# bronemos/view-fusion

Measured on AMD Instinct MI355X. Metric: denoise_steps_per_sec, higher is better.
Workload: dtype f32; 1 GPU; small UNet 64x64 (33.9M params), B=16/GPU N=6 (S=96 views/GPU), training iteration fwd+bwd+Adam, linear T=2000 schedule; global_batch=16, views=6, parallelism=dp1, launch=HIP-graph replay of the whole iteration

## Files before the change

### include/vf_hip.h

```cpp
#ifndef VF_HIP_H
#define VF_HIP_H
#ifdef __cplusplus
extern "C" {
#endif

int vf_gn_fwd(const float* x, const float* gamma, const float* beta, float* y, float* mean ,
              float* rstd , int S, int C, int HW, int groups, float eps, int silu, void* stream);
int vf_gn_bwd_emits_rowsum(int C, int HW, int groups);
int vf_gn_bwd(const float* x, const float* gamma, const float* beta, const float* mean, const float* rstd,
              const float* dy, const float* addend, float* dx, float* dgamma_part, float* dbeta_part,
              float* dx_rowsum, int S, int C, int HW, int groups, int silu, void* stream);
int vf_gn_cat_fwd(const float* x, const float* x2, int C1, const float* gamma, const float* beta, float* y, float* mean,
                  float* rstd, int S, int C, int HW, int groups, float eps, int silu, void* stream);
int vf_gn_cat_bwd(const float* x, const float* x2, int C1, const float* gamma, const float* beta, const float* mean,
                  const float* rstd, const float* dy, const float* addend, const float* addend2, float* dx, float* dx2,
                  float* dgamma_part, float* dbeta_part, float* dx_rowsum, int S, int C, int HW, int groups, int silu,
                  void* stream);
int vf_rowsum(const float* x, float* out , int rows, int len, void* stream);
int vf_bias_grad(const float* dy, float* db, float* dvb, int S, int C, int HW, void* stream);
int vf_colsum(const float* part , float* out , int batch, int S, int C,
              void* stream);
int vf_colsum_multi(const void* desc, int n, long total_blocks, void* stream);

int vf_conv_pack_sizes(int Cout, int Cin, int KS, long* fwd_floats, long* bwd_floats);
int vf_conv_pack_weights(const float* w_oihw, float* w_fwd, float* w_bwd , int Cout, int Cin, int KS,
                         void* stream);
int vf_conv_pack_weights_multi(const void* desc, int nlayers, long total_blocks, void* stream);
int vf_conv_fwd(const float* x, const float* w_packed, const float* bias ,
                const float* view_bias , const float* residual , float* y,
                float* ws , long ws_floats, int S, int Cin, int Cout, int H, int W, int KS, int mode,
                void* stream);
int vf_conv_fwd_gn(const float* x, const float* w_packed, const float* bias, const float* view_bias, const float* residual,
                   float* y, int store_y, const float* gn_gamma, const float* gn_beta, float* a_out, float* gn_stats,
                   int groups, float eps, int silu, float* ws, long ws_floats, int S, int Cin, int Cout, int H, int W,
                   int KS, int mode, void* stream);
int vf_conv_small_supported(int Cin, int Cout, int H, int W, int KS, int mode);
int vf_conv_small(const float* x, const float* x2 , int C1, const float* w_oihw, const float* bias ,
                  const float* view_bias , const float* residual , float* y, int S, int Cin, int Cout,
                  int H, int W, int KS, int mode, void* stream);
int vf_conv_small_res(const float* x, const float* w_oihw, const float* bias , const float* view_bias ,
                      float* y, int S, int Cin, int Cout, int H, int W, const float* rx, const float* rx2 ,
                      int rC1, int rC, const float* rw_oihw, const float* rbias , void* stream);
int vf_conv_small_gn(const float* x, const float* x2 , int C1, const float* w_oihw, const float* bias ,
                     const float* view_bias , const float* residual , float* y, int S, int Cin,
                     int Cout, int H, int W, int KS, const unsigned long long* in_stats ,
                     const float* in_gamma, const float* in_beta, int in_groups, float eps, int silu,
                     unsigned long long* out_stats , const float* rx , const float* rx2 ,
                     int rC1, int rC, const float* rw_oihw, const float* rbias , const float* w_packed ,
                     int mode, void* stream);
long vf_conv_small_pack_floats(int Cout, int Cin);
int vf_conv_small_pack(const float* w_oihw, float* w_packed, int Cout, int Cin, void* stream);
long vf_conv_fwd_ws_floats(int S, int Cin, int Cout, int H, int W, int KS);
int vf_conv1x1_cat_fwd(const float* x1, const float* x2, int C1, const float* w_packed, const float* bias, float* y,
                       float* ws, long ws_floats, int S, int Cin, int Cout, int H, int W, void* stream);
int vf_conv1x1_cat_dgrad(const float* dy, const float* w_packed_bwd, float* dx1, float* dx2, int C1, int S, int Cin,
                         int Cout, int H, int W, void* stream);
int vf_conv1x1_cat_wgrad(const float* x1, const float* x2, int C1, const float* dy, float* dw_oihw, float* ws,
                         long ws_floats, int S, int Cin, int Cout, int H, int W, void* stream);
long vf_conv1x1_bf16x3_pack_dwords(int M, int K);
int vf_conv1x1_bf16x3_pack(const float* w_oihw, void* w3_fwd, void* w3_bwd, int Cout, int Cin, void* stream);
int vf_conv1x1_bf16x3(const float* x, const float* x2, int C1in, const void* w3, const float* bias,
                      const float* view_bias, const float* residual, float* y, float* y2, int C1out, int S, int Cin,
                      int Cout, int HW, void* stream);
long vf_conv_wgrad_ws_floats(int S, int Cin, int Cout, int H, int W, int KS);
int vf_conv_wgrad(const float* x, const float* dy, float* dw_oihw, float* ws, long ws_floats, int S, int Cin,
                  int Cout, int H, int W, int KS, int mode, void* stream);
int vf_conv_wgrad_main(const float* x, const float* dy, float* dw_oihw, float* ws, long ws_floats, int S, int Cin,
                       int Cout, int H, int W, int KS, int mode, long long* desc9, int* nblocks, void* stream);
int vf_conv1x1_cat_wgrad_main(const float* x1, const float* x2, int C1, const float* dy, float* dw_oihw, float* ws,
                              long ws_floats, int S, int Cin, int Cout, int H, int W, long long* desc9, int* nblocks,
                              void* stream);
int vf_sumpool2(const float* x, float* y, long n_out, int Wo, void* stream);

int vf_wino_supported(int H, int W, int mode);
int vf_wino_pack_sizes(int Cout, int Cin, long* fwd_floats, long* bwd_floats);
int vf_wino_pack_weights(const float* w_oihw, float* u_fwd, float* u_bwd , int Cout, int Cin,
                         void* stream);
int vf_wino_pack_weights_multi(const void* desc, int nlayers, long total_blocks, void* stream);
long vf_wino_conv_ws_floats(int S, int Cin, int Cout, int H, int W);
int vf_wino_conv_fill_pct(int S, int Cin, int Cout, int H, int W, int* tiles_out);
int vf_wino_conv_fwd(const float* x, const float* u_packed, const float* bias, const float* view_bias,
                     const float* residual, float* y, float* ws, long ws_floats, int S, int Cin, int Cout, int H,
                     int W, int mode, void* stream);
int vf_wino_conv_gn_fusable(int S, int Cin, int Cout, int H, int W, int mode, int groups);
int vf_wino_conv_fwd_gn(const float* x, const float* u_packed, const float* bias , const float* view_bias ,
                        const float* residual , float* y, int store_y, const float* gn_gamma, const float* gn_beta,
                        float* a_out, int groups, float eps, int silu, float* ws, long ws_floats, int S, int Cin, int Cout,
                        int H, int W, int mode, void* stream);
int vf_wino44_supported(int H, int W, int mode);
int vf_wino44_pack_sizes(int Cout, int Cin, long* fwd_floats, long* bwd_floats);
int vf_wino44_pack_weights(const float* w_oihw, float* u_fwd, float* u_bwd , int Cout, int Cin,
                           void* stream);
int vf_wino44_pack_weights_multi(const void* desc, int nlayers, long total_blocks, void* stream);
long vf_wino44_conv_ws_floats(int S, int Cin, int Cout, int H, int W);
int vf_wino44_conv_fill_pct(int S, int Cin, int Cout, int H, int W, int* tiles_out);
int vf_wino44_conv_fwd(const float* x, const float* u_packed, const float* bias, const float* view_bias,
                       const float* residual, float* y, float* ws, long ws_floats, int S, int Cin, int Cout, int H,
                       int W, int mode, void* stream);
int vf_wino_wgrad_supported(int H, int W, int mode);
long vf_wino_wgrad_ws_floats(int S, int Cin, int Cout, int H, int W);
int vf_wino_wgrad(const float* x, const float* dy, float* dw_oihw, float* db, float* db2, float* ws, long ws_floats,
                  int S, int Cin, int Cout, int H, int W, int mode, void* stream);
int vf_wino_wgrad_main(const float* x, const float* dy, float* dw_oihw, float* db, float* db2, float* ws, long ws_floats,
                       int S, int Cin, int Cout, int H, int W, int mode, long long* desc9, int* nblocks, void* stream);
int vf_wino44_reduce_multi(const void* table, int nrows, int nblocks, void* stream);

int vf_time_affine_fwd(const void* desc, int ngroups, const float* emb, float* out, int S, int K, int CT,
                       void* stream);
long vf_time_affine_ws_floats(int S, int K);
int vf_time_affine_bwd(const void* desc, int ngroups, const float* emb, const float* de, float* dw ,
                       float* db , const void* gdst, float* demb , float* ws, int S, int K,
                       int CT, void* stream);

int vf_bgemm(const float* A, const float* B, float* C, const float* bias , int batch, int M, int N,
             int K, long sAb, long sAm, long sAk, long sBb, long sBk, long sBn, long sCb, long sCm, long sCn,
             float alpha, float beta, void* stream);
int vf_attention_fwd(const float* qkv, float* out, float* P , int S, int C, int L, void* stream);
int vf_attention_fwd_kernel(int S, int C, int L);
int vf_attention_dscore(const float* qkv, const float* dO, const float* P, float* dS, float* dqkv, int S, int C, int L,
                        void* stream);
int vf_attention_dvdk(const float* qkv, const float* dO, const float* P, const float* dS, float* dqkv, int S, int C, int L,
                      void* stream);
int vf_attn_stream_fwd(const float* qkv, float* out, float* rowstat , int S, int C, int L, void* stream);
int vf_attn_stream_bwd(const float* qkv, const float* out, const float* dO, const float* rowstat, float* delta,
                       float* dqkv, int S, int C, int L, void* stream);
int vf_softmax_fwd(const float* x, float* y, int rows, int cols, void* stream);
int vf_softmax_bwd(const float* y, const float* dy, float* dx, int rows, int cols, void* stream);

int vf_sincos_embed(const float* level , const float* angle , float* out , int S, int dim,
                    void* stream);
int vf_swish_fwd(const float* x, float* y, long n, void* stream);
int vf_swish_bwd(const float* x, const float* dy, float* dx, long n, void* stream);
int vf_concat_channels(float* a, float* b, float* out, int S, long na, long nb, int split, void* stream);
int vf_dropout(const float* x, const float* u, float* y, long n, float p, void* stream);

int vf_gather_level(const float* gammas, const long long* t, const float* u , float* level, int B,
                    void* stream);
int vf_stack_views(const float* y_cond , const float* y_t ,
                   const float* noise , const float* level, const float* angle, const int* off ,
                   float* x , float* level_s, float* angle_s, int B, int Nmax,
                   int Cc , int HW, int S,
                   int copy_cond, void* stream);
int vf_compose_fwd(const float* unet_out, const int* off, const float* target , float* noise_hat,
                   float* weights , float* loss_part , float* loss, int B,
                   int Cout, int HW, int maxV, int weighting, void* stream);
int vf_compose_mse_bwd(const float* unet_out, const int* off, const float* target, const float* noise_hat,
                       const float* gloss, float* dout, int B, int Cout, int HW, int weighting, void* stream);
int vf_compose_loss_fwd(const float* unet_out, const int* off, const float* target, const float* level,
                        float* noise_hat, float* loss_part , float* sample_loss ,
                        float* sample_w , float* loss, float* bin_sum , int* bin_cnt ,
                        int B, int Cout, int HW, int weighting, int penalty, float delta, int weight_kind, float a,
                        float b, int K, void* stream);
int vf_compose_loss_bwd(const float* unet_out, const int* off, const float* target, const float* noise_hat,
                        const float* gloss, const float* sample_w, float* dout, int B, int Cout, int HW, int weighting,
                        int penalty, float delta, void* stream);
int vf_compose_loss_fwd_scaled(const float* unet_out, const int* off, const float* target, const float* level,
                               const float* scale , float* noise_hat, float* loss_part ,
                               float* sample_loss , float* sample_w , float* loss,
                               float* bin_sum , int* bin_cnt , int B, int Cout, int HW,
                               int weighting, int penalty, float delta, int weight_kind, float a, float b, int K,
                               void* stream);
int vf_draw_level(unsigned long long seed, const long long* ids , const long long* words ,
                  const float* gammas, int T, int K, const unsigned long long* c, const float* iw, const int* ready,
                  long long* t, float* u , float* level , float* iw_out , int B, void* stream);
int vf_level_stats(const float* sample_loss, const float* sample_w , const long long* t, int B, int T, int K,
                   float beta, int warmup, double eps, float* m, int* seen, unsigned long long* c, float* iw,
                   int* ready, void* stream);
int vf_level_table_host(const double* q, int T, int K, double eps, unsigned long long* c, int* lo, float* iw);
int vf_level_draw_host(const unsigned* x, int n, int T, int K, const unsigned long long* c, const float* iw,
                       long long* t, float* iw_out);
int vf_loss_weights_host(const float* level, int B, int kind, float a, float b, float* out );
int vf_compose_loss_pred_fwd(const float* unet_out, const int* off, const float* noise ,
                             const float* y_0, const float* level, const float* scale , float* noise_hat,
                             float* loss_part , float* sample_loss ,
                             float* sample_w , float* loss, float* bin_sum ,
                             int* bin_cnt , int B, int Cout, int HW, int weighting, int penalty, float delta,
                             int weight_kind, float a, float b, int K, int pred, void* stream);
int vf_compose_loss_pred_bwd(const float* unet_out, const int* off, const float* noise ,
                             const float* y_0, const float* level, const float* noise_hat, const float* gloss,
                             const float* sample_w, float* dout, int B, int Cout, int HW, int weighting, int penalty,
                             float delta, int pred, void* stream);
int vf_loss_weights_pred_host(const float* level, int B, int pred, int kind, float a, float b, float* out );
int vf_p_sample_tail(const float* unet_out, const int* off, const float* y_t, const float* z ,
                     const long long* t, const float* sqrt_recip_gammas, const float* sqrt_recipm1_gammas,
                     const float* posterior_log_variance, const float* posterior_mean_coef1,
                     const float* posterior_mean_coef2, float* y_next , float* mean_out ,
                     float* weights , int B, int Cout, int HW, int maxV, int weighting, int clip,
                     void* stream);

int vf_draw_train(unsigned long long seed, const long long* ids, const float* gammas, int T, long long* t,
                  float* u , float* level , int B, void* stream);
int vf_randn_ids(unsigned long long seed, const long long* ids, int kind, int step, float* out, int B, int n,
                 void* stream);
int vf_philox_ids(unsigned long long seed, const long long* ids, int kind, int step, unsigned* out, int B, int n,
                  void* stream);
int vf_p_sample_tail_rng(const float* unet_out, const int* off, const float* y_t, unsigned long long seed,
                         const long long* ids, const long long* t, const float* sqrt_recip_gammas,
                         const float* sqrt_recipm1_gammas, const float* posterior_log_variance,
                         const float* posterior_mean_coef1, const float* posterior_mean_coef2,
                         float* y_next , float* mean_out , float* weights , int B, int Cout,
                         int HW, int maxV, int weighting, int clip, void* stream);
int vf_sampler_step(const float* unet_out, const int* off, const float* y_t, const float* z ,
                    const long long* kidx, const float* a, const float* b, const float* cy, const float* c0,
                    const float* c1, const float* sigma, float* y0_prev , float* y_next,
                    float* weights , int B, int Cout, int HW, int maxV, int weighting, void* stream);
int vf_sampler_step_rng(const float* unet_out, const int* off, const float* y_t, unsigned long long seed,
                        const long long* ids, const long long* kidx, const long long* tau, const float* a,
                        const float* b, const float* cy, const float* c0, const float* c1, const float* sigma,
                        float* y0_prev , float* y_next, float* weights , int B, int Cout, int HW,
                        int maxV, int weighting, void* stream);
int vf_stack_views_cfg(const float* y_cond, const float* y_t, const float* noise , const float* level,
                       const float* angle, const int* off , const unsigned char* drop , float* x,
                       float* level_s, float* angle_s, int B, int Nmax, int Cc, int HW, int S, int copy_cond,
                       int null_rows, void* stream);
int vf_draw_cond_drop(unsigned long long seed, const long long* ids, unsigned thr, unsigned char* drop , int B,
                      void* stream);
int vf_p_sample_tail_cfg(const float* unet_out, const int* off, const float* y_t, const float* z ,
                         const long long* t, const float* sqrt_recip_gammas, const float* sqrt_recipm1_gammas,
                         const float* posterior_log_variance, const float* posterior_mean_coef1,
                         const float* posterior_mean_coef2, float* y_next , float* mean_out ,
                         float* weights , int B, int Cout, int HW, int maxV, int weighting, int clip,
                         const float* g , void* stream);
int vf_p_sample_tail_cfg_rng(const float* unet_out, const int* off, const float* y_t, unsigned long long seed,
                             const long long* ids, const long long* t, const float* sqrt_recip_gammas,
                             const float* sqrt_recipm1_gammas, const float* posterior_log_variance,
                             const float* posterior_mean_coef1, const float* posterior_mean_coef2,
                             float* y_next , float* mean_out , float* weights , int B,
                             int Cout, int HW, int maxV, int weighting, int clip, const float* g ,
                             void* stream);
int vf_sampler_step_cfg(const float* unet_out, const int* off, const float* y_t, const float* z ,
                        const long long* kidx, const float* a, const float* b, const float* cy, const float* c0,
                        const float* c1, const float* sigma, float* y0_prev , float* y_next,
                        float* weights , int B, int Cout, int HW, int maxV, int weighting,
                        const float* g , void* stream);
int vf_sampler_step_cfg_rng(const float* unet_out, const int* off, const float* y_t, unsigned long long seed,
                            const long long* ids, const long long* kidx, const long long* tau, const float* a,
                            const float* b, const float* cy, const float* c0, const float* c1, const float* sigma,
                            float* y0_prev , float* y_next, float* weights , int B, int Cout, int HW,
                            int maxV, int weighting, const float* g , void* stream);
int vf_compose_eps(const float* unet_out, const int* off, const float* g , float* eps,
                   float* weights , double* part, int B, int Cout, int HW, int maxV, int weighting, int fused,
                   void* stream);
int vf_sample_stat(const float* eps, const double* part , const float* y, const long long* idx, const float* ta,
                   const float* tb, float* stat, int B, int HW, float phi, int k, float frac, float cmax, int fused,
                   void* stream);
int vf_abs_quantile(const float* x, int B, int n, int k, float frac, float* out , void* stream);
int vf_p_sample_tail_eps(const float* eps, const float* stat, const float* y_t, const float* z ,
                         const long long* t, const float* sqrt_recip_gammas, const float* sqrt_recipm1_gammas,
                         const float* posterior_log_variance, const float* posterior_mean_coef1,
                         const float* posterior_mean_coef2, float* y_next , float* mean_out , int B,
                         int HW, int clip, int rescale, int thr, void* stream);
int vf_p_sample_tail_eps_rng(const float* eps, const float* stat, const float* y_t, unsigned long long seed,
                             const long long* ids, const long long* t, const float* sqrt_recip_gammas,
                             const float* sqrt_recipm1_gammas, const float* posterior_log_variance,
                             const float* posterior_mean_coef1, const float* posterior_mean_coef2,
                             float* y_next , float* mean_out , int B, int HW, int clip, int rescale,
                             int thr, void* stream);
int vf_sampler_step_eps(const float* eps, const float* stat, const float* y_t, const float* z ,
                        const long long* kidx, const float* a, const float* b, const float* cy, const float* c0,
                        const float* c1, const float* sigma, float* y0_prev , float* y_next, int B,
                        int HW, int rescale, int thr, void* stream);
int vf_sampler_step_eps_rng(const float* eps, const float* stat, const float* y_t, unsigned long long seed,
                            const long long* ids, const long long* kidx, const long long* tau, const float* a,
                            const float* b, const float* cy, const float* c0, const float* c1, const float* sigma,
                            float* y0_prev , float* y_next, int B, int HW, int rescale, int thr, void* stream);
int vf_distill_begin(unsigned long long seed, const long long* ids , const long long* i_in ,
                     const long long* tau_s, const float* gammas, int K, const float* y_0, const float* noise,
                     long long* i_out, long long* k1, long long* k0, float* level_s, float* z_t, int B, int n,
                     void* stream);
int vf_distill_target(const float* unet_out, const int* off, const float* y, const float* x1, const float* z_t,
                      const float* level_s, const long long* idx, const long long* kidx, const float* a, const float* b,
                      const float* w1, const float* w2, float* x_tilde, float* eps_tilde, int B, int Cout, int HW,
                      int weighting, const float* g , void* stream);
int vf_distill_step_host(unsigned long long seed, const long long* ids, int K, long long* i_out , int B);
int vf_loss_weights_trunc_snr_host(const float* level, int B, int pred, float* out );
int vf_rng_host_philox(const unsigned* counter , const unsigned* key , unsigned* out );
int vf_rng_host_normal(unsigned long long seed, const long long* ids, int kind, int step, float* out ,
                       int B, int n);
int vf_rng_host_train_scalars(unsigned long long seed, const long long* ids, int T, long long* t, float* u, int B);
int vf_cond_drop_host(unsigned long long seed, const long long* ids, unsigned thr, unsigned char* drop , int B);

int vf_batch_assemble(const unsigned char* store, long N, int H, int W, unsigned long long seed, const long long* ids,
                      const long long* objects, int B, int train, int relative, int all, float* y_0, float* y_cond,
                      float* angle, long long* objects_out, void* stream);
int vf_batch_host_plan(unsigned long long seed, const long long* ids, int B, int train, int lo, int hi, long N,
                       const long long* objects, int* src, int* target, int* q01, int* second, long long* view_count,
                       long long* object);

int vf_psnr(const float* generated, const float* target, float* out , int B, int n, void* stream);
long vf_ssim_workspace_floats(int B, int C, int H, int W);
int vf_ssim(const float* generated, const float* target, float* out , float* workspace, int B, int C, int H,
            int W, const float* window11, float data_range, void* stream);
int vf_lpips_prep(const float* generated, const float* target, float* out, int B, int HW, void* stream);
int vf_relu(float* x, long n, void* stream);
int vf_relu_maxpool2(float* y, float* pooled, long planes, int H, int W, void* stream);
int vf_lpips_layer_tiles(int C, int HW);
long vf_lpips_workspace_floats(int B, int H, int W);
int vf_lpips_layer(const float* feat, const float* lin, float* workspace, int B, int C, int HW, int slot0, int slots,
                   void* stream);
int vf_lpips_finish(const float* workspace, float* out , int B, int slots, void* stream);

int vf_adam_multi(const void* desc, int ntensors, long total_blocks, float lr, float beta1, float beta2, float eps,
                  float bias_correction1, float bias_correction2, void* stream);
int vf_adam_multi_dev(const void* desc, int ntensors, long total_blocks, const float* scalars, float beta1, float beta2,
                      float eps, void* stream);
int vf_adam_set_scalars(float* scalars, float lr, float bc1, float bc2, void* stream);

int vf_grad_sumsq_multi(const void* desc, int ntensors, long total_blocks, double* partial, void* stream);
int vf_grad_norm_finish(const double* partial, long n, const float* max_norm, float* out, void* stream);
int vf_adam_multi_ex(const void* desc, const void* ema_tab, int ntensors, long total_blocks, float lr, float beta1,
                     float beta2, float eps, float bias_correction1, float bias_correction2, const float* gscale,
                     const float* ema_scal, void* stream);
int vf_adam_multi_ex_dev(const void* desc, const void* ema_tab, int ntensors, long total_blocks, const float* scalars,
                         float beta1, float beta2, float eps, const float* gscale, const float* ema_scal, void* stream);
int vf_adam_set_scalars_ex(float* scalars, float lr, float bc1, float bc2, float* xs, float ema_d, float ema_omd,
                           float max_norm, void* stream);
int vf_swap_multi(const void* desc, const void* ema_tab, int ntensors, long total_blocks, void* stream);

int vf_grad_accum_multi(const void* desc, int ntensors, long total_blocks, const float* scalars, void* stream);

int vf_xgmi_alloc(void** ptr, long bytes);
int vf_xgmi_free(void* ptr);
int vf_xgmi_export(void* ptr, void* handle64 );
int vf_xgmi_open(const void* handle64, void** ptr);
int vf_xgmi_close(void* ptr);
int vf_xgmi_signal(const void* const* peer_flags, int world, int rank, int slot, unsigned epoch, void* stream);
int vf_xgmi_wait(const void* my_flags, int world, int slot_lo, int slot_hi, unsigned epoch, void* status,
                 long timeout_us, void* stream);
int vf_xgmi_reduce_adam(const void* desc, int ntensors, long total_blocks, const void* const* peer_bases,
                        const float* my_base, float* gavg_base, int world, const float* scalars, float beta1,
                        float beta2, float eps, void* stream);

#ifdef __cplusplus
}
#endif
#endif
```

### view_fusion_amd/_lib.py

```python
import ctypes
import os

import torch

_HERE = os.path.dirname(os.path.abspath(__file__))
LIB_PATH = os.path.join(_HERE, "lib", "libvf_hip.so")
_OVERRIDE = os.environ.get("VF_HIP_LIB") if os.environ.get("VF_DEBUG_AB") == "1" else None
if _OVERRIDE:
    LIB_PATH = _OVERRIDE
elif os.environ.get("VF_HIP_LIB"):
    import warnings
    warnings.warn("VF_HIP_LIB is ignored unless VF_DEBUG_AB=1 (kernel-tuning aid)", stacklevel=2)

_P, _I, _L, _F = ctypes.c_void_p, ctypes.c_int, ctypes.c_long, ctypes.c_float
_U64 = ctypes.c_uint64

SIGNATURES = {
    "vf_gn_fwd": [_P, _P, _P, _P, _P, _P, _I, _I, _I, _I, _F, _I, _P],
    "vf_gn_bwd_emits_rowsum": [_I, _I, _I],
    "vf_gn_cat_fwd": [_P, _P, _I, _P, _P, _P, _P, _P, _I, _I, _I, _I, _F, _I, _P],
    "vf_gn_cat_bwd": [_P, _P, _I, _P, _P, _P, _P, _P, _P, _P, _P, _P, _P, _P, _P, _I, _I, _I, _I, _I, _P],
    "vf_conv1x1_cat_fwd": [_P, _P, _I, _P, _P, _P, _P, _L, _I, _I, _I, _I, _I, _P],
    "vf_conv1x1_cat_dgrad": [_P, _P, _P, _P, _I, _I, _I, _I, _I, _I, _P],
    "vf_conv1x1_cat_wgrad": [_P, _P, _I, _P, _P, _P, _L, _I, _I, _I, _I, _I, _P],
    "vf_gn_bwd": [_P, _P, _P, _P, _P, _P, _P, _P, _P, _P, _P, _I, _I, _I, _I, _I, _P],
    "vf_rowsum": [_P, _P, _I, _I, _P],
    "vf_bias_grad": [_P, _P, _P, _I, _I, _I, _P],
    "vf_colsum": [_P, _P, _I, _I, _I, _P],
    "vf_colsum_multi": [_P, _I, _L, _P],
    "vf_conv_pack_sizes": [_I, _I, _I, ctypes.POINTER(_L), ctypes.POINTER(_L)],
    "vf_conv_pack_weights": [_P, _P, _P, _I, _I, _I, _P],
    "vf_conv_pack_weights_multi": [_P, _I, _L, _P],
    "vf_conv_fwd": [_P, _P, _P, _P, _P, _P, _P, _L, _I, _I, _I, _I, _I, _I, _I, _P],
    "vf_conv_fwd_ws_floats": [_I, _I, _I, _I, _I, _I],
    "vf_conv_fwd_gn": [_P, _P, _P, _P, _P, _P, _I, _P, _P, _P, _P, _I, _F, _I, _P, _L, _I, _I, _I, _I, _I, _I, _I, _P],
    "vf_conv_wgrad_ws_floats": [_I, _I, _I, _I, _I, _I],
    "vf_conv_wgrad": [_P, _P, _P, _P, _L, _I, _I, _I, _I, _I, _I, _I, _P],
    "vf_conv1x1_bf16x3_pack_dwords": [_I, _I],
    "vf_conv1x1_bf16x3_pack": [_P, _P, _P, _I, _I, _P],
    "vf_conv1x1_bf16x3": [_P, _P, _I, _P, _P, _P, _P, _P, _P, _I, _I, _I, _I, _I, _P],
    "vf_wino_supported": [_I, _I, _I],
    "vf_wino_pack_sizes": [_I, _I, ctypes.POINTER(_L), ctypes.POINTER(_L)],
    "vf_wino_pack_weights": [_P, _P, _P, _I, _I, _P],
    "vf_wino_pack_weights_multi": [_P, _I, _L, _P],
    "vf_wino_conv_ws_floats": [_I, _I, _I, _I, _I],
    "vf_wino_conv_fill_pct": [_I, _I, _I, _I, _I, ctypes.POINTER(_I)],
    "vf_wino_conv_fwd": [_P, _P, _P, _P, _P, _P, _P, _L, _I, _I, _I, _I, _I, _I, _P],
    "vf_wino_conv_gn_fusable": [_I, _I, _I, _I, _I, _I, _I],
    "vf_wino_conv_fwd_gn": [_P, _P, _P, _P, _P, _P, _I, _P, _P, _P, _I, _F, _I, _P, _L, _I, _I, _I, _I, _I, _I, _P],
    "vf_wino44_supported": [_I, _I, _I],
    "vf_wino44_pack_sizes": [_I, _I, ctypes.POINTER(_L), ctypes.POINTER(_L)],
    "vf_wino44_pack_weights": [_P, _P, _P, _I, _I, _P],
    "vf_wino44_pack_weights_multi": [_P, _I, _L, _P],
    "vf_wino44_conv_ws_floats": [_I, _I, _I, _I, _I],
    "vf_wino44_conv_fill_pct": [_I, _I, _I, _I, _I, ctypes.POINTER(_I)],
    "vf_wino44_conv_fwd": [_P, _P, _P, _P, _P, _P, _P, _L, _I, _I, _I, _I, _I, _I, _P],
    "vf_wino_wgrad_ws_floats": [_I, _I, _I, _I, _I],
    "vf_wino_wgrad_supported": [_I, _I, _I],
    "vf_wino_wgrad": [_P, _P, _P, _P, _P, _P, _L, _I, _I, _I, _I, _I, _I, _P],
    "vf_wino_wgrad_main": [_P, _P, _P, _P, _P, _P, _L, _I, _I, _I, _I, _I, _I, _P, _P, _P],
    "vf_wino44_reduce_multi": [_P, _I, _I, _P],
    "vf_conv_wgrad_main": [_P, _P, _P, _P, _L, _I, _I, _I, _I, _I, _I, _I, _P, _P, _P],
    "vf_conv1x1_cat_wgrad_main": [_P, _P, _I, _P, _P, _P, _L, _I, _I, _I, _I, _I, _P, _P, _P],
    "vf_sumpool2": [_P, _P, _L, _I, _P],
    "vf_time_affine_fwd": [_P, _I, _P, _P, _I, _I, _I, _P],
    "vf_time_affine_ws_floats": [_I, _I],
    "vf_time_affine_bwd": [_P, _I, _P, _P, _P, _P, _P, _P, _P, _I, _I, _I, _P],
    "vf_bgemm": [_P, _P, _P, _P, _I, _I, _I, _I, _L, _L, _L, _L, _L, _L, _L, _L, _L, _F, _F, _P],
    "vf_attention_fwd": [_P, _P, _P, _I, _I, _I, _P],
    "vf_attention_fwd_kernel": [_I, _I, _I],
    "vf_attention_dscore": [_P, _P, _P, _P, _P, _I, _I, _I, _P],
    "vf_attention_dvdk": [_P, _P, _P, _P, _P, _I, _I, _I, _P],
    "vf_attn_stream_fwd": [_P, _P, _P, _I, _I, _I, _P],
    "vf_attn_stream_bwd": [_P, _P, _P, _P, _P, _P, _I, _I, _I, _P],
    "vf_softmax_fwd": [_P, _P, _I, _I, _P],
    "vf_softmax_bwd": [_P, _P, _P, _I, _I, _P],
    "vf_sincos_embed": [_P, _P, _P, _I, _I, _P],
    "vf_swish_fwd": [_P, _P, _L, _P],
    "vf_swish_bwd": [_P, _P, _P, _L, _P],
    "vf_concat_channels": [_P, _P, _P, _I, _L, _L, _I, _P],
    "vf_dropout": [_P, _P, _P, _L, _F, _P],
    "vf_adam_multi": [_P, _I, _L, _F, _F, _F, _F, _F, _F, _P],
    "vf_conv_small_supported": [_I, _I, _I, _I, _I, _I],
    "vf_conv_small": [_P, _P, _I, _P, _P, _P, _P, _P, _I, _I, _I, _I, _I, _I, _I, _P],
    "vf_conv_small_res": [_P, _P, _P, _P, _P, _I, _I, _I, _I, _I, _P, _P, _I, _I, _P, _P, _P],
    "vf_conv_small_gn": [_P, _P, _I, _P, _P, _P, _P, _P, _I, _I, _I, _I, _I, _I, _P, _P, _P, _I, _F, _I, _P, _P, _P, _I, _I,
                         _P, _P, _P, _I, _P],
    "vf_conv_small_pack_floats": [_I, _I],
    "vf_conv_small_pack": [_P, _P, _I, _I, _P],
    "vf_adam_multi_dev": [_P, _I, _L, _P, _F, _F, _F, _P],
    "vf_adam_set_scalars": [_P, _F, _F, _F, _P],
    "vf_grad_sumsq_multi": [_P, _I, _L, _P, _P],
    "vf_grad_norm_finish": [_P, _L, _P, _P, _P],
    "vf_adam_multi_ex": [_P, _P, _I, _L, _F, _F, _F, _F, _F, _F, _P, _P, _P],
    "vf_adam_multi_ex_dev": [_P, _P, _I, _L, _P, _F, _F, _F, _P, _P, _P],
    "vf_adam_set_scalars_ex": [_P, _F, _F, _F, _P, _F, _F, _F, _P],
    "vf_swap_multi": [_P, _P, _I, _L, _P],
    "vf_grad_accum_multi": [_P, _I, _L, _P, _P],
    "vf_xgmi_alloc": [ctypes.POINTER(_P), _L],
    "vf_xgmi_free": [_P],
    "vf_xgmi_export": [_P, _P],
    "vf_xgmi_open": [_P, ctypes.POINTER(_P)],
    "vf_xgmi_close": [_P],
    "vf_xgmi_signal": [ctypes.POINTER(_P), _I, _I, _I, ctypes.c_uint, _P],
    "vf_xgmi_wait": [_P, _I, _I, _I, ctypes.c_uint, _P, _L, _P],
    "vf_xgmi_reduce_adam": [_P, _I, _L, ctypes.POINTER(_P), _P, _P, _I, _P, _F, _F, _F, _P],
    "vf_psnr": [_P, _P, _P, _I, _I, _P],
    "vf_ssim_workspace_floats": [_I, _I, _I, _I],
    "vf_ssim": [_P, _P, _P, _P, _I, _I, _I, _I, _P, _F, _P],
    "vf_lpips_prep": [_P, _P, _P, _I, _I, _P],
    "vf_relu": [_P, _L, _P],
    "vf_relu_maxpool2": [_P, _P, _L, _I, _I, _P],
    "vf_lpips_layer_tiles": [_I, _I],
    "vf_lpips_workspace_floats": [_I, _I, _I],
    "vf_lpips_layer": [_P, _P, _P, _I, _I, _I, _I, _I, _P],
    "vf_lpips_finish": [_P, _P, _I, _I, _P],
    "vf_gather_level": [_P, _P, _P, _P, _I, _P],
    "vf_stack_views": [_P, _P, _P, _P, _P, _P, _P, _P, _P, _I, _I, _I, _I, _I, _I, _P],
    "vf_compose_fwd": [_P, _P, _P, _P, _P, _P, _P, _I, _I, _I, _I, _I, _P],
    "vf_compose_mse_bwd": [_P, _P, _P, _P, _P, _P, _I, _I, _I, _I, _P],
    "vf_compose_loss_fwd": [_P, _P, _P, _P, _P, _P, _P, _P, _P, _P, _P, _I, _I, _I, _I, _I, _F, _I, _F, _F, _I, _P],
    "vf_compose_loss_bwd": [_P, _P, _P, _P, _P, _P, _P, _I, _I, _I, _I, _I, _F, _P],
    "vf_loss_weights_host": [_P, _I, _I, _F, _F, _P],
    "vf_compose_loss_fwd_scaled": [_P, _P, _P, _P, _P, _P, _P, _P, _P, _P, _P, _P, _I, _I, _I, _I, _I, _F, _I, _F, _F, _I,
                                   _P],
    "vf_compose_loss_pred_fwd": [_P, _P, _P, _P, _P, _P, _P, _P, _P, _P, _P, _P, _P, _I, _I, _I, _I, _I, _F, _I, _F, _F, _I,
                                 _I, _P],
    "vf_compose_loss_pred_bwd": [_P, _P, _P, _P, _P, _P, _P, _P, _P, _I, _I, _I, _I, _I, _F, _I, _P],
    "vf_loss_weights_pred_host": [_P, _I, _I, _I, _F, _F, _P],
    "vf_draw_level": [_U64, _P, _P, _P, _I, _I, _P, _P, _P, _P, _P, _P, _P, _I, _P],
    "vf_level_stats": [_P, _P, _P, _I, _I, _I, _F, _I, ctypes.c_double, _P, _P, _P, _P, _P, _P],
    "vf_level_table_host": [_P, _I, _I, ctypes.c_double, _P, _P, _P],
    "vf_level_draw_host": [_P, _I, _I, _I, _P, _P, _P, _P],
    "vf_p_sample_tail": [_P, _P, _P, _P, _P, _P, _P, _P, _P, _P, _P, _P, _P, _I, _I, _I, _I, _I, _I, _P],
    "vf_draw_train": [_U64, _P, _P, _I, _P, _P, _P, _I, _P],
    "vf_randn_ids": [_U64, _P, _I, _I, _P, _I, _I, _P],
    "vf_philox_ids": [_U64, _P, _I, _I, _P, _I, _I, _P],
    "vf_p_sample_tail_rng": [_P, _P, _P, _U64, _P, _P, _P, _P, _P, _P, _P, _P, _P, _P, _I, _I, _I, _I, _I, _I, _P],
    "vf_sampler_step": [_P, _P, _P, _P, _P, _P, _P, _P, _P, _P, _P, _P, _P, _P, _I, _I, _I, _I, _I, _P],
    "vf_sampler_step_rng": [_P, _P, _P, _U64, _P, _P, _P, _P, _P, _P, _P, _P, _P, _P, _P, _P, _I, _I, _I, _I, _I, _P],
    "vf_stack_views_cfg": [_P, _P, _P, _P, _P, _P, _P, _P, _P, _P, _I, _I, _I, _I, _I, _I, _I, _P],
    "vf_draw_cond_drop": [_U64, _P, ctypes.c_uint, _P, _I, _P],
    "vf_cond_drop_host": [_U64, _P, ctypes.c_uint, _P, _I],
    "vf_p_sample_tail_cfg": [_P, _P, _P, _P, _P, _P, _P, _P, _P, _P, _P, _P, _P, _I, _I, _I, _I, _I, _I, _P, _P],
    "vf_p_sample_tail_cfg_rng": [_P, _P, _P, _U64, _P, _P, _P, _P, _P, _P, _P, _P, _P, _P, _I, _I, _I, _I, _I, _I, _P, _P],
    "vf_sampler_step_cfg": [_P, _P, _P, _P, _P, _P, _P, _P, _P, _P, _P, _P, _P, _P, _I, _I, _I, _I, _I, _P, _P],
    "vf_sampler_step_cfg_rng": [_P, _P, _P, _U64, _P, _P, _P, _P, _P, _P, _P, _P, _P, _P, _P, _P, _I, _I, _I, _I, _I, _P, _P],
    "vf_compose_eps": [_P, _P, _P, _P, _P, _P, _I, _I, _I, _I, _I, _I, _P],
    "vf_sample_stat": [_P, _P, _P, _P, _P, _P, _P, _I, _I, _F, _I, _F, _F, _I, _P],
    "vf_abs_quantile": [_P, _I, _I, _I, _F, _P, _P],
    "vf_p_sample_tail_eps": [_P, _P, _P, _P, _P, _P, _P, _P, _P, _P, _P, _P, _I, _I, _I, _I, _I, _P],
    "vf_p_sample_tail_eps_rng": [_P, _P, _P, _U64, _P, _P, _P, _P, _P, _P, _P, _P, _P, _I, _I, _I, _I, _I, _P],
    "vf_sampler_step_eps": [_P, _P, _P, _P, _P, _P, _P, _P, _P, _P, _P, _P, _P, _I, _I, _I, _I, _P],
    "vf_sampler_step_eps_rng": [_P, _P, _P, _U64, _P, _P, _P, _P, _P, _P, _P, _P, _P, _P, _P, _I, _I, _I, _I, _P],
    "vf_distill_begin": [_U64, _P, _P, _P, _P, _I, _P, _P, _P, _P, _P, _P, _P, _I, _I, _P],
    "vf_distill_target": [_P, _P, _P, _P, _P, _P, _P, _P, _P, _P, _P, _P, _P, _P, _I, _I, _I, _I, _P, _P],
    "vf_distill_step_host": [_U64, _P, _I, _P, _I],
    "vf_loss_weights_trunc_snr_host": [_P, _I, _I, _P],
    "vf_rng_host_philox": [_P, _P, _P],
    "vf_rng_host_normal": [_U64, _P, _I, _I, _P, _I, _I],
    "vf_rng_host_train_scalars": [_U64, _P, _I, _P, _P, _I],
    "vf_batch_assemble": [_P, _L, _I, _I, _U64, _P, _P, _I, _I, _I, _I, _P, _P, _P, _P, _P],
    "vf_batch_host_plan": [_U64, _P, _I, _I, _I, _I, _L, _P, _P, _P, _P, _P, _P, _P],
}
_RESTYPE = {"vf_conv1x1_bf16x3_pack_dwords": _L, "vf_conv_wgrad_ws_floats": _L, "vf_time_affine_ws_floats": _L, "vf_wino_conv_ws_floats": _L, "vf_wino44_conv_ws_floats": _L, "vf_wino_wgrad_ws_floats": _L, "vf_conv_fwd_ws_floats": _L,
            "vf_conv_small_pack_floats": _L, "vf_ssim_workspace_floats": _L, "vf_lpips_workspace_floats": _L}

_lib = None
N_CALLS = 0


class VFHipError(RuntimeError):
    pass


def load():
    global _lib
    if _lib is None:
        if not os.path.exists(LIB_PATH):
            raise VFHipError(
                f"{LIB_PATH} not found: build it with `python -m view_fusion_amd.build` "
                "(there is no CPU / eager fallback for the ViewFusion hot path)")
        lib = ctypes.CDLL(LIB_PATH)
        if _OVERRIDE:
            import sys
            print(f"[view_fusion_amd] VF_DEBUG_AB: loading {LIB_PATH} instead of lib/libvf_hip.so", file=sys.stderr)
        missing = [name for name in SIGNATURES if not hasattr(lib, name)]
        if missing:
            raise VFHipError(f"{LIB_PATH} does not export {missing}: stale build? run `python -m view_fusion_amd.build`")
        for name, args in SIGNATURES.items():
            fn = getattr(lib, name)
            fn.argtypes = args
            fn.restype = _RESTYPE.get(name, _I)
        _lib = lib
    return _lib


def call(name, *args):
    global N_CALLS
    N_CALLS += 1
    rc = getattr(load(), name)(*args)
    if rc != 0:
        raise VFHipError(f"{name} failed with hipError_t {rc}")
```

### view_fusion_amd/csrc/attention.hip

```cpp
#include "common.h"

namespace {

__global__ __launch_bounds__(512) void attn_fwd_kh_kernel(const float* __restrict__ qkv, float* __restrict__ out,
                                                          float* __restrict__ P, int C, float alpha) {
    constexpr int L = 256, NTH = 512, QW = 128, NKT = 4, CKA = 16, RSV = L + 4;
    constexpr int KS = L + 32;
    constexpr int KQ = CKA * KS + CKA * QW, VT = 32 * RSV;
    __shared__ __attribute__((aligned(16))) float lds[2 * (KQ > VT ? KQ : VT)];
    __shared__ float oex[2][4][16][64];
    __shared__ float red[2][2][QW];

    const int tid = threadIdx.x, lane = tid & 63, wid = tid >> 6;
    const int li = lane & 31, lh = lane >> 5;
    const int qb = wid & 3, kh = wid >> 2;
    const int b = blockIdx.y, q0 = blockIdx.x * QW;
    const float* qp = qkv + (size_t)b * 3 * C * L;
    const float* kp = qp + (size_t)C * L;
    const float* vp = qp + (size_t)2 * C * L;

#ifdef VF_ATTN_STAMPS
    long long st_[6] = {clock64(), 0, 0, 0, 0, 0}, rt0_ = wall_clock64();
#endif
    f32x16 acc[NKT];
#pragma unroll
    for (int t = 0; t < NKT; ++t) acc[t] = (f32x16){0};

    float4 kr0, kr1, qr;
#define VF_AK_LOAD(C0) {                                                                                    \
        kr0 = *reinterpret_cast<const float4*>(kp + (size_t)((C0) + tid / 64) * L + 4 * (tid % 64));          \
        kr1 = *reinterpret_cast<const float4*>(kp + (size_t)((C0) + 8 + tid / 64) * L + 4 * (tid % 64));      \
        qr = *reinterpret_cast<const float4*>(qp + (size_t)((C0) + tid / 32) * L + q0 + 4 * (tid % 32)); }
#define VF_AK_STORE(BUF) { float* kl_ = lds + (BUF) * KQ;                                                    \
        *reinterpret_cast<float4*>(kl_ + (tid / 64) * KS + 4 * (tid % 64)) = kr0;                             \
        *reinterpret_cast<float4*>(kl_ + (8 + tid / 64) * KS + 4 * (tid % 64)) = kr1;                         \
        *reinterpret_cast<float4*>(kl_ + CKA * KS + (tid / 32) * QW + 4 * (tid % 32)) = qr; }
    VF_AK_LOAD(0);
    VF_AK_STORE(0);
    VF_AK_LOAD(min(CKA, C - CKA));
    __syncthreads();
    for (int c0 = 0, cur = 0; c0 < C; c0 += CKA, cur ^= 1) {
        VF_AK_STORE(cur ^ 1);
        VF_AK_LOAD(min(c0 + 2 * CKA, C - CKA));
        const float* Kl = lds + cur * KQ;
        const float* Ql = Kl + CKA * KS;
        const float* kq = Kl + lh * KS + kh * NKT * 32 + li;
        const float* qq = Ql + lh * QW + qb * 32 + li;
        float bq = qq[0], ak0 = kq[0], ak1 = kq[32], ak2 = kq[64], ak3 = kq[96];
#pragma unroll
        for (int s = 0; s < CKA / 2; ++s) {
            float bqn = bq, an0 = ak0, an1 = ak1, an2 = ak2, an3 = ak3;
            if (s + 1 < CKA / 2) {
                bqn = qq[(2 * s + 2) * QW];
                an0 = kq[(2 * s + 2) * KS];
                an1 = kq[(2 * s + 2) * KS + 32];
                an2 = kq[(2 * s + 2) * KS + 64];
                an3 = kq[(2 * s + 2) * KS + 96];
            }
            __builtin_amdgcn_sched_barrier(0);
            acc[0] = __builtin_amdgcn_mfma_f32_32x32x2f32(ak0, bq, acc[0], 0, 0, 0);
            acc[1] = __builtin_amdgcn_mfma_f32_32x32x2f32(ak1, bq, acc[1], 0, 0, 0);
            acc[2] = __builtin_amdgcn_mfma_f32_32x32x2f32(ak2, bq, acc[2], 0, 0, 0);
            acc[3] = __builtin_amdgcn_mfma_f32_32x32x2f32(ak3, bq, acc[3], 0, 0, 0);
            __builtin_amdgcn_sched_barrier(0);
            bq = bqn; ak0 = an0; ak1 = an1; ak2 = an2; ak3 = an3;
        }
        __syncthreads();
    }
#undef VF_AK_LOAD
#undef VF_AK_STORE
#ifdef VF_ATTN_STAMPS
    st_[1] = clock64();
#endif
    float4 vr0, vr1, vr2, vr3;
#define VF_AK_LV(I, C0) { const int e = tid + (I) * NTH;                                                   \
        vr##I = *reinterpret_cast<const float4*>(vp + (size_t)((C0) + e / 64) * L + 4 * (e % 64)); }
#define VF_AK_SV(I, BUF) { const int e = tid + (I) * NTH;                                                   \
        *reinterpret_cast<float4*>(lds + (BUF) * VT + (e / 64) * RSV + 4 * (e % 64)) = vr##I; }
#define VF_AK_LOADV(C0) { VF_AK_LV(0, C0) VF_AK_LV(1, C0) VF_AK_LV(2, C0) VF_AK_LV(3, C0) }
#define VF_AK_STOREV(BUF) { VF_AK_SV(0, BUF) VF_AK_SV(1, BUF) VF_AK_SV(2, BUF) VF_AK_SV(3, BUF) }
    VF_AK_LOADV(0);

    const int ql = qb * 32 + li;
    float mx = -INFINITY;
#pragma unroll
    for (int t = 0; t < NKT; ++t)
#pragma unroll
        for (int r = 0; r < 16; ++r) mx = fmaxf(mx, acc[t][r]);
    mx = fmaxf(mx, __shfl_xor(mx, 32, 64));
    if (lh == 0) red[0][kh][ql] = mx;
    __syncthreads();
    mx = fmaxf(red[0][0][ql], red[0][1][ql]);
    const float c2 = alpha * 1.44269504088896341f, mc = mx * c2;
    float sum = 0.f;
#pragma unroll
    for (int t = 0; t < NKT; ++t)
#pragma unroll
        for (int r = 0; r < 16; ++r) {
            const float p = __builtin_amdgcn_exp2f(fmaf(acc[t][r], c2, -mc));
            acc[t][r] = p;
            sum += p;
        }
    sum += __shfl_xor(sum, 32, 64);
    if (lh == 0) red[1][kh][ql] = sum;
    VF_AK_STOREV(0);
    VF_AK_LOADV(min(32, C - 32));
    __syncthreads();
    const float inv = 1.0f / (red[1][0][ql] + red[1][1][ql]);
#pragma unroll
    for (int t = 0; t < NKT; ++t)
#pragma unroll
        for (int r = 0; r < 16; ++r) acc[t][r] *= inv;

    const int qi = q0 + ql;
#ifdef VF_ATTN_STAMPS
    st_[2] = clock64();
    if (false) {
#else
    if (P) {
#endif
        float* pr = P + ((size_t)b * L + qi) * L + kh * NKT * 32;
#pragma unroll
        for (int t = 0; t < NKT; ++t)
#pragma unroll
            for (int g = 0; g < 4; ++g)
                *reinterpret_cast<float4*>(pr + t * 32 + 8 * g + 4 * lh) =
                    make_float4(acc[t][4 * g], acc[t][4 * g + 1], acc[t][4 * g + 2], acc[t][4 * g + 3]);
    }
#ifdef VF_ATTN_STAMPS
    st_[3] = clock64();
#endif

    f32x16 oprev = {0};
    for (int c0 = 0, cur = 0; c0 < C; c0 += 32, cur ^= 1) {
        if (kh == 0 && c0 > 0) {
#pragma unroll
            for (int r = 0; r < 16; ++r) {
                const int c = c0 - 32 + (r & 3) + 8 * (r >> 2) + 4 * lh;
                out[((size_t)b * C + c) * L + qi] = oprev[r] + oex[cur ^ 1][qb][r][lane];
            }
        }
        VF_AK_STOREV(cur ^ 1);
        VF_AK_LOADV(min(c0 + 64, C - 32));
        const float* Vl = lds + cur * VT;
        f32x16 o = {0};
        const float* vq = Vl + li * RSV + kh * NKT * 32 + 4 * lh;
        float4 av = *reinterpret_cast<const float4*>(vq);
#pragma unroll
        for (int t = 0; t < NKT; ++t)
#pragma unroll
            for (int g = 0; g < 4; ++g) {
                float4 avn = av;
                if (t * 4 + g + 1 < NKT * 4) avn = *reinterpret_cast<const float4*>(vq + (t * 4 + g + 1) * 8);
                __builtin_amdgcn_sched_barrier(0);
                o = __builtin_amdgcn_mfma_f32_32x32x2f32(av.x, acc[t][4 * g + 0], o, 0, 0, 0);
                o = __builtin_amdgcn_mfma_f32_32x32x2f32(av.y, acc[t][4 * g + 1], o, 0, 0, 0);
                o = __builtin_amdgcn_mfma_f32_32x32x2f32(av.z, acc[t][4 * g + 2], o, 0, 0, 0);
                o = __builtin_amdgcn_mfma_f32_32x32x2f32(av.w, acc[t][4 * g + 3], o, 0, 0, 0);
                __builtin_amdgcn_sched_barrier(0);
                av = avn;
            }
        if (kh == 1) {
#pragma unroll
            for (int r = 0; r < 16; ++r) oex[cur][qb][r][lane] = o[r];
        } else {
            oprev = o;
        }
        VF_LDS_BARRIER();
    }
    if (kh == 0) {
        const int last = (C / 32 - 1) & 1;
#pragma unroll
        for (int r = 0; r < 16; ++r) {
            const int c = C - 32 + (r & 3) + 8 * (r >> 2) + 4 * lh;
            out[((size_t)b * C + c) * L + qi] = oprev[r] + oex[last][qb][r][lane];
        }
    }
#undef VF_AK_LOADV
#undef VF_AK_STOREV
#undef VF_AK_LV
#undef VF_AK_SV
#ifdef VF_ATTN_STAMPS
    if (tid == 0 && P) {
        long long* o = reinterpret_cast<long long*>(P) + (size_t)(blockIdx.y * gridDim.x + blockIdx.x) * 8;
        o[0] = st_[0]; o[1] = st_[1]; o[2] = st_[2]; o[3] = st_[3]; o[4] = clock64(); o[5] = 0;
        o[6] = rt0_; o[7] = wall_clock64();
    }
#endif
}

template <bool DSCORE>
__global__ __launch_bounds__(256, 3) void attn_fwd_q32_kernel(const float* __restrict__ qkv, float* __restrict__ out,
                                                              float* __restrict__ P, int C, float alpha, int S,
                                                              const float* __restrict__ dO, float* __restrict__ dS) {
    constexpr int L = 256, NTH = 256, NKT = 2, CKA = 16;
    constexpr int KS = L + 32;
    constexpr int KQ = CKA * KS + CKA * 32;
    constexpr int RSV = 36, VW = 32 * RSV;
    constexpr int OEX = 4 * 16 * 64;
    constexpr int PV = 4 * VW + 2 * OEX;
    __shared__ __attribute__((aligned(16))) float lds[2 * KQ > PV ? 2 * KQ : PV];
    __shared__ float red[2][4][32];

    const int tid = threadIdx.x, lane = tid & 63;
    const int w = __builtin_amdgcn_readfirstlane(tid >> 6);
    const int li = lane & 31, lh = lane >> 5;
    int b, u;
    {
        const int i = blockIdx.x, nfull = (S >> 3) << 6;
        if (i < nfull) { const int j = i >> 3; b = ((j >> 3) << 3) + (i & 7); u = j & 7; }
        else { const int r = i - nfull; b = ((S >> 3) << 3) + (r >> 3); u = r & 7; }
    }
    const int q0 = u * 32;
    const float* qp = DSCORE ? dO + (size_t)b * C * L : qkv + (size_t)b * 3 * C * L;
    const float* kp = qkv + ((size_t)b * 3 + (DSCORE ? 2 : 1)) * C * L;
    const float* vp = qkv + ((size_t)b * 3 + (DSCORE ? 1 : 2)) * C * L;
#ifdef VF_ATTN_STAMPS
    long long st_[6] = {clock64(), 0, 0, 0, 0, 0}, rt0_ = wall_clock64();
#endif

    f32x16 acc[NKT];
#pragma unroll
    for (int t = 0; t < NKT; ++t) acc[t] = (f32x16){0};

    f32x4 ka0, ka1, ka2, ka3, qa, kb0, kb1, kb2, kb3, qb_;
    const int qe = tid & 127;
    unsigned kvo = (unsigned)((4 * w * L + 4 * lane) * 4);
    unsigned qvo = (unsigned)(((qe >> 3) * L + q0 + 4 * (qe & 7)) * 4);
    float* const kst = lds + 4 * w * KS + 4 * lane;
    float* const qst = lds + CKA * KS + (qe >> 3) * 32 + 4 * (qe & 7);
#define VF_GLD4(BASE, OFS, IMM) (*(const __attribute__((address_space(1))) f32x4*)((const __attribute__((address_space(1))) char*)(BASE) + (OFS) + (IMM)))
#define VF_A3_LK(R, I, KC) R##I = VF_GLD4(KC, kvo, (I) * (L * 4));
#define VF_A3_LOAD(R, Q, C0) { const char* kc_ = uniform_ptr(kp + (size_t)(C0) * L);                               \
        const char* qc_ = uniform_ptr(qp + (size_t)(C0) * L);                                                    \
        asm("" : "+s"(kc_), "+s"(qc_), "+v"(kvo), "+v"(qvo));                                                    \
        VF_A3_LK(R, 0, kc_) VF_A3_LK(R, 1, kc_) VF_A3_LK(R, 2, kc_) VF_A3_LK(R, 3, kc_)                             \
        Q = VF_GLD4(qc_, qvo, 0); }
#define VF_A3_SK(R, I, BUF) *reinterpret_cast<f32x4*>(kst + (BUF) * KQ + (I) * KS) = R##I;
#define VF_A3_STORE(R, Q, BUF) { VF_A3_SK(R, 0, BUF) VF_A3_SK(R, 1, BUF) VF_A3_SK(R, 2, BUF) VF_A3_SK(R, 3, BUF)   \
        *reinterpret_cast<f32x4*>(qst + (BUF) * KQ) = Q; }
#define VF_A3_MFMAS(BUF, MID) {                                                                                 \
        const float* Kl = lds + (BUF) * KQ;                                                                    \
        const float* kq = Kl + lh * KS + w * (NKT * 32) + li;                                                  \
        const float* qq = Kl + CKA * KS + lh * 32 + li;                                                        \
        float bq = qq[0], ak0 = kq[0], ak1 = kq[32];                                                           \
        _Pragma("unroll")                                                                                      \
        for (int s = 0; s < CKA / 2; ++s) {                                                                    \
            float bqn = bq, an0 = ak0, an1 = ak1;                                                              \
            if (s + 1 < CKA / 2) {                                                                             \
                bqn = qq[(2 * s + 2) * 32];                                                                    \
                an0 = kq[(2 * s + 2) * KS];                                                                    \
                an1 = kq[(2 * s + 2) * KS + 32];                                                               \
            }                                                                                                  \
            __builtin_amdgcn_sched_barrier(0);                                                                 \
            acc[0] = __builtin_amdgcn_mfma_f32_32x32x2f32(ak0, bq, acc[0], 0, 0, 0);                           \
            acc[1] = __builtin_amdgcn_mfma_f32_32x32x2f32(ak1, bq, acc[1], 0, 0, 0);                           \
            __builtin_amdgcn_sched_barrier(0);                                                                 \
            if (s == 0) { MID __builtin_amdgcn_sched_barrier(0); }                                             \
            bq = bqn; ak0 = an0; ak1 = an1;                                                                    \
        } }
    VF_A3_LOAD(ka, qa, 0);
    VF_A3_STORE(ka, qa, 0);
    VF_A3_LOAD(ka, qa, CKA);
    VF_A3_LOAD(kb, qb_, min(2 * CKA, C - CKA));
    __syncthreads();
    for (int c0 = 0; c0 < C; c0 += 2 * CKA) {
        VF_A3_MFMAS(0, VF_A3_STORE(ka, qa, 1) VF_A3_LOAD(ka, qa, min(c0 + 3 * CKA, C - CKA)));
        VF_LDS_BARRIER();
        VF_A3_MFMAS(1, VF_A3_STORE(kb, qb_, 0) VF_A3_LOAD(kb, qb_, min(c0 + 4 * CKA, C - CKA)));
        VF_LDS_BARRIER();
    }
#undef VF_A3_MFMAS
#undef VF_A3_LOAD
#undef VF_A3_STORE
#undef VF_A3_LK
#undef VF_A3_SK

#ifdef VF_ATTN_STAMPS
    st_[1] = clock64();
#endif
    f32x4 va0, va1, va2, va3, vb0, vb1, vb2, vb3;
    unsigned vvo = (unsigned)((4 * (lane >> 3) * L + w * (NKT * 32) + 4 * (lane & 7)) * 4);
    float* const Vw = lds + w * VW;
    float* const vdst = Vw + 4 * (lane >> 3) * RSV + 4 * (lane & 7);
#define VF_A3_LV(R, I, VC) R##I = VF_GLD4(VC, vvo, (I) * (L * 4));
#define VF_A3_LOADV(R, N) { const char* vc_ = uniform_ptr(vp + (size_t)(((N) >> 1) * 32) * L + ((N) & 1) * 32);      \
        asm("" : "+s"(vc_), "+v"(vvo));                                                                          \
        VF_A3_LV(R, 0, vc_) VF_A3_LV(R, 1, vc_) VF_A3_LV(R, 2, vc_) VF_A3_LV(R, 3, vc_) }
#define VF_A3_SV(R, I) *reinterpret_cast<f32x4*>(vdst + (I) * RSV) = R##I;
#define VF_A3_STOREV(R) { VF_A3_SV(R, 0) VF_A3_SV(R, 1) VF_A3_SV(R, 2) VF_A3_SV(R, 3) }
    const int npiece = C / 16;
    VF_A3_LOADV(va, 0);
    VF_A3_LOADV(vb, 1);

    const int qi = q0 + li;
    if constexpr (DSCORE) {
        const size_t prow = ((size_t)b * L + qi) * L + w * (NKT * 32) + 4 * lh;
        float4 pv[NKT][4];
#pragma unroll
        for (int t = 0; t < NKT; ++t)
#pragma unroll
            for (int g = 0; g < 4; ++g) pv[t][g] = *reinterpret_cast<const float4*>(P + prow + t * 32 + 8 * g);
        float dot = 0.f;
#pragma unroll
        for (int t = 0; t < NKT; ++t)
#pragma unroll
            for (int g = 0; g < 4; ++g)
                dot += (pv[t][g].x * acc[t][4 * g] + pv[t][g].y * acc[t][4 * g + 1]) +
                       (pv[t][g].z * acc[t][4 * g + 2] + pv[t][g].w * acc[t][4 * g + 3]);
        dot += __shfl_xor(dot, 32, 64);
        if (lh == 0) red[0][w][li] = dot;
        __syncthreads();
        VF_A3_STOREV(va);
        VF_A3_LOADV(va, min(2, npiece - 1));
        dot = (red[0][0][li] + red[0][1][li]) + (red[0][2][li] + red[0][3][li]);
#pragma unroll
        for (int t = 0; t < NKT; ++t)
#pragma unroll
            for (int g = 0; g < 4; ++g) {
                const float4 d = make_float4(pv[t][g].x * (acc[t][4 * g] - dot), pv[t][g].y * (acc[t][4 * g + 1] - dot),
                                             pv[t][g].z * (acc[t][4 * g + 2] - dot), pv[t][g].w * (acc[t][4 * g + 3] - dot));
                *reinterpret_cast<float4*>(dS + prow + t * 32 + 8 * g) = d;
                acc[t][4 * g] = d.x; acc[t][4 * g + 1] = d.y; acc[t][4 * g + 2] = d.z; acc[t][4 * g + 3] = d.w;
            }
    } else {
    float mx = -INFINITY;
#pragma unroll
    for (int t = 0; t < NKT; ++t)
#pragma unroll
        for (int r = 0; r < 16; ++r) mx = fmaxf(mx, acc[t][r]);
    mx = fmaxf(mx, __shfl_xor(mx, 32, 64));
    if (lh == 0) red[0][w][li] = mx;
    __syncthreads();
    mx = fmaxf(fmaxf(red[0][0][li], red[0][1][li]), fmaxf(red[0][2][li], red[0][3][li]));
    const float c2 = alpha * 1.44269504088896341f, mc = mx * c2;
    float sum = 0.f;
#pragma unroll
    for (int t = 0; t < NKT; ++t)
#pragma unroll
        for (int r = 0; r < 16; ++r) {
            const float p = __builtin_amdgcn_exp2f(fmaf(acc[t][r], c2, -mc));
            acc[t][r] = p;
            sum += p;
        }
    sum += __shfl_xor(sum, 32, 64);
    if (lh == 0) red[1][w][li] = sum;
    VF_A3_STOREV(va);
    VF_A3_LOADV(va, min(2, npiece - 1));
    __syncthreads();
    const float inv = 1.0f / ((red[1][0][li] + red[1][1][li]) + (red[1][2][li] + red[1][3][li]));
#pragma unroll
    for (int t = 0; t < NKT; ++t)
#pragma unroll
        for (int r = 0; r < 16; ++r) acc[t][r] *= inv;

#ifdef VF_ATTN_STAMPS
    st_[2] = clock64();
    if (false) {
#else
    if (P) {
#endif
        float* pr = P + ((size_t)b * L + qi) * L + w * (NKT * 32);
#pragma unroll
        for (int t = 0; t < NKT; ++t)
#pragma unroll
            for (int g = 0; g < 4; ++g)
                *reinterpret_cast<float4*>(pr + t * 32 + 8 * g + 4 * lh) =
                    make_float4(acc[t][4 * g], acc[t][4 * g + 1], acc[t][4 * g + 2], acc[t][4 * g + 3]);
    }
    }

#ifdef VF_ATTN_STAMPS
    st_[3] = clock64();
#endif
    float* const oex = lds + 4 * VW;
    const float* vq = Vw + li * RSV + 4 * lh;
#define VF_A3_PV(T) {                                                                                          \
        float4 av = *reinterpret_cast<const float4*>(vq);                                                      \
        _Pragma("unroll")                                                                                      \
        for (int g = 0; g < 4; ++g) {                                                                          \
            float4 avn = av;                                                                                   \
            if (g + 1 < 4) avn = *reinterpret_cast<const float4*>(vq + (g + 1) * 8);                           \
            __builtin_amdgcn_sched_barrier(0);                                                                 \
            o = __builtin_amdgcn_mfma_f32_32x32x2f32(av.x, acc[T][4 * g + 0], o, 0, 0, 0);                      \
            o = __builtin_amdgcn_mfma_f32_32x32x2f32(av.y, acc[T][4 * g + 1], o, 0, 0, 0);                      \
            o = __builtin_amdgcn_mfma_f32_32x32x2f32(av.z, acc[T][4 * g + 2], o, 0, 0, 0);                      \
            o = __builtin_amdgcn_mfma_f32_32x32x2f32(av.w, acc[T][4 * g + 3], o, 0, 0, 0);                      \
            __builtin_amdgcn_sched_barrier(0);                                                                 \
            av = avn;                                                                                          \
        } }
    for (int ct = 0; ct < npiece / 2; ++ct) {
        f32x16 o = {0};
        VF_A3_PV(0)
        VF_A3_STOREV(vb);
        VF_A3_LOADV(vb, min(2 * ct + 3, npiece - 1));
        VF_A3_PV(1)
        VF_A3_STOREV(va);
        VF_A3_LOADV(va, min(2 * ct + 4, npiece - 1));
        float* ox = oex + (ct & 1) * OEX;
#pragma unroll
        for (int r = 0; r < 16; ++r) ox[(w * 16 + r) * 64 + lane] = o[r];
        VF_LDS_BARRIER();
        float* ob = out + ((size_t)b * (DSCORE ? 3 * C : C) + ct * 32 + 8 * w + 4 * lh) * L + qi;
#pragma unroll
        for (int r = 0; r < 4; ++r) {
            const float* x_ = ox + (4 * w + r) * 64 + lane;
            const float v_ = (x_[0] + x_[16 * 64]) + (x_[32 * 64] + x_[48 * 64]);
            ob[(size_t)r * L] = DSCORE ? alpha * v_ : v_;
        }
    }
#undef VF_A3_PV
#undef VF_A3_LOADV
#undef VF_A3_STOREV
#undef VF_A3_LV
#undef VF_A3_SV
#undef VF_GLD4
#ifdef VF_ATTN_STAMPS
    if (tid == 0 && P) {
        long long* o_ = reinterpret_cast<long long*>(P) + (size_t)blockIdx.x * 8;
        o_[0] = st_[0]; o_[1] = st_[1]; o_[2] = st_[2]; o_[3] = st_[3]; o_[4] = clock64(); o_[5] = 0;
        o_[6] = rt0_; o_[7] = wall_clock64();
    }
#endif
}

template <int L>
__global__ __launch_bounds__(L / 32 * 64) void attn_fwd_split_kernel(const float* __restrict__ qkv,
                                                                     float* __restrict__ out, float* __restrict__ P,
                                                                     int C, float alpha) {
    constexpr int NW = L / 32, NTH = NW * 64, CKA = 32;
    constexpr int KS = L + 32;
    constexpr int PS = 40;
    constexpr int STAGE = CKA * KS + CKA * 32, PSZ = L * PS;
    __shared__ __attribute__((aligned(16))) float lds[STAGE > PSZ ? STAGE : PSZ];
    __shared__ float red[2][NW][32];
    float* const Kl = lds;
    float* const Ql = lds + CKA * KS;
    float* const Pl = lds;

    const int tid = threadIdx.x, lane = tid & 63, wid = tid >> 6;
    const int li = lane & 31, lh = lane >> 5;
    const int b = blockIdx.y, q0 = blockIdx.x * 32;
    const float* qb = qkv + (size_t)b * 3 * C * L;
    const float* kb = qb + (size_t)C * L;
    const float* vb = qb + (size_t)2 * C * L;

    constexpr int NK4 = CKA * L / 4 / NTH;
    static_assert(NK4 == 4, "K staging");
    constexpr int NQ4 = NTH >= 256 ? 1 : 256 / NTH;
    const int eq = tid & 255;
    float4 kr0, kr1, kr2, kr3, qr, qr1;
    qr1 = make_float4(0.f, 0.f, 0.f, 0.f);
#define VF_AS_LK(I, C0) { const int e = tid + (I) * NTH;                                                   \
        kr##I = *reinterpret_cast<const float4*>(kb + (size_t)((C0) + e / (L / 4)) * L + 4 * (e % (L / 4))); }
#define VF_AS_SK(I) { const int e = tid + (I) * NTH;                                                        \
        *reinterpret_cast<float4*>(Kl + (e / (L / 4)) * KS + 4 * (e % (L / 4))) = kr##I; }
#define load_chunk(C0) { VF_AS_LK(0, C0) VF_AS_LK(1, C0) VF_AS_LK(2, C0) VF_AS_LK(3, C0)                  \
        qr = *reinterpret_cast<const float4*>(qb + (size_t)((C0) + eq / 8) * L + q0 + 4 * (eq % 8));           \
        if constexpr (NQ4 == 2)                                                                                \
            qr1 = *reinterpret_cast<const float4*>(qb + (size_t)((C0) + (eq + NTH) / 8) * L + q0 + 4 * (eq % 8)); }
    f32x16 acc = {0};
    load_chunk(0);
    for (int c0 = 0; c0 < C; c0 += CKA) {
        __syncthreads();
        VF_AS_SK(0) VF_AS_SK(1) VF_AS_SK(2) VF_AS_SK(3)
        if (tid < 256) *reinterpret_cast<float4*>(Ql + (eq / 8) * 32 + 4 * (eq % 8)) = qr;
        if constexpr (NQ4 == 2) *reinterpret_cast<float4*>(Ql + ((eq + NTH) / 8) * 32 + 4 * (eq % 8)) = qr1;
        __syncthreads();
        load_chunk(min(c0 + CKA, C - CKA));
#pragma unroll
        for (int s = 0; s < CKA / 2; ++s)
            acc = __builtin_amdgcn_mfma_f32_32x32x2f32(Kl[(2 * s + lh) * KS + wid * 32 + li],
                                                       Ql[(2 * s + lh) * 32 + li], acc, 0, 0, 0);
    }

    constexpr int NB = L / 64;
    const int ntile = C / 32;
#undef load_chunk
#undef VF_AS_LK
#undef VF_AS_SK
    float4 va0, va1, va2, va3, va4, va5, va6, va7, vn0, vn1, vn2, vn3, vn4, vn5, vn6, vn7;
#define VF_AS_LV1(V, G, SRC) V##G = *reinterpret_cast<const float4*>((SRC) + 8 * (G));
#define load_v(V, TILE, KB) { const float* src_ = vb + (size_t)((TILE) * 32 + li) * L + (KB) * 64 + 4 * lh;  \
        VF_AS_LV1(V, 0, src_) VF_AS_LV1(V, 1, src_) VF_AS_LV1(V, 2, src_) VF_AS_LV1(V, 3, src_)              \
        VF_AS_LV1(V, 4, src_) VF_AS_LV1(V, 5, src_) VF_AS_LV1(V, 6, src_) VF_AS_LV1(V, 7, src_) }
    load_v(va, min(wid, ntile - 1), 0);

    float mx = acc[0];
#pragma unroll
    for (int r = 1; r < 16; ++r) mx = fmaxf(mx, acc[r]);
    mx = fmaxf(mx, __shfl_xor(mx, 32, 64));
    if (lh == 0) red[0][wid][li] = mx;
    __syncthreads();
    mx = red[0][0][li];
#pragma unroll
    for (int w = 1; w < NW; ++w) mx = fmaxf(mx, red[0][w][li]);
    const float c2 = alpha * 1.44269504088896341f, mc = mx * c2;
    float sum = 0.f;
#pragma unroll
    for (int r = 0; r < 16; ++r) {
        acc[r] = __builtin_amdgcn_exp2f(fmaf(acc[r], c2, -mc));
        sum += acc[r];
    }
    sum += __shfl_xor(sum, 32, 64);
    if (lh == 0) red[1][wid][li] = sum;
    __syncthreads();
    sum = red[1][0][li];
#pragma unroll
    for (int w = 1; w < NW; ++w) sum += red[1][w][li];
    const float inv = 1.0f / sum;
#pragma unroll
    for (int r = 0; r < 16; ++r) acc[r] *= inv;

#pragma unroll
    for (int r = 0; r < 16; ++r) Pl[(wid * 32 + 8 * (r >> 2) + 4 * lh + (r & 3)) * PS + li] = acc[r];
    if (P) {
        float* pr = P + ((size_t)b * L + q0 + li) * L + wid * 32 + 4 * lh;
#pragma unroll
        for (int g = 0; g < 4; ++g)
            *reinterpret_cast<float4*>(pr + 8 * g) = make_float4(acc[4 * g], acc[4 * g + 1], acc[4 * g + 2], acc[4 * g + 3]);
    }
    __syncthreads();

    for (int t = wid; t < ntile; t += NW) {
        f32x16 o = {0};
#pragma unroll 1
        for (int kbt = 0; kbt < NB; ++kbt) {
            const int nt = kbt + 1 < NB ? t : min(t + NW, ntile - 1), nk = kbt + 1 < NB ? kbt + 1 : 0;
            load_v(vn, nt, nk);
            const float* pl = Pl + (kbt * 64 + 4 * lh) * PS + li;
#define VF_AS_PV(G) {                                                                                        \
                o = __builtin_amdgcn_mfma_f32_32x32x2f32(va##G.x, pl[(8 * (G) + 0) * PS], o, 0, 0, 0);          \
                o = __builtin_amdgcn_mfma_f32_32x32x2f32(va##G.y, pl[(8 * (G) + 1) * PS], o, 0, 0, 0);          \
                o = __builtin_amdgcn_mfma_f32_32x32x2f32(va##G.z, pl[(8 * (G) + 2) * PS], o, 0, 0, 0);          \
                o = __builtin_amdgcn_mfma_f32_32x32x2f32(va##G.w, pl[(8 * (G) + 3) * PS], o, 0, 0, 0); }
            VF_AS_PV(0) VF_AS_PV(1) VF_AS_PV(2) VF_AS_PV(3) VF_AS_PV(4) VF_AS_PV(5) VF_AS_PV(6) VF_AS_PV(7)
#undef VF_AS_PV
            va0 = vn0; va1 = vn1; va2 = vn2; va3 = vn3; va4 = vn4; va5 = vn5; va6 = vn6; va7 = vn7;
        }
        float* ob = out + ((size_t)b * C + t * 32 + 4 * lh) * L + q0 + li;
#pragma unroll
        for (int r = 0; r < 16; ++r) ob[(size_t)((r & 3) + 8 * (r >> 2)) * L] = o[r];
    }
#undef load_v
#undef VF_AS_LV1
}

template <int L>
__global__ __launch_bounds__(L / 32 * 64) void attn_fwd_q16_kernel(const float* __restrict__ qkv, float* __restrict__ out,
                                                                   float* __restrict__ P, int C, float alpha) {
    constexpr int NW = L / 32, QB = 16, PF = 16;
    constexpr int KPI = L < 128 ? L : 128;
    constexpr int NG = KPI / 16, NH = L / KPI;
    __shared__ __attribute__((aligned(16))) float Pl[(L / 4) * QB * 4];
    __shared__ float red[2][NW][QB];
    __shared__ __attribute__((aligned(16))) float oxs[NW / 2][4][64];

    const int tid = threadIdx.x, lane = tid & 63, wid = tid >> 6;
    const int j = lane & 15, kk = lane >> 4;
    const int b = blockIdx.y, q0 = blockIdx.x * QB;
    const float* qb = qkv + (size_t)b * 3 * C * L;
    const float* kb = qb + (size_t)C * L;
    const float* vb = qb + (size_t)2 * C * L;

    const float* kcol = kb + (size_t)kk * L + 32 * wid + j;
    const float* qcol = qb + (size_t)kk * L + q0 + j;
    const int nblk = C / (4 * PF);
    f32x4 s0 = {0.f, 0.f, 0.f, 0.f}, s1 = s0;
    float kA[PF], kB[PF], qA[PF], lA[PF], lB[PF], rA[PF];
#define VF_Q16_LOAD(K0, K1, QD, BLK)                                                                          \
    { const size_t o_ = (size_t)min((BLK), nblk - 1) * (4 * PF) * L;        \
      _Pragma("unroll") for (int s = 0; s < PF; ++s) {                                                         \
          K0[s] = kcol[o_ + (size_t)(4 * s) * L]; K1[s] = kcol[o_ + (size_t)(4 * s) * L + 16];                  \
          QD[s] = qcol[o_ + (size_t)(4 * s) * L]; } }
#define VF_Q16_MMA(K0, K1, QD)                                                                                \
    { _Pragma("unroll") for (int s = 0; s < PF; ++s) {                                                         \
          s0 = __builtin_amdgcn_mfma_f32_16x16x4f32(K0[s], QD[s], s0, 0, 0, 0);                                 \
          s1 = __builtin_amdgcn_mfma_f32_16x16x4f32(K1[s], QD[s], s1, 0, 0, 0); } }
    VF_Q16_LOAD(kA, kB, qA, 0);
    for (int blk = 0; blk < nblk; blk += 2) {
        VF_Q16_LOAD(lA, lB, rA, blk + 1);
        VF_Q16_MMA(kA, kB, qA);
        if (blk + 1 < nblk) {
            VF_Q16_LOAD(kA, kB, qA, blk + 2);
            VF_Q16_MMA(lA, lB, rA);
        }
    }
#undef VF_Q16_LOAD
#undef VF_Q16_MMA

    const int nitem = NH * (C / 16);
    float4 va0, va1, va2, va3, va4, va5, va6, va7, vn0, vn1, vn2, vn3, vn4, vn5, vn6, vn7;
    va4 = va5 = va6 = va7 = vn4 = vn5 = vn6 = vn7 = make_float4(0.f, 0.f, 0.f, 0.f);
#define VF_Q16_LV1(V, G, SRC) if constexpr ((G) < NG) V##G = *reinterpret_cast<const float4*>((SRC) + 16 * (G));
#define VF_Q16_LOADV(V, ITEM) { const int it_ = min((ITEM), nitem - 1);                                        \
        const float* src_ = vb + (size_t)((it_ / NH) * 16 + j) * L + KPI * (it_ % NH) + 4 * kk;                 \
        VF_Q16_LV1(V, 0, src_) VF_Q16_LV1(V, 1, src_) VF_Q16_LV1(V, 2, src_) VF_Q16_LV1(V, 3, src_)             \
        VF_Q16_LV1(V, 4, src_) VF_Q16_LV1(V, 5, src_) VF_Q16_LV1(V, 6, src_) VF_Q16_LV1(V, 7, src_) }
    VF_Q16_LOADV(va, wid);

    float mx = fmaxf(fmaxf(fmaxf(s0[0], s0[1]), fmaxf(s0[2], s0[3])), fmaxf(fmaxf(s1[0], s1[1]), fmaxf(s1[2], s1[3])));
    mx = fmaxf(mx, __shfl_xor(mx, 16, 64));
    mx = fmaxf(mx, __shfl_xor(mx, 32, 64));
    if (kk == 0) red[0][wid][j] = mx;
    __syncthreads();
    mx = red[0][0][j];
#pragma unroll
    for (int w = 1; w < NW; ++w) mx = fmaxf(mx, red[0][w][j]);
    const float c2 = alpha * 1.44269504088896341f, mc = mx * c2;
    float sum = 0.f;
#pragma unroll
    for (int r = 0; r < 4; ++r) {
        s0[r] = __builtin_amdgcn_exp2f(fmaf(s0[r], c2, -mc));
        s1[r] = __builtin_amdgcn_exp2f(fmaf(s1[r], c2, -mc));
        sum += s0[r] + s1[r];
    }
    sum += __shfl_xor(sum, 16, 64);
    sum += __shfl_xor(sum, 32, 64);
    if (kk == 0) red[1][wid][j] = sum;
    __syncthreads();
    sum = red[1][0][j];
#pragma unroll
    for (int w = 1; w < NW; ++w) sum += red[1][w][j];
    const float inv = 1.0f / sum;
    s0 *= inv;
    s1 *= inv;

    *reinterpret_cast<f32x4*>(Pl + ((8 * wid + kk) * QB + j) * 4) = s0;
    *reinterpret_cast<f32x4*>(Pl + ((8 * wid + 4 + kk) * QB + j) * 4) = s1;
    if (P) {
        float* pr = P + ((size_t)b * L + q0 + j) * L + 32 * wid + 4 * kk;
        *reinterpret_cast<f32x4*>(pr) = s0;
        *reinterpret_cast<f32x4*>(pr + 16) = s1;
    }
    __syncthreads();

    for (int base = 0; base < nitem; base += NW) {
        const int it = base + wid, t = it / NH, h = it % NH;
        VF_Q16_LOADV(vn, it + NW);
        f32x4 pb[NG];
#pragma unroll
        for (int g = 0; g < NG; ++g) pb[g] = *reinterpret_cast<const f32x4*>(Pl + (((KPI / 4) * h + 4 * g + kk) * QB + j) * 4);
        f32x4 o = {0.f, 0.f, 0.f, 0.f};
#define VF_Q16_PV(G) if constexpr ((G) < NG) {                                                                \
        o = __builtin_amdgcn_mfma_f32_16x16x4f32(va##G.x, pb[(G) < NG ? (G) : 0][0], o, 0, 0, 0);                 \
        o = __builtin_amdgcn_mfma_f32_16x16x4f32(va##G.y, pb[(G) < NG ? (G) : 0][1], o, 0, 0, 0);                 \
        o = __builtin_amdgcn_mfma_f32_16x16x4f32(va##G.z, pb[(G) < NG ? (G) : 0][2], o, 0, 0, 0);                 \
        o = __builtin_amdgcn_mfma_f32_16x16x4f32(va##G.w, pb[(G) < NG ? (G) : 0][3], o, 0, 0, 0); }
        VF_Q16_PV(0) VF_Q16_PV(1) VF_Q16_PV(2) VF_Q16_PV(3) VF_Q16_PV(4) VF_Q16_PV(5) VF_Q16_PV(6) VF_Q16_PV(7)
#undef VF_Q16_PV
        va0 = vn0; va1 = vn1; va2 = vn2; va3 = vn3; va4 = vn4; va5 = vn5; va6 = vn6; va7 = vn7;
        float* ob = out + ((size_t)b * C + t * 16 + 4 * kk) * L + q0 + j;
        if constexpr (NH == 2) {
            if (h == 1) {
#pragma unroll
                for (int r = 0; r < 4; ++r) oxs[wid >> 1][r][lane] = o[r];
            }
            __syncthreads();
            if (h == 0) {
#pragma unroll
                for (int r = 0; r < 4; ++r) ob[(size_t)r * L] = o[r] + oxs[wid >> 1][r][lane];
            }
            if (base + NW < nitem) __syncthreads();
        } else {
#pragma unroll
            for (int r = 0; r < 4; ++r) ob[(size_t)r * L] = o[r];
        }
    }
#undef VF_Q16_LOADV
#undef VF_Q16_LV1
}

__global__ __launch_bounds__(256, 5) void attn_bwd_dvdk_kernel(const float* __restrict__ qkv, const float* __restrict__ dO,
                                                               const float* __restrict__ P, const float* __restrict__ dS,
                                                               float* __restrict__ dqkv, int C, float alpha, int S) {
    constexpr int L = 256, BKQ = 32, AS = BKQ + 4, BS = 128 + 4;
    __shared__ __attribute__((aligned(16))) float Al[64 * AS];
    __shared__ __attribute__((aligned(16))) float Bl[BKQ * BS];
    const int tid = threadIdx.x, lane = tid & 63;
    const int w = __builtin_amdgcn_readfirstlane(tid >> 6);
    const int wm = w & 1, wn = w >> 1, li = lane & 31, lh = lane >> 5;
    const int nt = (C / 64) * 2;
    int pair, tile;
    {
        const int i = blockIdx.x, npair = 2 * S, nfull = (npair >> 3) << 3;
        if (i < nfull * nt) { const int j = i >> 3; pair = ((j / nt) << 3) + (i & 7); tile = j % nt; }
        else { const int r = i - nfull * nt; pair = nfull + r / nt; tile = r % nt; }
    }
    const int b = pair >> 1, z = pair & 1;
    const int m0 = (tile >> 1) * 64, n0 = (tile & 1) * 128;
    const float* A = z ? qkv + (size_t)b * 3 * C * L : dO + (size_t)b * C * L;
    const float* B = (z ? dS : P) + (size_t)b * L * L + n0;
    float* out = dqkv + ((size_t)b * 3 + (z ? 1 : 2)) * C * L;

    unsigned avo = (unsigned)(((tid >> 3) * L + 4 * (tid & 7)) * 4), bvo = (unsigned)(((tid >> 5) * L + 4 * (tid & 31)) * 4);
    f32x4 ar0, ar1, br0, br1, br2, br3;
#define VF_GLD4(BASE, OFS, IMM) (*(const __attribute__((address_space(1))) f32x4*)((const __attribute__((address_space(1))) char*)(BASE) + (OFS) + (IMM)))
#define VF_KV_LOAD(K0) {                                                                                        \
        const char* a0_ = uniform_ptr(A + (size_t)m0 * L + (K0));                                                \
        const char* a1_ = uniform_ptr(A + (size_t)(m0 + 32) * L + (K0));                                         \
        const char* b0_ = uniform_ptr(B + (size_t)(K0) * L);                                                     \
        const char* b1_ = uniform_ptr(B + (size_t)((K0) + 8) * L);                                               \
        const char* b2_ = uniform_ptr(B + (size_t)((K0) + 16) * L);                                              \
        const char* b3_ = uniform_ptr(B + (size_t)((K0) + 24) * L);                                              \
        asm("" : "+s"(a0_), "+s"(a1_), "+s"(b0_), "+s"(b1_), "+s"(b2_), "+s"(b3_), "+v"(avo), "+v"(bvo));        \
        ar0 = VF_GLD4(a0_, avo, 0); ar1 = VF_GLD4(a1_, avo, 0);                                                  \
        br0 = VF_GLD4(b0_, bvo, 0); br1 = VF_GLD4(b1_, bvo, 0); br2 = VF_GLD4(b2_, bvo, 0); br3 = VF_GLD4(b3_, bvo, 0); }
    float* const ast = Al + (tid >> 3) * AS + 4 * (tid & 7);
    float* const bst = Bl + (tid >> 5) * BS + 4 * (tid & 31);
#define VF_KV_STORE() {                                                                                         \
        *reinterpret_cast<f32x4*>(ast) = ar0; *reinterpret_cast<f32x4*>(ast + 32 * AS) = ar1;                    \
        *reinterpret_cast<f32x4*>(bst) = br0; *reinterpret_cast<f32x4*>(bst + 8 * BS) = br1;                     \
        *reinterpret_cast<f32x4*>(bst + 16 * BS) = br2; *reinterpret_cast<f32x4*>(bst + 24 * BS) = br3; }

    f32x16 acc0 = {0}, acc1 = {0};
    const float* af = Al + (wm * 32 + li) * AS + 4 * lh;
    const float* bf = Bl + (4 * lh) * BS + wn * 64 + li;
    VF_KV_LOAD(0);
    for (int k0 = 0; k0 < L; k0 += BKQ) {
        VF_LDS_BARRIER();
        VF_KV_STORE();
        VF_LDS_BARRIER();
        float4 a_cur = *reinterpret_cast<const float4*>(af);
        float b00 = bf[0], b01 = bf[BS], b02 = bf[2 * BS], b03 = bf[3 * BS];
        float b10 = bf[32], b11 = bf[BS + 32], b12 = bf[2 * BS + 32], b13 = bf[3 * BS + 32];
#pragma unroll
        for (int grp = 0; grp < BKQ / 8; ++grp) {
            float4 a_nxt = a_cur;
            float c00 = b00, c01 = b01, c02 = b02, c03 = b03, c10 = b10, c11 = b11, c12 = b12, c13 = b13;
            if (grp + 1 < BKQ / 8) {
                a_nxt = *reinterpret_cast<const float4*>(af + 8 * (grp + 1));
                const float* bn = bf + 8 * (grp + 1) * BS;
                c00 = bn[0]; c01 = bn[BS]; c02 = bn[2 * BS]; c03 = bn[3 * BS];
                c10 = bn[32]; c11 = bn[BS + 32]; c12 = bn[2 * BS + 32]; c13 = bn[3 * BS + 32];
            }
            __builtin_amdgcn_sched_barrier(0);
            acc0 = __builtin_amdgcn_mfma_f32_32x32x2f32(a_cur.x, b00, acc0, 0, 0, 0);
            acc1 = __builtin_amdgcn_mfma_f32_32x32x2f32(a_cur.x, b10, acc1, 0, 0, 0);
            acc0 = __builtin_amdgcn_mfma_f32_32x32x2f32(a_cur.y, b01, acc0, 0, 0, 0);
            acc1 = __builtin_amdgcn_mfma_f32_32x32x2f32(a_cur.y, b11, acc1, 0, 0, 0);
            __builtin_amdgcn_sched_barrier(0);
            if (grp == 0) { VF_KV_LOAD(min(k0 + BKQ, L - BKQ)); __builtin_amdgcn_sched_barrier(0); }
            acc0 = __builtin_amdgcn_mfma_f32_32x32x2f32(a_cur.z, b02, acc0, 0, 0, 0);
            acc1 = __builtin_amdgcn_mfma_f32_32x32x2f32(a_cur.z, b12, acc1, 0, 0, 0);
            acc0 = __builtin_amdgcn_mfma_f32_32x32x2f32(a_cur.w, b03, acc0, 0, 0, 0);
            acc1 = __builtin_amdgcn_mfma_f32_32x32x2f32(a_cur.w, b13, acc1, 0, 0, 0);
            __builtin_amdgcn_sched_barrier(0);
            a_cur = a_nxt;
            b00 = c00; b01 = c01; b02 = c02; b03 = c03; b10 = c10; b11 = c11; b12 = c12; b13 = c13;
        }
    }
#undef VF_KV_LOAD
#undef VF_KV_STORE
#undef VF_GLD4
    const float sc = z ? alpha : 1.0f;
    float* o = out + (size_t)(m0 + wm * 32 + 4 * lh) * L + n0 + wn * 64 + li;
#pragma unroll
    for (int r = 0; r < 16; ++r) {
        const int c = (r & 3) + 8 * (r >> 2);
        o[(size_t)c * L] = sc * acc0[r];
        o[(size_t)c * L + 32] = sc * acc1[r];
    }
}

}

extern "C" {

int vf_attention_fwd_kernel(int S, int C, int L) {
    if (S <= 0 || C <= 0 || C % 32 != 0) return 0;
    static const bool q16 = !(getenv("VF_ATTN_Q16") && getenv("VF_ATTN_Q16")[0] == '0');
    static const bool q32 = !(getenv("VF_ATTN_Q32") && getenv("VF_ATTN_Q32")[0] == '0');
    const bool q32_wins = 177 * ((S + 31) / 32) + 30 < 660 * ((S + 127) / 128);
    if ((L == 256 || L == 64) && S <= 16 && C % 64 == 0 && q16) return 1;
    if (L == 256 && q32 && q32_wins) return 2;
    if (L == 256 && S <= 52 && !q32) return 3;
    if (L == 256) return 4;
    return L == 64 ? 3 : 0;
}

int vf_attention_fwd(const float* qkv, float* out, float* P, int S, int C, int L, void* stream) {
    if (S <= 0) return 0;
    if (C % 32 != 0) return (int)hipErrorInvalidValue;
    const float alpha = 1.0f / sqrtf((float)C);
    hipStream_t st = (hipStream_t)stream;
    const int kernel = vf_attention_fwd_kernel(S, C, L);
    if (kernel == 1 && L == 256)
        hipLaunchKernelGGL(attn_fwd_q16_kernel<256>, dim3(16, S), dim3(512), 0, st, qkv, out, P, C, alpha);
    else if (kernel == 1)
        hipLaunchKernelGGL(attn_fwd_q16_kernel<64>, dim3(4, S), dim3(128), 0, st, qkv, out, P, C, alpha);
    else if (kernel == 2)
        hipLaunchKernelGGL(attn_fwd_q32_kernel<false>, dim3(8 * S), dim3(256), 0, st, qkv, out, P, C, alpha, S, nullptr, nullptr);
    else if (kernel == 3 && L == 256)
        hipLaunchKernelGGL(attn_fwd_split_kernel<256>, dim3(8, S), dim3(512), 0, st, qkv, out, P, C, alpha);
    else if (kernel == 4)
        hipLaunchKernelGGL(attn_fwd_kh_kernel, dim3(2, S), dim3(512), 0, st, qkv, out, P, C, alpha);
    else if (kernel == 3)
        hipLaunchKernelGGL(attn_fwd_split_kernel<64>, dim3(2, S), dim3(128), 0, st, qkv, out, P, C, alpha);
    else
        return (int)hipErrorInvalidValue;
    VF_RETURN_LAST_ERROR();
}

int vf_attention_dscore(const float* qkv, const float* dO, const float* P, float* dS, float* dqkv, int S, int C, int L,
                        void* stream) {
    if (S <= 0) return 0;
    if (L != 256 || C % 32 != 0 || C < 32) return (int)hipErrorInvalidValue;
    hipLaunchKernelGGL(attn_fwd_q32_kernel<true>, dim3(8 * S), dim3(256), 0, (hipStream_t)stream, qkv, dqkv,
                       const_cast<float*>(P), C, 1.0f / sqrtf((float)C), S, dO, dS);
    VF_RETURN_LAST_ERROR();
}

int vf_attention_dvdk(const float* qkv, const float* dO, const float* P, const float* dS, float* dqkv, int S, int C, int L,
                      void* stream) {
    if (S <= 0) return 0;
    if (L != 256 || C % 64 != 0 || C < 64) return (int)hipErrorInvalidValue;
    hipLaunchKernelGGL(attn_bwd_dvdk_kernel, dim3(2 * S * (C / 64) * 2), dim3(256), 0, (hipStream_t)stream, qkv, dO, P, dS,
                       dqkv, C, 1.0f / sqrtf((float)C), S);
    VF_RETURN_LAST_ERROR();
}

}
```

### view_fusion_amd/csrc/gemm.hip

```cpp
#include "common.h"

namespace {

constexpr int BM = 64, BN = 64, BK = 32, LDT = 65;

struct GemmArgs {
    const float* A;
    const float* B;
    float* C;
    const float* bias;
    int M, N, K;
    long sAb, sAm, sAk, sBb, sBk, sBn, sCb, sCm, sCn;
    float alpha, beta;
    int xcd_batches;
};

__global__ __launch_bounds__(256) void bgemm_kernel(GemmArgs g) {
    __shared__ float Al[BK * LDT];
    __shared__ float Bl[BK * LDT];
    const int tid = threadIdx.x, lane = tid & 63, wid = tid >> 6;
    const int wm = wid & 1, wn = wid >> 1, li = lane & 31, lh = lane >> 5;
    const int m0 = blockIdx.y * BM, n0 = blockIdx.x * BN, b = blockIdx.z;
    const float* A = g.A + (long)b * g.sAb;
    const float* B = g.B + (long)b * g.sBb;
// ... 28 lines not shown
    float* C = g.C + (long)b * g.sCb;
    const int n = n0 + wn * 32 + li;
    if (n < g.N) {
        const float bn = g.bias ? g.bias[n] : 0.f;
#pragma unroll
        for (int r = 0; r < 16; ++r) {
            const int m = m0 + wm * 32 + (r & 3) + 8 * (r >> 2) + 4 * lh;
            if (m < g.M) {
                float* p = C + (long)m * g.sCm + (long)n * g.sCn;
                float v = g.alpha * acc[r] + bn;
                if (g.beta != 0.f) v += g.beta * *p;
                *p = v;
            }
        }
    }
}


template <bool A_KC, bool B_KC>
__global__ __launch_bounds__(256) void bgemm_v2_kernel(GemmArgs g) {
    constexpr int KS_ = BK + 4;
    __shared__ __attribute__((aligned(16))) float Al[A_KC ? BM * KS_ : BK * BM];
    __shared__ __attribute__((aligned(16))) float Bl[B_KC ? BN * KS_ : BK * BN];
    const int tid = threadIdx.x, lane = tid & 63, wid = tid >> 6;
    const int wm = wid & 1, wn = wid >> 1, li = lane & 31, lh = lane >> 5;
    int bx = blockIdx.x, by = blockIdx.y, b = blockIdx.z;
    if (g.xcd_batches) {
        const int nt = gridDim.x * gridDim.y, i = bx + gridDim.x * (by + gridDim.y * b);
        if (i < (g.xcd_batches << 3) * nt) {
            const int j = i >> 3, tile = j % nt;
            b = ((j / nt) << 3) + (i & 7);
            bx = tile % gridDim.x; by = tile / gridDim.x;
        }
    }
    const int m0 = by * BM, n0 = bx * BN;
    const float* A = g.A + (long)b * g.sAb;
    const float* B = g.B + (long)b * g.sBb;

    float4 ar[2], br[2];
    auto load = [&](int k0) {
#pragma unroll
        for (int i = 0; i < 2; ++i) {
            float4 v = make_float4(0.f, 0.f, 0.f, 0.f);
            if (A_KC) {
                const int m = (tid >> 3) + 32 * i, kq = tid & 7;
                if (m0 + m < g.M && k0 + 4 * kq < g.K)
                    v = *reinterpret_cast<const float4*>(A + (long)(m0 + m) * g.sAm + k0 + 4 * kq);
            } else {
                const int k = (tid >> 4) + 16 * i, mq = tid & 15;
                if (k0 + k < g.K && m0 + 4 * mq < g.M)
                    v = *reinterpret_cast<const float4*>(A + (long)(k0 + k) * g.sAk + m0 + 4 * mq);
            }
            ar[i] = v;
            float4 u = make_float4(0.f, 0.f, 0.f, 0.f);
            if (B_KC) {
                const int n = (tid >> 3) + 32 * i, kq = tid & 7;
                if (n0 + n < g.N && k0 + 4 * kq < g.K)
                    u = *reinterpret_cast<const float4*>(B + (long)(n0 + n) * g.sBn + k0 + 4 * kq);
            } else {
                const int k = (tid >> 4) + 16 * i, nq = tid & 15;
                if (k0 + k < g.K && n0 + 4 * nq < g.N)
                    u = *reinterpret_cast<const float4*>(B + (long)(k0 + k) * g.sBk + n0 + 4 * nq);
            }
            br[i] = u;
        }
    };
    auto store = [&]() {
#pragma unroll
        for (int i = 0; i < 2; ++i) {
            if (A_KC) *reinterpret_cast<float4*>(Al + ((tid >> 3) + 32 * i) * KS_ + 4 * (tid & 7)) = ar[i];
            else      *reinterpret_cast<float4*>(Al + ((tid >> 4) + 16 * i) * BM + 4 * (tid & 15)) = ar[i];
            if (B_KC) *reinterpret_cast<float4*>(Bl + ((tid >> 3) + 32 * i) * KS_ + 4 * (tid & 7)) = br[i];
            else      *reinterpret_cast<float4*>(Bl + ((tid >> 4) + 16 * i) * BN + 4 * (tid & 15)) = br[i];
        }
    };
    auto frag_a = [&](int grp) -> float4 {
        if (A_KC) return *reinterpret_cast<const float4*>(Al + (wm * 32 + li) * KS_ + 8 * grp + 4 * lh);
        const float* p = Al + (8 * grp + 4 * lh) * BM + wm * 32 + li;
        return make_float4(p[0], p[BM], p[2 * BM], p[3 * BM]);
    };
    auto frag_b = [&](int grp) -> float4 {
        if (B_KC) return *reinterpret_cast<const float4*>(Bl + (wn * 32 + li) * KS_ + 8 * grp + 4 * lh);
        const float* p = Bl + (8 * grp + 4 * lh) * BN + wn * 32 + li;
        return make_float4(p[0], p[BN], p[2 * BN], p[3 * BN]);
    };

    f32x16 acc = {0};
    load(0);
    for (int k0 = 0; k0 < g.K; k0 += BK) {
        __syncthreads();
        store();
        __syncthreads();
        if (k0 + BK < g.K) load(k0 + BK);
        float4 a_cur = frag_a(0), b_cur = frag_b(0);
#pragma unroll
        for (int grp = 0; grp < BK / 8; ++grp) {
            float4 a_nxt = a_cur, b_nxt = b_cur;
            if (grp + 1 < BK / 8) { a_nxt = frag_a(grp + 1); b_nxt = frag_b(grp + 1); }
            __builtin_amdgcn_sched_barrier(0);
            acc = __builtin_amdgcn_mfma_f32_32x32x2f32(a_cur.x, b_cur.x, acc, 0, 0, 0);
            acc = __builtin_amdgcn_mfma_f32_32x32x2f32(a_cur.y, b_cur.y, acc, 0, 0, 0);
            acc = __builtin_amdgcn_mfma_f32_32x32x2f32(a_cur.z, b_cur.z, acc, 0, 0, 0);
            acc = __builtin_amdgcn_mfma_f32_32x32x2f32(a_cur.w, b_cur.w, acc, 0, 0, 0);
            __builtin_amdgcn_sched_barrier(0);
            a_cur = a_nxt; b_cur = b_nxt;
        }
    }
    float* C = g.C + (long)b * g.sCb;
    const int n = n0 + wn * 32 + li;
    if (n < g.N) {
        const float bn = g.bias ? g.bias[n] : 0.f;
#pragma unroll
        for (int r = 0; r < 16; ++r) {
            const int m = m0 + wm * 32 + (r & 3) + 8 * (r >> 2) + 4 * lh;
            if (m < g.M) {
                float* p = C + (long)m * g.sCm + n;
                float v = g.alpha * acc[r] + bn;
                if (g.beta != 0.f) v += g.beta * *p;
                *p = v;
            }
        }
    }
}

template <int MAXV>
__global__ __launch_bounds__(256) void softmax_fwd_kernel(const float* __restrict__ x, float* __restrict__ y,
                                                          int rows, int cols) {
    const int row = blockIdx.x * 4 + (threadIdx.x >> 6);
    if (row >= rows) return;
    const int lane = threadIdx.x & 63;
    const float* xr = x + (size_t)row * cols;
    float v[MAXV];
    float mx = -INFINITY;
#pragma unroll
    for (int i = 0; i < MAXV; ++i) {
        const int c = lane + 64 * i;
        v[i] = c < cols ? xr[c] : -INFINITY;
        mx = fmaxf(mx, v[i]);
    }
    mx = wave_max(mx);
    float sum = 0.f;
#pragma unroll
    for (int i = 0; i < MAXV; ++i) {
        v[i] = expf(v[i] - mx);
        sum += v[i];
    }
    sum = wave_sum(sum);
    const float inv = 1.0f / sum;
    float* yr = y + (size_t)row * cols;
#pragma unroll
    for (int i = 0; i < MAXV; ++i) {
        const int c = lane + 64 * i;
        if (c < cols) yr[c] = v[i] * inv;
    }
}

template <int MAXV>
__global__ __launch_bounds__(256) void softmax_bwd_kernel(const float* __restrict__ y, const float* __restrict__ dy,
                                                          float* __restrict__ dx, int rows, int cols) {
    const int row = blockIdx.x * 4 + (threadIdx.x >> 6);
    if (row >= rows) return;
    const int lane = threadIdx.x & 63;
    const float* yr = y + (size_t)row * cols;
    const float* dr = dy + (size_t)row * cols;
    float yv[MAXV], dv[MAXV];
    float dot = 0.f;
#pragma unroll
    for (int i = 0; i < MAXV; ++i) {
        const int c = lane + 64 * i;
        yv[i] = c < cols ? yr[c] : 0.f;
        dv[i] = c < cols ? dr[c] : 0.f;
        dot += yv[i] * dv[i];
    }
    dot = wave_sum(dot);
    float* xr = dx + (size_t)row * cols;
#pragma unroll
    for (int i = 0; i < MAXV; ++i) {
        const int c = lane + 64 * i;
        if (c < cols) xr[c] = yv[i] * (dv[i] - dot);
    }
}

}

namespace {

struct TADesc {
    const float* w;
    const float* b;
    long long C, out_off, c_off;
};

struct TAGrad {
    float* dw;
    float* db;
};

__device__ __forceinline__ int ta_group(const TADesc* __restrict__ d, int ng, int cg) {
    int lo = 0, hi = ng;
    while (hi - lo > 1) {
        const int mid = (lo + hi) >> 1;
        if (d[mid].c_off <= cg) lo = mid; else hi = mid;
    }
    return lo;
}

__global__ __launch_bounds__(256) void time_affine_fwd_kernel(const TADesc* __restrict__ desc, int ng,
                                                              const float* __restrict__ emb, float* __restrict__ out,
                                                              int S, int K, int CT) {
    const int idx = blockIdx.x * 256 + threadIdx.x;
    if (idx >= CT * S) return;
    const int cg = idx % CT, s = idx / CT;
    const TADesc d = desc[ta_group(desc, ng, cg)];
    const int c = cg - (int)d.c_off;
    const float4* e4 = reinterpret_cast<const float4*>(emb + (size_t)s * K);
    const float4* w4 = reinterpret_cast<const float4*>(d.w + (size_t)c * K);
    float a0 = 0.f, a1 = 0.f;
    for (int k = 0; k < K / 4; k += 2) {
        const float4 e0 = e4[k], w0 = w4[k], e1 = e4[k + 1], w1 = w4[k + 1];
        a0 += (e0.x * w0.x + e0.y * w0.y) + (e0.z * w0.z + e0.w * w0.w);
        a1 += (e1.x * w1.x + e1.y * w1.y) + (e1.z * w1.z + e1.w * w1.w);
    }
    out[d.out_off + (size_t)s * d.C + c] = (a0 + a1) + (d.b ? d.b[c] : 0.f);
}

__global__ __launch_bounds__(256) void time_affine_bwd_w_kernel(const TADesc* __restrict__ desc, int ng,
                                                                const float* __restrict__ emb,
                                                                const float* __restrict__ de, float* __restrict__ dw,
                                                                float* __restrict__ db,
                                                                const TAGrad* __restrict__ gdst, int S, int K, int CT) {
    const int idx = blockIdx.x * 256 + threadIdx.x;
    if (idx >= CT * K) return;
    const int k = idx % K, cg = idx / K;
    const int gi = ta_group(desc, ng, cg);
    const TADesc d = desc[gi];
    const int c = cg - (int)d.c_off;
    if (gdst) {
        dw = gdst[gi].dw - (size_t)d.c_off * K;
        db = gdst[gi].db - d.c_off;
    }
    const float* g = de + d.out_off + c;
    float a[4] = {0.f, 0.f, 0.f, 0.f}, bsum[4] = {0.f, 0.f, 0.f, 0.f};
    int s = 0;
    for (; s + 3 < S; s += 4) {
#pragma unroll
        for (int j = 0; j < 4; ++j) {
            const float gv = g[(size_t)(s + j) * d.C];
            a[j] += gv * emb[(size_t)(s + j) * K + k];
            bsum[j] += gv;
        }
    }
    for (; s < S; ++s) {
        const float gv = g[(size_t)s * d.C];
        a[0] += gv * emb[(size_t)s * K + k];
        bsum[0] += gv;
    }
    dw[(size_t)cg * K + k] = (a[0] + a[1]) + (a[2] + a[3]);
    if (k == 0) db[cg] = (bsum[0] + bsum[1]) + (bsum[2] + bsum[3]);
}

constexpr int TA_NSPLIT = 16;

__global__ __launch_bounds__(256) void time_affine_bwd_x_kernel(const TADesc* __restrict__ desc, int ng,
                                                                const float* __restrict__ de,
                                                                float* __restrict__ partial, int S, int K) {
    __shared__ float part[256];
    const int s = blockIdx.x, sp = blockIdx.y, kk = threadIdx.x % K, p = threadIdx.x / K, np = 256 / K;
    float a0 = 0.f, a1 = 0.f;
    for (int g = 0; g < ng; ++g) {
        const TADesc d = desc[g];
        const float* gr = de + d.out_off + (size_t)s * d.C;
        const int step = np * TA_NSPLIT;
        int c = sp * np + p;
        for (; c + step < (int)d.C; c += 2 * step) {
            a0 += gr[c] * d.w[(size_t)c * K + kk];
            a1 += gr[c + step] * d.w[(size_t)(c + step) * K + kk];
        }
        if (c < (int)d.C) a0 += gr[c] * d.w[(size_t)c * K + kk];
    }
    part[threadIdx.x] = a0 + a1;
    __syncthreads();
    if (p == 0) {
        float t = 0.f;
        for (int q = 0; q < np; ++q) t += part[q * K + kk];
        partial[((size_t)sp * S + s) * K + kk] = t;
    }
}

__global__ __launch_bounds__(256) void time_affine_bwd_x_sum_kernel(const float* __restrict__ partial,
                                                                    float* __restrict__ demb, int n) {
    const int i = blockIdx.x * 256 + threadIdx.x;
    if (i >= n) return;
    float t[TA_NSPLIT];
#pragma unroll
    for (int q = 0; q < TA_NSPLIT; ++q) t[q] = partial[(size_t)q * n + i];
    float a = 0.f;
#pragma unroll
    for (int q = 0; q < TA_NSPLIT; ++q) a += t[q];
    demb[i] = a;
}

}

extern "C" {

int vf_bgemm(const float* A, const float* B, float* C, const float* bias, int batch, int M, int N, int K,
             long sAb, long sAm, long sAk, long sBb, long sBk, long sBn, long sCb, long sCm, long sCn,
             float alpha, float beta, void* stream) {
    if (batch <= 0 || M <= 0 || N <= 0) return 0;
    GemmArgs g;
    g.A = A; g.B = B; g.C = C; g.bias = bias; g.M = M; g.N = N; g.K = K;
    g.sAb = sAb; g.sAm = sAm; g.sAk = sAk; g.sBb = sBb; g.sBk = sBk; g.sBn = sBn;
    g.sCb = sCb; g.sCm = sCm; g.sCn = sCn; g.alpha = alpha; g.beta = beta;
    const dim3 grid((N + BN - 1) / BN, (M + BM - 1) / BM, batch);
    hipStream_t st = (hipStream_t)stream;
    static const bool xcd = !(getenv("VF_GEMM_XCD") && getenv("VF_GEMM_XCD")[0] == '0');
    g.xcd_batches = xcd ? batch / 8 : 0;
    auto mul4 = [](long v) { return (v & 3) == 0; };
    const bool a_kc = sAk == 1, a_mc = sAm == 1, b_kc = sBk == 1, b_nc = sBn == 1;
    const bool fast = (a_kc || a_mc) && (b_kc || b_nc) && sCn == 1 && mul4(K) && mul4(sAb) && mul4(sBb) &&
                      (a_kc ? mul4(sAm) : (mul4(sAk) && mul4(M))) && (b_kc ? mul4(sBn) : (mul4(sBk) && mul4(N))) &&
                      ((reinterpret_cast<size_t>(A) | reinterpret_cast<size_t>(B)) & 15) == 0;
    if (fast) {
        if (a_kc && b_kc) hipLaunchKernelGGL((bgemm_v2_kernel<true, true>), grid, dim3(256), 0, st, g);
        else if (a_kc) hipLaunchKernelGGL((bgemm_v2_kernel<true, false>), grid, dim3(256), 0, st, g);
        else if (b_kc) hipLaunchKernelGGL((bgemm_v2_kernel<false, true>), grid, dim3(256), 0, st, g);
        else hipLaunchKernelGGL((bgemm_v2_kernel<false, false>), grid, dim3(256), 0, st, g);
        VF_RETURN_LAST_ERROR();
    }
    hipLaunchKernelGGL(bgemm_kernel, grid, dim3(256), 0, st, g);
    VF_RETURN_LAST_ERROR();
}

int vf_softmax_fwd(const float* x, float* y, int rows, int cols, void* stream) {
    if (rows <= 0) return 0;
    hipStream_t st = (hipStream_t)stream;
    const dim3 grid((rows + 3) / 4), blk(256);
    if (cols <= 64) hipLaunchKernelGGL(softmax_fwd_kernel<1>, grid, blk, 0, st, x, y, rows, cols);
    else if (cols <= 256) hipLaunchKernelGGL(softmax_fwd_kernel<4>, grid, blk, 0, st, x, y, rows, cols);
    else if (cols <= 1024) hipLaunchKernelGGL(softmax_fwd_kernel<16>, grid, blk, 0, st, x, y, rows, cols);
    else if (cols <= 4096) hipLaunchKernelGGL(softmax_fwd_kernel<64>, grid, blk, 0, st, x, y, rows, cols);
    else return (int)hipErrorInvalidValue;
    VF_RETURN_LAST_ERROR();
}

int vf_softmax_bwd(const float* y, const float* dy, float* dx, int rows, int cols, void* stream) {
    if (rows <= 0) return 0;
    hipStream_t st = (hipStream_t)stream;
    const dim3 grid((rows + 3) / 4), blk(256);
    if (cols <= 64) hipLaunchKernelGGL(softmax_bwd_kernel<1>, grid, blk, 0, st, y, dy, dx, rows, cols);
    else if (cols <= 256) hipLaunchKernelGGL(softmax_bwd_kernel<4>, grid, blk, 0, st, y, dy, dx, rows, cols);
    else if (cols <= 1024) hipLaunchKernelGGL(softmax_bwd_kernel<16>, grid, blk, 0, st, y, dy, dx, rows, cols);
    else if (cols <= 4096) hipLaunchKernelGGL(softmax_bwd_kernel<64>, grid, blk, 0, st, y, dy, dx, rows, cols);
    else return (int)hipErrorInvalidValue;
    VF_RETURN_LAST_ERROR();
}


int vf_time_affine_fwd(const void* desc, int ngroups, const float* emb, float* out, int S, int K, int CT,
                       void* stream) {
    if (ngroups <= 0 || S <= 0) return 0;
    if (K % 8 != 0 || K > 256 || 256 % K != 0) return (int)hipErrorInvalidValue;
    hipLaunchKernelGGL(time_affine_fwd_kernel, dim3((CT * S + 255) / 256), dim3(256), 0, (hipStream_t)stream,
                       (const TADesc*)desc, ngroups, emb, out, S, K, CT);
    VF_RETURN_LAST_ERROR();
}

long vf_time_affine_ws_floats(int S, int K) { return (long)TA_NSPLIT * S * K; }

int vf_time_affine_bwd(const void* desc, int ngroups, const float* emb, const float* de, float* dw, float* db,
                       const void* gdst, float* demb, float* ws, int S, int K, int CT, void* stream) {
    if (ngroups <= 0 || S <= 0) return 0;
    if (K % 8 != 0 || K > 256 || 256 % K != 0) return (int)hipErrorInvalidValue;
    hipStream_t st = (hipStream_t)stream;
    hipLaunchKernelGGL(time_affine_bwd_w_kernel, dim3((CT * K + 255) / 256), dim3(256), 0, st, (const TADesc*)desc,
                       ngroups, emb, de, dw, db, (const TAGrad*)gdst, S, K, CT);
    if (demb) {
        if (!ws) return (int)hipErrorInvalidValue;
        hipLaunchKernelGGL(time_affine_bwd_x_kernel, dim3(S, TA_NSPLIT), dim3(256), 0, st, (const TADesc*)desc,
                           ngroups, de, ws, S, K);
        hipLaunchKernelGGL(time_affine_bwd_x_sum_kernel, dim3((S * K + 255) / 256), dim3(256), 0, st, ws, demb, S * K);
    }
    VF_RETURN_LAST_ERROR();
}

}
```

### view_fusion_amd/ops/__init__.py

```python
from .. import _lib, reducer
from .state import st
from . import state, core, deferred, policy, packing, bf16x3, norm, conv, dense, attention, diffusion, capture
from .core import (
    _CALL_KIND, _MODES, _WS_MAX, _c, _call, _check, _launch, _ptr, _raw_stream, _stream, _workspace
)
from .deferred import (
    _CS_RING, _colsum, _colsum_rows, _defer_begin, _defer_ok, _gout, _gslot, _rowsum_get, _rowsum_put, _wred_rows,
    _wred_ws, begin_capture, drop_deferred, end_capture, flush_deferred, wred_arena_bytes
)
from .capture import (
    prime_tables
)
from .policy import (
    _WINO_COST, _wino_cycles, _wino_kind, can_fold_residual, use_small_conv, use_winograd, use_winograd_wgrad,
    wino_kind
)
from .packing import (
    _WINO_ABI, _conv_ws, _packed, _packed_small, _packed_wino, _wino_ws, pack_all
)
from .bf16x3 import (
    _packed_b3, _use_b3
)
from .norm import (
    _GroupNormCatSkipFn, _GroupNormFn, _GroupNormSkipFn, _gn_backward, _gn_forward, cat_fusable, group_norm,
    group_norm_cat_skip, group_norm_skip
)
from .conv import (
    _Conv1x1CatFn, _Conv2dFn, _conv_small, _conv_small_res, conv1x1_cat, conv2d, conv2d_gn
)
from .dense import (
    _DropoutFn, _LinearFn, _SwishFn, _TimeAffineFn, _bgemm, _ta_desc, dropout, linear, sincos_embedding, swish,
    time_affine_all
)
from .attention import (
    _AttentionFn, _AttentionStreamFn, _ConcatFn, attention, attention_route, attention_streaming, concat_channels
)
from .diffusion import (
    _ComposeLossFn, _ComposeLossOptFn, compose, compose_loss, compose_mse_loss, draw_train, gather_level, p_sample_tail, philox_ids, psnr, randn_ids,
    sample_ids, sampler_step, ssim, stack_views, view_offsets, cond_drop_threshold, draw_cond_drop, guidance_scales,
    abs_quantile, quantile_position, threshold_scratch, threshold_settings,
    LevelSampler, check_level_sampler, draw_level, level_draw_host, level_stats, level_table_host,
    PREDICTIONS, _ComposeLossPredFn, check_prediction, loss_weights_pred_host,
    distill_begin, distill_step_host, distill_target
)
from .lpips import (
    LPIPS_TAPS, LPIPS_WIDTHS, lpips
)
```

### view_fusion_amd/ops/attention.py

```python
import math

import torch

from .state import st
from .core import _c, _call, _check, _launch, _ptr, _stream
from .dense import _bgemm




class _AttentionFn(torch.autograd.Function):

    @staticmethod
    def forward(ctx, qkv, need_p):
        _check(qkv)
        S, C3, H, W = qkv.shape
        C, L = C3 // 3, H * W
        alpha = 1.0 / math.sqrt(C)
        out = torch.empty(S, C, H, W, device=qkv.device, dtype=torch.float32)
        if L in (64, 256) and C % 32 == 0:
            P = torch.empty(S, L, L, device=qkv.device, dtype=torch.float32) if need_p else None
            _launch("attn_fwd", 4.0 * S * L * L * C, "vf_attention_fwd", _ptr(qkv), _ptr(out), _ptr(P), S, C, L, _stream(),
                    nbytes=4.0 * (qkv.numel() + out.numel() + (S * L * L if need_p else 0)))
        else:
            P = torch.empty(S, L, L, device=qkv.device, dtype=torch.float32)
            _bgemm(qkv, qkv, P, None, S, L, L, C, (C3 * L, 1, L), (C3 * L, L, 1), (L * L, L, 1), alpha,
                   offA=0, offB=C * L)
            _call("vf_softmax_fwd", _ptr(P), _ptr(P), S * L, L, _stream())
            _bgemm(qkv, P, out, None, S, C, L, L, (C3 * L, L, 1), (L * L, 1, L), (C * L, L, 1), offA=2 * C * L)
        ctx.save_for_backward(qkv, P)
        return out

    @staticmethod
    def backward(ctx, dO):
        qkv, P = ctx.saved_tensors
        dO = _c(dO)
        S, C3, H, W = qkv.shape
        C, L = C3 // 3, H * W
        alpha = 1.0 / math.sqrt(C)
        dqkv = torch.empty_like(qkv)
        dS = torch.empty_like(P)
        st._KIND_OVERRIDE = "attn_bwd" if st.KERNEL_LOG is not None else None
        fused_dq = False
        if L == 256 and C % 32 == 0 and st.ATTN_DSCORE:
            _call("vf_attention_dscore", _ptr(qkv), _ptr(dO), _ptr(P), _ptr(dS), _ptr(dqkv), S, C, L, _stream(),
                  flops=4.0 * S * L * L * C)
            fused_dq = True
        else:
            _bgemm(dO, qkv, dS, None, S, L, L, C, (C * L, 1, L), (C3 * L, L, 1), (L * L, L, 1), offB=2 * C * L)
            _call("vf_softmax_bwd", _ptr(P), _ptr(dS), _ptr(dS), S * L, L, _stream())
        if fused_dq and C % 64 == 0 and st.ATTN_DVDK:
            _call("vf_attention_dvdk", _ptr(qkv), _ptr(dO), _ptr(P), _ptr(dS), _ptr(dqkv), S, C, L, _stream(),
                  flops=4.0 * S * L * L * C)
            st._KIND_OVERRIDE = None
            return dqkv, None
        _bgemm(dO, P, dqkv, None, S, C, L, L, (C * L, L, 1), (L * L, L, 1), (C3 * L, L, 1), offC=2 * C * L)
        if not fused_dq:
            _bgemm(qkv, dS, dqkv, None, S, C, L, L, (C3 * L, L, 1), (L * L, 1, L), (C3 * L, L, 1), alpha,
                   offA=C * L, offC=0)
        _bgemm(qkv, dS, dqkv, None, S, C, L, L, (C3 * L, L, 1), (L * L, L, 1), (C3 * L, L, 1), alpha,
               offA=0, offC=C * L)
        st._KIND_OVERRIDE = None
        return dqkv, None


STREAM_MIN_L = 4097


def attention_route(C, L):
    if L >= STREAM_MIN_L:
        return "stream"
    if L in (64, 256) and C % 32 == 0:
        return "fused"
    return "generic"


class _AttentionStreamFn(torch.autograd.Function):

    @staticmethod
    def forward(ctx, qkv, need_stat):
        _check(qkv)
        S, C3, H, W = qkv.shape
        C, L = C3 // 3, H * W
        out = torch.empty(S, C, H, W, device=qkv.device, dtype=torch.float32)
        rowstat = torch.empty(S, 2, L, device=qkv.device, dtype=torch.float32) if need_stat else None
        _launch("attn_fwd", 4.0 * S * L * L * C, "vf_attn_stream_fwd", _ptr(qkv), _ptr(out), _ptr(rowstat), S, C, L,
                _stream(), nbytes=4.0 * (qkv.numel() + out.numel() + (2 * S * L if need_stat else 0)))
        ctx.save_for_backward(qkv, out, rowstat)
        return out

    @staticmethod
    def backward(ctx, dO):
        qkv, out, rowstat = ctx.saved_tensors
        dO = _c(dO)
        S, C3, H, W = qkv.shape
        C, L = C3 // 3, H * W
        dqkv = torch.empty_like(qkv)
        delta = torch.empty(S, L, device=qkv.device, dtype=torch.float32)
        _launch("attn_bwd", 14.0 * S * L * L * C, "vf_attn_stream_bwd", _ptr(qkv), _ptr(out), _ptr(dO), _ptr(rowstat),
                _ptr(delta), _ptr(dqkv), S, C, L, _stream(),
                nbytes=4.0 * (2 * qkv.numel() + 2 * out.numel() + 3 * S * L))
        return dqkv, None


def attention_streaming(qkv):
    return _AttentionStreamFn.apply(qkv, torch.is_grad_enabled() and qkv.requires_grad)


def attention(qkv):
    if attention_route(qkv.shape[1] // 3, qkv.shape[2] * qkv.shape[3]) == "stream":
        return attention_streaming(qkv)
    return _AttentionFn.apply(qkv, torch.is_grad_enabled() and qkv.requires_grad)


class _ConcatFn(torch.autograd.Function):
    @staticmethod
    def forward(ctx, a, b):
        _check(a, b)
        S, Ca, H, W = a.shape
        Cb = b.shape[1]
        out = torch.empty(S, Ca + Cb, H, W, device=a.device, dtype=torch.float32)
        _call("vf_concat_channels", _ptr(a), _ptr(b), _ptr(out), S, Ca * H * W, Cb * H * W, 0, _stream())
        ctx.shapes = (a.shape, b.shape)
        return out

    @staticmethod
    def backward(ctx, dout):
        dout = _c(dout)
        sa, sb = ctx.shapes
        da = torch.empty(sa, device=dout.device, dtype=torch.float32)
        db = torch.empty(sb, device=dout.device, dtype=torch.float32)
        _call("vf_concat_channels", _ptr(da), _ptr(db), _ptr(dout), sa[0], da[0].numel(), db[0].numel(), 1,
                  _stream())
        return da, db


def concat_channels(a, b):
    return _ConcatFn.apply(a, b)
```

### view_fusion_amd/ops/conv.py

```python
import ctypes

import torch

from .. import _lib, reducer
from .state import st
from .bf16x3 import _packed_b3, _use_b3
from .core import _MODES, _c, _call, _check, _launch, _ptr, _stream, _workspace
from .deferred import _defer_begin, _gout, _rowsum_get, _rowsum_put, _wred_ws
from .norm import group_norm
from .packing import _WINO_ABI, _conv_ws, _packed, _packed_small, _packed_wino, _wino_ws
from .policy import use_small_conv, use_winograd, use_winograd_wgrad, wino_kind


def _wgrad(entry, front, back, need, owners, keep, generic, flops, tag, strm):
    dev = keep[0].device
    ws = _wred_ws(dev, need) if (st.WRED_DEFER and (st.WRED_DEFER_GENERIC or not generic)
                                 and _defer_begin(owners, st.slab_sums)) else None
    if ws is None:
        ws = _workspace(dev, need)
        _launch("conv_wgrad", flops, entry, *front, _ptr(ws), ws.numel(), *back, strm, tag=tag)
        return False
    row, nblk = (ctypes.c_longlong * 9)(), ctypes.c_int(0)
    _launch("conv_wgrad", flops, entry + "_main", *front, _ptr(ws), ws.numel(), *back, ctypes.cast(row, ctypes.c_void_p),
            ctypes.cast(ctypes.pointer(nblk), ctypes.c_void_p), strm, tag=tag)
    st.slab_sums.add(dev, (list(row), nblk.value, (ws, *keep)))
    return True


def _conv_small(x, x2, weight, bias, view_bias, residual, S, Cin, Cout, H, W, KS, m):
    wd = weight.detach()
    _check(wd)
    y = torch.empty(S, Cout, H, W, device=x.device, dtype=torch.float32)
    wp = _packed_small(weight) if KS == 3 else None
    if wp is not None:
        _launch("conv_fwd", 2.0 * S * Cout * Cin * 9 * H * W, "vf_conv_small_gn", _ptr(x), None, 0, _ptr(wd), _ptr(bias),
                _ptr(view_bias), _ptr(residual), _ptr(y), S, Cin, Cout, H, W, 3, None, None, None, 0, 1e-5, 0, None, None,
                None, 0, 0, None, None, _ptr(wp), m, _stream(), tag=(Cin, Cout, H, KS, m))
        return y
    _launch("conv_fwd", 2.0 * S * Cout * Cin * KS * KS * H * W, "vf_conv_small", _ptr(x), _ptr(x2),
            x.shape[1] if x2 is not None else 0, _ptr(wd), _ptr(bias), _ptr(view_bias), _ptr(residual), _ptr(y), S, Cin,
            Cout, H, W, KS, m, _stream(), tag=(Cin, Cout, H, KS, m))
    return y


def _conv_small_res(x, layer, view_bias, res_layer, rx, rx2):
    S, Cin, H, W = x.shape
    Cout = layer.weight.shape[0]
    rC = res_layer.weight.shape[1]
    rC1 = rx.shape[1]
    assert rC1 + (rx2.shape[1] if rx2 is not None else 0) == rC and res_layer.weight.shape[0] == Cout
    wd, rwd = layer.weight.detach(), res_layer.weight.detach()
    _check(x, wd, rwd, layer.bias, view_bias, rx, rx2, res_layer.bias)
    y = torch.empty(S, Cout, H, W, device=x.device, dtype=torch.float32)
    wp = _packed_small(layer)
    if wp is not None:
        _launch("conv_fwd", 2.0 * S * Cout * (Cin * 9 + rC) * H * W, "vf_conv_small_gn", _ptr(x), None, 0, _ptr(wd),
                _ptr(layer.bias), _ptr(view_bias), None, _ptr(y), S, Cin, Cout, H, W, 3, None, None, None, 0, 1e-5, 0, None,
                _ptr(rx), _ptr(rx2), rC1, rC, _ptr(rwd), _ptr(res_layer.bias), _ptr(wp), 0, _stream(), tag=(Cin, Cout, H, 3, 0))
        return y
    _launch("conv_fwd", 2.0 * S * Cout * (Cin * 9 + rC) * H * W, "vf_conv_small_res", _ptr(x), _ptr(wd), _ptr(layer.bias),
            _ptr(view_bias), _ptr(y), S, Cin, Cout, H, W, _ptr(rx), _ptr(rx2), rC1, rC, _ptr(rwd), _ptr(res_layer.bias),
            _stream(), tag=(Cin, Cout, H, 3, 0))
    return y


class _Conv2dFn(torch.autograd.Function):

    @staticmethod
    def forward(ctx, x, weight, bias, view_bias, residual, layer, mode, training, twin, tap=False):
        _check(x, bias, view_bias, residual)
        ctx.tap = tap
        if tap:
            ctx.set_materialize_grads(False)
        S, Cin, Hi, Wi = x.shape
        Cout, _, KS, _ = weight.shape
        m = _MODES[mode]
        if m == 1 and (Hi % 2 or Wi % 2):
            raise ValueError(f"stride-2 conv on a {Hi}x{Wi} map: both sides must be even")
        H, W = (Hi // 2, Wi // 2) if m == 1 else ((Hi * 2, Wi * 2) if m == 2 else (Hi, Wi))
        y = torch.empty(S, Cout, H, W, device=x.device, dtype=torch.float32)
        flops = 2.0 * S * Cout * Cin * KS * KS * H * W
        nb = 4.0 * (x.numel() + y.numel() + weight.numel() + (residual.numel() if residual is not None else 0))
        wino = wino_kind(S, Cin, Cout, H, W, KS, m, train=bool(training))
        ctx.b3 = _use_b3(KS, m, H * W)
        if ctx.b3:
            wf, wb = _packed_b3(layer, force=training)
            _launch("conv_fwd", flops, "vf_conv1x1_bf16x3", _ptr(x), None, 0, ctypes.c_void_p(wf.data_ptr()), _ptr(bias),
                    _ptr(view_bias), _ptr(residual), _ptr(y), None, 0, S, Cin, Cout, H * W, _stream(),
                    tag=(Cin, Cout, H, KS, m))
        elif wino:
            wf, wb = _packed_wino(layer, training, wino)
            ws, nws = _wino_ws(x.device, S, Cin, Cout, H, W, wino)
            _launch("conv_fwd", flops, _WINO_ABI[wino][3], _ptr(x), _ptr(wf), _ptr(bias), _ptr(view_bias),
                    _ptr(residual), _ptr(y), _ptr(ws), nws, S, Cin, Cout, H, W, m, _stream(),
                    tag=(Cin, Cout, H, KS, m), nbytes=nb)
        else:
            wf, wb = _packed(layer, force=training)
            ws, nws = _conv_ws(x.device, S, Cin, Cout, H, W, KS)
            _launch("conv_fwd", flops, "vf_conv_fwd", _ptr(x), _ptr(wf), _ptr(bias), _ptr(view_bias),
                    _ptr(residual), _ptr(y), _ptr(ws), nws, S, Cin, Cout, H, W, KS, m, _stream(),
                    tag=(Cin, Cout, H, KS, m))
        ctx.flops, ctx.tag = flops, (Cin, Cout, H, KS, m)
        ctx.save_for_backward(x)
        ctx.wino = wino
        ctx.wb, ctx.m, ctx.KS, ctx.Cout = wb, m, KS, Cout
        ctx.has = (bias is not None, view_bias is not None, residual is not None)
        ctx.pw, ctx.pb, ctx.twin = weight, bias, (twin.bias if twin is not None else None)
        return (y, x.view_as(x)) if tap else y

    @staticmethod
    def backward(ctx, dy, dtap=None):
        (x,) = ctx.saved_tensors
        dy = _c(dy)
        dtap = _c(dtap) if dtap is not None else None
        S, Cin, Hi, Wi = x.shape
        _, Cout, H, W = dy.shape
        KS, m = ctx.KS, ctx.m
        strm = _stream()
        dx = dw = db = dvb = dres = None
        if ctx.needs_input_grad[0] and ctx.wino:
            dfull = torch.empty(S, Cin, H, W, device=x.device, dtype=torch.float32)
            ws, nws = _wino_ws(x.device, S, Cout, Cin, H, W, ctx.wino)
            _launch("conv_dgrad", ctx.flops, _WINO_ABI[ctx.wino][3], _ptr(dy), _ptr(ctx.wb), None, None, None,
                    _ptr(dfull), _ptr(ws), nws, S, Cout, Cin, H, W, 0, strm, tag=ctx.tag,
                    nbytes=4.0 * (dy.numel() + dfull.numel() + ctx.pw.numel()))
            if m == 2:
                dx = torch.empty_like(x)
                _call("vf_sumpool2", _ptr(dfull), _ptr(dx), dx.numel(), Wi, strm)
            else:
                dx = dfull
        elif ctx.needs_input_grad[0] and ctx.b3:
            dx = torch.empty_like(x)
            _launch("conv_dgrad", ctx.flops, "vf_conv1x1_bf16x3", _ptr(dy), None, 0, ctypes.c_void_p(ctx.wb.data_ptr()), None,
                    None, None, _ptr(dx), None, 0, S, Cout, Cin, H * W, strm, tag=ctx.tag)
        elif ctx.needs_input_grad[0]:
            if m == 0:
                dx = torch.empty_like(x)
                ws, nws = _conv_ws(x.device, S, Cout, Cin, H, W, KS)
                _launch("conv_dgrad", ctx.flops, "vf_conv_fwd", _ptr(dy), _ptr(ctx.wb), None, None, None, _ptr(dx),
                        _ptr(ws), nws, S, Cout, Cin, H, W, KS, 0, strm, tag=ctx.tag)
            elif m == 1:
                dx = torch.empty_like(x)
                _launch("conv_dgrad", ctx.flops, "vf_conv_fwd", _ptr(dy), _ptr(ctx.wb), None, None, _ptr(dtap), _ptr(dx),
                        None, 0, S, Cout, Cin, H, W, KS, 4, strm, tag=ctx.tag)
                dtap = None
            else:
                dup = torch.empty(S, Cin, H, W, device=x.device, dtype=torch.float32)
                _launch("conv_dgrad", ctx.flops, "vf_conv_fwd", _ptr(dy), _ptr(ctx.wb), None, None, None, _ptr(dup),
                        None, 0, S, Cout, Cin, H, W, KS, 0, strm, tag=ctx.tag)
                dx = torch.empty_like(x)
                _call("vf_sumpool2", _ptr(dup), _ptr(dx), dx.numel(), Wi, strm)
        hb, hv, hr = ctx.has
        want_b, want_v = hb and ctx.needs_input_grad[2], hv and ctx.needs_input_grad[3]
        arena = reducer.ACTIVE is not None
        hit = _rowsum_get(dy) if (want_b or want_v) else None
        if hit is not None:
            dvb, db = hit[1], (hit[2].view_as(hit[2]) if hit[2] is not None else None)
        db2 = None
        if ctx.needs_input_grad[1] and use_winograd_wgrad(S, Cin, Cout, H, W, KS, m):
            need = _lib.load().vf_wino_wgrad_ws_floats(S, Cin, Cout, H, W)
            dw = _gout(ctx.pw, Cout, Cin, 3, 3, like=x)
            db_here = None
            if want_b and db is None:
                db = db_here = _gout(ctx.pb, Cout, like=x)
                if hr:
                    db2 = _gout(ctx.twin, Cout, like=x)
            owners = [ctx.pw] + ([ctx.pb] if db_here is not None else []) + \
                     ([ctx.twin] if (db2 is not None and ctx.twin is not None) else [])
            if _wgrad("vf_wino_wgrad", (_ptr(x), _ptr(dy), _ptr(dw), _ptr(db_here), _ptr(db2)), (S, Cin, Cout, H, W, m),
                      need, owners, (dw, db_here, db2), False, ctx.flops, ctx.tag, strm):
                dw = dw.view_as(dw)
                if db_here is not None:
                    db = db_here.view_as(db_here)
        elif ctx.needs_input_grad[1]:
            need = _lib.load().vf_conv_wgrad_ws_floats(S, Cin, Cout, H, W, KS)
            dw = _gout(ctx.pw, Cout, Cin, KS, KS, like=x)
            if _wgrad("vf_conv_wgrad", (_ptr(x), _ptr(dy), _ptr(dw)), (S, Cin, Cout, H, W, KS, m), need, [ctx.pw],
                      (dw, None, None), True, ctx.flops, ctx.tag, strm):
                dw = dw.view_as(dw)
        if want_b or want_v:
            if (want_v and dvb is None) or (want_b and db is None and dvb is None):
                if Cout >= 192:
                    db_new = _gout(ctx.pb, Cout, like=x) if (want_b and db is None) else None
                    dvb = torch.empty(S, Cout, device=x.device, dtype=torch.float32) if want_v else None
                    _call("vf_bias_grad", _ptr(dy), _ptr(db_new), _ptr(dvb), S, Cout, H * W, strm)
                    db = db_new if db_new is not None else db
                else:
                    dvb = torch.empty(S, Cout, device=x.device, dtype=torch.float32)
                    _call("vf_rowsum", _ptr(dy), _ptr(dvb), S * Cout, H * W, strm)
            if want_b and db is None:
                db = _gout(ctx.pb, Cout, like=x)
                _call("vf_colsum", _ptr(dvb), _ptr(db), 1, S, Cout, strm)
            if hr and want_b:
                _rowsum_put(dy, dvb, db2 if (db2 is not None or arena) else db)
            if not want_b:
                db = None
            if not want_v:
                dvb = None
        if hr and ctx.needs_input_grad[4]:
            dres = dy
        if dtap is not None:
            dx = dtap if dx is None else dx + dtap
        return dx, dw, db, dvb, dres, None, None, None, None, None


class _Conv1x1CatFn(torch.autograd.Function):

    @staticmethod
    def forward(ctx, x1, x2, weight, bias, layer, training):
        _check(x1, x2, bias)
        S, C1, H, W = x1.shape
        Cout, Cin = weight.shape[0], weight.shape[1]
        y = torch.empty(S, Cout, H, W, device=x1.device, dtype=torch.float32)
        ctx.b3 = _use_b3(1, 0, H * W)
        if ctx.b3:
            wf, wb = _packed_b3(layer, force=training)
            _launch("conv_fwd", 2.0 * S * Cout * Cin * H * W, "vf_conv1x1_bf16x3", _ptr(x1), _ptr(x2), C1,
                    ctypes.c_void_p(wf.data_ptr()), _ptr(bias), None, None, _ptr(y), None, 0, S, Cin, Cout, H * W, _stream(),
                    tag=(Cin, Cout, H, 1, 0))
        else:
            wf, wb = _packed(layer, force=training)
            ws, nws = _conv_ws(x1.device, S, Cin, Cout, H, W, 1)
            _launch("conv_fwd", 2.0 * S * Cout * Cin * H * W, "vf_conv1x1_cat_fwd", _ptr(x1), _ptr(x2), C1, _ptr(wf),
                    _ptr(bias), _ptr(y), _ptr(ws), nws, S, Cin, Cout, H, W, _stream(), tag=(Cin, Cout, H, 1, 0))
        ctx.save_for_backward(x1, x2)
        ctx.wb, ctx.dims, ctx.has_bias = wb, (Cin, Cout), bias is not None
        ctx.pw, ctx.pb = weight, bias
        return y

    @staticmethod
    def backward(ctx, dy):
        x1, x2 = ctx.saved_tensors
        dy = _c(dy)
        S, C1, H, W = x1.shape
        Cin, Cout = ctx.dims
        strm = _stream()
        flops, tag = 2.0 * S * Cout * Cin * H * W, (Cin, Cout, H, 1, 0)
        dx1 = dx2 = dw = db = None
        if ctx.needs_input_grad[0] or ctx.needs_input_grad[1]:
            dx1, dx2 = torch.empty_like(x1), torch.empty_like(x2)
            if ctx.b3:
                _launch("conv_dgrad", flops, "vf_conv1x1_bf16x3", _ptr(dy), None, 0, ctypes.c_void_p(ctx.wb.data_ptr()), None,
                        None, None, _ptr(dx1), _ptr(dx2), C1, S, Cout, Cin, H * W, strm, tag=tag)
            else:
                _launch("conv_dgrad", flops, "vf_conv1x1_cat_dgrad", _ptr(dy), _ptr(ctx.wb), _ptr(dx1), _ptr(dx2), C1, S,
                        Cin, Cout, H, W, strm, tag=tag)
        if ctx.needs_input_grad[2]:
            need = _lib.load().vf_conv_wgrad_ws_floats(S, Cin, Cout, H, W, 1)
            dw = _gout(ctx.pw, Cout, Cin, 1, 1, like=x1)
            if _wgrad("vf_conv1x1_cat_wgrad", (_ptr(x1), _ptr(x2), C1, _ptr(dy), _ptr(dw)), (S, Cin, Cout, H, W), need,
                      [ctx.pw], (dw, None, None), True, flops, tag, strm):
                dw = dw.view_as(dw)
        if ctx.has_bias and ctx.needs_input_grad[3]:
            hit = _rowsum_get(dy)
            db = hit[2].view_as(hit[2]) if (hit is not None and hit[2] is not None) else None
            if db is None:
                dvb = hit[1] if hit is not None else None
                if dvb is None:
                    dvb = torch.empty(S, Cout, device=x1.device, dtype=torch.float32)
                    _call("vf_rowsum", _ptr(dy), _ptr(dvb), S * Cout, H * W, strm)
                db = _gout(ctx.pb, Cout, like=x1)
                _call("vf_colsum", _ptr(dvb), _ptr(db), 1, S, Cout, strm)
        return dx1, dx2, dw, db, None, None


def conv1x1_cat(x1, x2, layer):
    if not torch.is_grad_enabled():
        S, C1, H, W = x1.shape
        Cout, Cin = layer.weight.shape[0], layer.weight.shape[1]
        if use_small_conv(S, Cin, Cout, H, W, 1, 0):
            _check(x1, x2, layer.bias)
            return _conv_small(x1, x2, layer.weight, layer.bias, None, None, S, Cin, Cout, H, W, 1, 0)
    training = torch.is_grad_enabled() and layer.weight.requires_grad
    return _Conv1x1CatFn.apply(x1, x2, layer.weight, layer.bias, layer, training)


def conv2d(x, layer, view_bias=None, residual=None, mode="same", twin=None, tap=False, res_fold=None):
    if not torch.is_grad_enabled():
        S, Cin, Hi, Wi = x.shape
        Cout, _, KS, _ = layer.weight.shape
        m = _MODES[mode]
        H, W = (Hi // 2, Wi // 2) if m == 1 else ((Hi * 2, Wi * 2) if m == 2 else (Hi, Wi))
        if res_fold is not None:
            assert residual is None and not tap
            return _conv_small_res(x, layer, view_bias, *res_fold)
        if use_small_conv(S, Cin, Cout, H, W, KS, m):
            _check(x, layer.bias, view_bias, residual)
            y = _conv_small(x, None, layer.weight, layer.bias, view_bias, residual, S, Cin, Cout, H, W, KS, m)
            return (y, x) if tap else y
    assert res_fold is None
    training = torch.is_grad_enabled() and layer.weight.requires_grad
    if tap and torch.is_grad_enabled():
        return _Conv2dFn.apply(x, layer.weight, layer.bias, view_bias, residual, layer, mode, training, twin, True)
    y = _Conv2dFn.apply(x, layer.weight, layer.bias, view_bias, residual, layer, mode, training, twin)
    return (y, x) if tap else y


def conv2d_gn(x, layer, gn, groups, silu, view_bias=None, residual=None, mode="same", want_y=False, res_fold=None):
    S, Cin, Hi, Wi = x.shape
    Cout, _, KS, _ = layer.weight.shape
    m = _MODES[mode]
    H, W = (Hi // 2, Wi // 2) if m == 1 else ((Hi * 2, Wi * 2) if m == 2 else (Hi, Wi))
    lib = _lib.load()
    fused = (not torch.is_grad_enabled() and not use_winograd(S, Cin, Cout, H, W, KS, m, False) and not _use_b3(KS, m, H * W)
             and not use_small_conv(S, Cin, Cout, H, W, KS, m)
             and lib.vf_conv_fwd_ws_floats(S, Cin, Cout, H, W, KS) > 0)
    if (st.WINO_GN_FUSION and not fused and not torch.is_grad_enabled() and res_fold is None
            and m in (0, 2) and KS == 3 and wino_kind(S, Cin, Cout, H, W, KS, m, False) == 1
            and lib.vf_wino_conv_gn_fusable(S, Cin, Cout, H, W, m, groups)):
        _check(x, layer.bias, view_bias, residual, gn.weight, gn.bias)
        y = torch.empty(S, Cout, H, W, device=x.device, dtype=torch.float32) if want_y else None
        a = torch.empty(S, Cout, H, W, device=x.device, dtype=torch.float32)
        wf, _ = _packed_wino(layer, False, 1)
        ws, nws = _wino_ws(x.device, S, Cin, Cout, H, W, 1)
        _launch("conv_fwd", 2.0 * S * Cout * Cin * 9 * H * W, "vf_wino_conv_fwd_gn", _ptr(x), _ptr(wf), _ptr(layer.bias),
                _ptr(view_bias), _ptr(residual), _ptr(y), int(want_y), _ptr(gn.weight), _ptr(gn.bias), _ptr(a), groups, 1e-5,
                int(silu), _ptr(ws), nws, S, Cin, Cout, H, W, m, _stream(), tag=(Cin, Cout, H, KS, m))
        return y, a
    if not fused:
        y = conv2d(x, layer, view_bias=view_bias, residual=residual, mode=mode, res_fold=res_fold)
        return y, group_norm(y, gn.weight, gn.bias, groups, silu)
    assert res_fold is None
    _check(x, layer.bias, view_bias, residual, gn.weight, gn.bias)
    y = torch.empty(S, Cout, H, W, device=x.device, dtype=torch.float32)
    a = torch.empty_like(y)
    stats = torch.empty(2 * S * groups, device=x.device, dtype=torch.float32)
    wf, _ = _packed(layer, force=False)
    ws, nws = _conv_ws(x.device, S, Cin, Cout, H, W, KS)
    _call("vf_conv_fwd_gn", _ptr(x), _ptr(wf), _ptr(layer.bias), _ptr(view_bias), _ptr(residual), _ptr(y), int(want_y),
              _ptr(gn.weight), _ptr(gn.bias), _ptr(a), _ptr(stats), groups, 1e-5, int(silu), _ptr(ws), nws, S, Cin, Cout,
              H, W, KS, m, _stream())
    return (y if want_y else None), a
```

### view_fusion_amd/ops/core.py

```python
import ctypes

import torch

from .. import _lib
from .state import st


_MODES = {"same": 0, "down2": 1, "up2": 2}


def _ptr(t, offset_elems=0):
    if t is None:
        return None
    return ctypes.c_void_p(t.data_ptr() + 4 * offset_elems)


def _raw_stream():
    return torch._C._cuda_getCurrentRawStream(torch._C._cuda_getDevice())


def _stream():
    return ctypes.c_void_p(_raw_stream())


def _check(*tensors):
    for t in tensors:
        if t is None:
            continue
        if not t.is_cuda:
            raise _lib.VFHipError("view_fusion_amd ops need CUDA/HIP tensors (no CPU fallback)")
        if t.dtype != torch.float32 or not t.is_contiguous():
            raise _lib.VFHipError(f"expected contiguous float32, got {t.dtype} contiguous={t.is_contiguous()}")


def _c(t):
    return t if t.is_contiguous() else t.contiguous()




def _launch(kind, flops, name, *args, tag=None, nbytes=0.0):
    if st.KERNEL_LOG is None:
        _lib.call(name, *args)
        return
    e0, e1 = torch.cuda.Event(enable_timing=True), torch.cuda.Event(enable_timing=True)
    e0.record()
    _lib.call(name, *args)
    e1.record()
    st.KERNEL_LOG.append((kind, flops, e0, e1, tag, name, nbytes))


_CALL_KIND = {"vf_wino44_pack_weights": "pack", "vf_wino44_pack_weights_multi": "pack", "vf_bgemm": "bgemm", "vf_softmax_bwd": "attn_bwd", "vf_softmax_fwd": "attn_fwd",
              "vf_attn_stream_fwd": "attn_fwd", "vf_attn_stream_bwd": "attn_bwd",
              "vf_colsum": "reduce", "vf_colsum_multi": "reduce", "vf_rowsum": "reduce", "vf_bias_grad": "reduce",
              "vf_sumpool2": "reduce", "vf_conv_pack_weights": "pack", "vf_wino_pack_weights": "pack",
              "vf_conv_pack_weights_multi": "pack", "vf_wino_pack_weights_multi": "pack",
              "vf_time_affine_fwd": "embed", "vf_time_affine_bwd": "embed", "vf_sincos_embed": "embed",
              "vf_swish_fwd": "embed", "vf_swish_bwd": "embed",
              "vf_stack_views": "diffusion", "vf_compose_fwd": "diffusion", "vf_compose_mse_bwd": "diffusion",
              "vf_compose_loss_fwd": "diffusion", "vf_compose_loss_bwd": "diffusion",
              "vf_compose_loss_pred_fwd": "diffusion", "vf_compose_loss_pred_bwd": "diffusion",
              "vf_compose_loss_fwd_scaled": "diffusion", "vf_draw_level": "diffusion", "vf_level_stats": "diffusion",
              "vf_gather_level": "diffusion", "vf_p_sample_tail": "diffusion",
              "vf_draw_train": "diffusion", "vf_randn_ids": "diffusion", "vf_philox_ids": "diffusion",
              "vf_p_sample_tail_rng": "diffusion", "vf_sampler_step": "diffusion", "vf_sampler_step_rng": "diffusion",
              "vf_stack_views_cfg": "diffusion", "vf_draw_cond_drop": "diffusion", "vf_p_sample_tail_cfg": "diffusion",
              "vf_p_sample_tail_cfg_rng": "diffusion", "vf_sampler_step_cfg": "diffusion",
              "vf_sampler_step_cfg_rng": "diffusion",
              "vf_compose_eps": "diffusion", "vf_sample_stat": "diffusion", "vf_abs_quantile": "diffusion",
              "vf_p_sample_tail_eps": "diffusion", "vf_p_sample_tail_eps_rng": "diffusion",
              "vf_sampler_step_eps": "diffusion", "vf_sampler_step_eps_rng": "diffusion",
              "vf_distill_begin": "diffusion", "vf_distill_target": "diffusion",
              "vf_grad_sumsq_multi": "adam", "vf_grad_norm_finish": "adam", "vf_adam_multi_ex": "adam",
              "vf_adam_multi_ex_dev": "adam", "vf_adam_set_scalars_ex": "adam", "vf_swap_multi": "adam", "vf_grad_accum_multi": "adam"}


def _call(name, *args, flops=0.0, nbytes=0.0):
    if st.KERNEL_LOG is None:
        _lib.call(name, *args)
        return
    _launch(st._KIND_OVERRIDE or _CALL_KIND.get(name, "misc"), flops, name, *args, nbytes=nbytes)


_WS_MAX = 4


def _workspace(device, nfloats):
    key = (device, _raw_stream())
    buf = st._ws.pop(key, None)
    if buf is None or buf.numel() < nfloats:
        new = torch.empty(int(nfloats), device=device, dtype=torch.float32)
        if torch.cuda.is_current_stream_capturing():
            if buf is not None:
                st._ws[key] = buf
            return new
        buf = new
    st._ws[key] = buf
    while len(st._ws) > _WS_MAX:
        st._ws.pop(next(iter(st._ws)))
    return buf
```

### view_fusion_amd/ops/deferred.py

```python
import ctypes
import functools

import torch

from .. import _lib, reducer
from .state import st
from .core import _call, _launch, _ptr, _stream




def _rowsum_put(t, rowsum, colsum):
    if st.ROWSUM_FUSION:
        t._vf_sums = (t._version, rowsum, colsum)


def _rowsum_get(t):
    h = getattr(t, "_vf_sums", None) if st.ROWSUM_FUSION else None
    if h is None or h[0] != t._version:
        return None
    return h


def _gslot(p):
    a = reducer.ACTIVE
    return a.slot(p) if (a is not None and p is not None) else None


def _gout(p, *shape, like):
    t = _gslot(p)
    return t if t is not None else torch.empty(*shape, device=like.device, dtype=torch.float32)




class _Arena:

    def __init__(self):
        self.buf, self.used = None, 0


def _wred_ws(device, need):
    a = st._WRED_ARENA.setdefault(device, _Arena())
    n = (int(need) + 63) // 64 * 64
    cap = 0 if a.buf is None else a.buf.numel()
    if a.used + n > cap:
        if torch.cuda.is_current_stream_capturing():
            return None
        a.buf = torch.empty(max(2 * cap, a.used + n, 1 << 24), device=device, dtype=torch.float32)
        a.used = 0
    ws = a.buf[a.used:a.used + n]
    a.used += n
    return ws


def wred_arena_bytes(device=None):
    return sum(4 * a.buf.numel() for d, a in st._WRED_ARENA.items() if a.buf is not None and (device is None or d == device))


_CS_RING = 16




class _CaptureTable:
    def __init__(self, table):
        self.table = table
        self.used = 0
        self.rows = []
        self.keep = []


class _Slot:

    def __init__(self):
        self.pinned = self.table = self.key = None
        self.event = torch.cuda.Event()
        self.rows = self.workgroups = 0


class _Deferred:

    def __init__(self, width, launch, rows_of, key_of, full):
        self.width, self.launch, self.rows_of, self.key_of, self.full = width, launch, rows_of, key_of, full
        self.pending = []
        self.device = None
        self.capture = None
        self.rings = {}
        self.keep = None

    def add(self, device, entry):
        self.pending.append(entry)
        self.device = device

    def begin_capture(self, device, max_rows):
        self.capture = _CaptureTable(torch.empty(max(1, max_rows), self.width, dtype=torch.int64, device=device))

    def end_capture(self):
        ct, self.capture = self.capture, None
        if ct is not None and ct.used:
            ct.table[:ct.used].copy_(torch.tensor(ct.rows, dtype=torch.int64))
        return ct

    def flush(self):
        pend, self.pending = self.pending, []
        if not pend:
            return
        if torch.cuda.is_current_stream_capturing():
            ct = self.capture
            rows, total = self.rows_of(pend)
            if ct is None or ct.used + len(rows) > ct.table.shape[0]:
                raise _lib.VFHipError(self.full)
            self.launch(ctypes.c_void_p(ct.table.data_ptr() + 8 * self.width * ct.used), len(rows), total, _stream())
            ct.used += len(rows)
            ct.rows += rows
            ct.keep.append(pend)
            return
        key = self.key_of(pend)
        ring = self.rings.setdefault(self.device, [])
        slot = next((s for s in ring if s.key == key), None)
        if slot is None:
            rows, total = self.rows_of(pend)
            if len(ring) < _CS_RING:
                slot = _Slot()
            else:
                slot = ring.pop(0)
                slot.event.synchronize()
            ring.append(slot)
            if slot.pinned is None or slot.pinned.shape[0] < len(rows):
                n = max(128, len(rows))
                slot.pinned = torch.empty(n, self.width, dtype=torch.int64).pin_memory()
                slot.table = torch.empty(n, self.width, dtype=torch.int64, device=self.device)
            slot.pinned[:len(rows)].copy_(torch.tensor(rows, dtype=torch.int64))
            slot.table[:len(rows)].copy_(slot.pinned[:len(rows)], non_blocking=True)
            slot.event.record()
            slot.key, slot.rows, slot.workgroups = key, len(rows), total
        self.launch(ctypes.c_void_p(slot.table.data_ptr()), slot.rows, slot.workgroups, _stream())
        self.keep = pend


def _wred_rows(pend):
    rows, first = [], 0
    for row, nblk, _ in pend:
        r = list(row)
        r[8] = (r[8] & ~0xFFFFFFFF) | first
        rows.append(r)
        first += nblk
    return rows, first


def _colsum_rows(pend):
    rows, first = [], 0
    for parts, dgb, batch, S, C in pend:
        rows.append([parts.data_ptr(), dgb.data_ptr(), S, C, batch, first])
        first += ((C + 63) // 64) * batch
    return rows, first


st.slab_sums = _Deferred(
    9, functools.partial(_launch, "conv_wgrad", 0.0, "vf_wino44_reduce_multi"), _wred_rows,
    lambda pend: tuple(v for row, _, _ in pend for v in row),
    "deferred weight-gradient slab sums inside a stream capture need ops.begin_capture() "
    "with max_conv_rows >= the number of 3x3 layers (one backward pass per capture)")
st.col_sums = _Deferred(
    6, functools.partial(_call, "vf_colsum_multi"), _colsum_rows,
    lambda pend: tuple(v for parts, dgb, _, S, C in pend for v in (parts.data_ptr(), dgb.data_ptr(), S, C)),
    "deferred GroupNorm parameter sums inside a stream capture need ops.begin_capture() "
    "with room for every GroupNorm layer (one backward pass per capture)")


def begin_capture(device, max_rows, max_conv_rows=0):
    st.col_sums.begin_capture(device, max_rows)
    if max_conv_rows:
        st.slab_sums.begin_capture(device, max_conv_rows)
    else:
        st.slab_sums.capture = None


def end_capture():
    drop_deferred()
    return st.col_sums.end_capture(), st.slab_sums.end_capture()


def _flush():
    st.slab_sums.flush()
    for a in st._WRED_ARENA.values():
        a.used = 0
    st._PENDING_TASK = None
    st.col_sums.flush()


def _defer_ok(params):
    a = reducer.ACTIVE
    flushes = a is not None and getattr(a, "flushes_colsums", False)
    for p in params:
        if p is None or p.grad is not None or getattr(p, "_vf_no_defer", False):
            return False
        if getattr(p, "_backward_hooks", None) and not (flushes and id(p) in a._alias):
            return False
        if a is None and getattr(p, "_post_accumulate_grad_hooks", None):
            return False
    return a is None or flushes


def _colsum(parts, dgb, batch, S, C, params):
    if _defer_begin(params, st.col_sums):
        st.col_sums.add(parts.device, (parts, dgb, batch, S, C))
        return
    _call("vf_colsum", _ptr(parts), _ptr(dgb), batch, S, C, _stream())


def _defer_begin(params, family):
    task = torch._C._current_graph_task_id()
    if not (st.COLSUM_DEFER and task != -1 and _defer_ok(params)
            and (family.capture is not None or not torch.cuda.is_current_stream_capturing())):
        return False
    if (st.col_sums.pending or st.slab_sums.pending) and st._PENDING_TASK != task:
        if torch.cuda.is_current_stream_capturing():
            st.col_sums.pending.clear()
            st.slab_sums.pending.clear()
        else:
            _flush()
    if not st.col_sums.pending and not st.slab_sums.pending:
        st._PENDING_TASK = task
        torch.autograd.Variable._execution_engine.queue_callback(_flush)
    return True


def flush_deferred():
    if st.col_sums.pending or st.slab_sums.pending:
        _flush()


def drop_deferred():
    st.col_sums.pending.clear()
    st.slab_sums.pending.clear()
    st._PENDING_TASK = None
    for a in st._WRED_ARENA.values():
        a.used = 0
```

### view_fusion_amd/ops/packing.py

```python
import ctypes

import torch

from .. import _lib
from .state import st
from .core import _MODES, _call, _check, _ptr, _stream, _workspace
from .policy import _WINO_ABI, wino_kind


def _conv_ws(device, S, Cin, Cout, H, W, KS):
    need = _lib.load().vf_conv_fwd_ws_floats(S, Cin, Cout, H, W, KS)
    if need <= 0:
        return None, 0
    ws = _workspace(device, need)
    return ws, ws.numel()


def _wino_ws(device, S, Cin, Cout, H, W, kind=1):
    need = getattr(_lib.load(), _WINO_ABI[kind][4])(S, Cin, Cout, H, W)
    if need <= 0:
        return None, 0
    ws = _workspace(device, need)
    return ws, ws.numel()


def _packed(layer, force):
    w = layer.weight
    cache = getattr(layer, "_vf_pack", None)
    key = (w._version, w.data_ptr(), w.device)
    if not force and cache is not None and cache[0] == key:
        return cache[1], cache[2]
    if force and cache is not None and getattr(layer, "_vf_pack_fresh", False):
        object.__setattr__(layer, "_vf_pack_fresh", False)
        return cache[1], cache[2]
    Cout, Cin, KS, _ = w.shape
    nf, nb = ctypes.c_long(), ctypes.c_long()
    _lib.call("vf_conv_pack_sizes", Cout, Cin, KS, ctypes.byref(nf), ctypes.byref(nb))
    if cache is not None and cache[1].numel() == nf.value and cache[1].device == w.device:
        wf, wb = cache[1], cache[2]
    else:
        wf = torch.empty(nf.value, device=w.device, dtype=torch.float32)
        wb = torch.empty(nb.value, device=w.device, dtype=torch.float32)
    wd = w.detach()
    _check(wd)
    _call("vf_conv_pack_weights", _ptr(wd), _ptr(wf), _ptr(wb), Cout, Cin, KS, _stream())
    object.__setattr__(layer, "_vf_pack", (None if force else key, wf, wb))
    return wf, wb




def _packed_wino(layer, force, kind=1):
    attr, f_sizes, f_pack = _WINO_ABI[kind][:3]
    w = layer.weight
    cache = getattr(layer, attr, None)
    key = (w._version, w.data_ptr(), w.device)
    if not force and cache is not None and cache[0] == key:
        return cache[1], cache[2]
    if force and cache is not None and getattr(layer, attr + "_fresh", False):
        object.__setattr__(layer, attr + "_fresh", False)
        return cache[1], cache[2]
    Cout, Cin = w.shape[0], w.shape[1]
    nf, nb = ctypes.c_long(), ctypes.c_long()
    _lib.call(f_sizes, Cout, Cin, ctypes.byref(nf), ctypes.byref(nb))
    if cache is not None and cache[1].numel() == nf.value and cache[1].device == w.device:
        uf, ub = cache[1], cache[2]
    else:
        uf = torch.empty(nf.value, device=w.device, dtype=torch.float32)
        ub = torch.empty(nb.value, device=w.device, dtype=torch.float32)
    wd = w.detach()
    _check(wd)
    _call(f_pack, _ptr(wd), _ptr(uf), _ptr(ub), Cout, Cin, _stream())
    object.__setattr__(layer, attr, (None if force else key, uf, ub))
    return uf, ub


def pack_all(root, S=None, hw=None):
    plan = getattr(root, "_vf_pack_plan", None)
    layers = plan[0] if plan is not None else [m for m in root.modules() if isinstance(m, torch.nn.Conv2d)]
    if not layers:
        return
    _check(layers[0].weight.detach())

    if hw is None:
        size = getattr(root, "_vf_image_size", None)
        hw = (size, size) if size is not None else None

    def kind_of(l):
        geom = getattr(l, "_vf_geom", None)
        if geom is None or S is None or hw is None:
            return 0
        H, W = hw[0] >> geom[0], hw[1] >> geom[0]
        return wino_kind(S, l.weight.shape[1], l.weight.shape[0], H, W, l.weight.shape[2], _MODES[geom[1]], train=True)

    kinds = tuple((l.weight.data_ptr(), kind_of(l)) for l in layers)
    key = (hw, kinds)
    if plan is None or plan[1] != key:
        dev = layers[0].weight.device
        rows, first = {0: [], 1: [], 2: []}, {0: 0, 1: 0, 2: 0}
        for l, (_, kind) in zip(layers, kinds):
            w = l.weight
            Cout, Cin, KS, _ = w.shape
            nf, nb = ctypes.c_long(), ctypes.c_long()
            if kind:
                _lib.call(_WINO_ABI[kind][1], Cout, Cin, ctypes.byref(nf), ctypes.byref(nb))
            else:
                _lib.call("vf_conv_pack_sizes", Cout, Cin, KS, ctypes.byref(nf), ctypes.byref(nb))
            pf = torch.empty(nf.value, device=dev, dtype=torch.float32)
            pb = torch.empty(nb.value, device=dev, dtype=torch.float32)
            nblk = (nf.value + nb.value + 255) // 256
            if kind:
                object.__setattr__(l, _WINO_ABI[kind][0], (None, pf, pb))
                rows[kind].append([w.data_ptr(), pf.data_ptr(), pb.data_ptr(), Cout, Cin, nf.value, nb.value, first[kind]])
            else:
                object.__setattr__(l, "_vf_pack", (None, pf, pb))
                rows[0].append([w.data_ptr(), pf.data_ptr(), pb.data_ptr(), Cout, Cin, KS, nf.value, nb.value, first[0]])
            first[kind] += nblk
        descs = tuple((torch.tensor(rows[k], dtype=torch.int64).to(dev) if rows[k] else None, len(rows[k]), first[k])
                      for k in (0, 1, 2))
        plan = (layers, key, descs)
        object.__setattr__(root, "_vf_pack_plan", plan)
    for k, fn in ((0, "vf_conv_pack_weights_multi"), (1, "vf_wino_pack_weights_multi"), (2, "vf_wino44_pack_weights_multi")):
        desc, n, blk = plan[2][k]
        if n:
            _call(fn, ctypes.c_void_p(desc.data_ptr()), n, blk, _stream())
    attrs = ("_vf_pack", "_vf_wpack", "_vf_w4pack")
    for l, (_, kind) in zip(layers, plan[1][1]):
        for k, attr in enumerate(attrs):
            c = getattr(l, attr, None)
            if c is not None and c[0] is not None:
                object.__setattr__(l, attr, (None, c[1], c[2]))
        object.__setattr__(l, attrs[kind] + "_fresh", True)
        c = getattr(l.weight, "_vf_small_pack", None)
        if c is not None and c[0] is not None:
            l.weight._vf_small_pack = (None, c[1])




def _packed_small(layer_or_weight):
    w = layer_or_weight.weight if hasattr(layer_or_weight, "weight") else layer_or_weight
    if not st.SMALL_PACK or w.shape[2] != 3 or torch.is_grad_enabled():
        return None
    key = (w._version, w.data_ptr(), w.device)
    cache = getattr(w, "_vf_small_pack", None)
    if cache is not None and cache[0] == key:
        return cache[1]
    Cout, Cin = w.shape[0], w.shape[1]
    n = _lib.load().vf_conv_small_pack_floats(Cout, Cin)
    wp = cache[1] if (cache is not None and cache[1].numel() == n and cache[1].device == w.device) else \
        torch.empty(n, device=w.device, dtype=torch.float32)
    wd = w.detach()
    _check(wd)
    _call("vf_conv_small_pack", _ptr(wd), _ptr(wp), Cout, Cin, _stream())
    try:
        w._vf_small_pack = (key, wp)
    except AttributeError:
        pass
    return wp
```

### view_fusion_amd/ops/state.py

```python
import os


class State:
    def __init__(self):
        self.KERNEL_LOG = None
        self._KIND_OVERRIDE = None
        self.WINOGRAD = True
        self.FORCE_WINOGRAD = False
        self.WINO_MIN_TILES = int(os.environ.get("VF_WINO_MIN_TILES", 30))
        self.WINO_MIN_FILL = int(os.environ.get("VF_WINO_MIN_FILL", 65))
        self.WINO_WGRAD_MIN_TILES = int(os.environ.get("VF_WINO_WGRAD_MIN_TILES", 256))
        self.WINOGRAD_WGRAD = True
        self.WINOGRAD44 = os.environ.get("VF_WINO44", "1") == "1"
        self.FORCE_WINOGRAD44 = False
        self.SMALL_CONV = os.environ.get("VF_SMALL_CONV", "1") == "1"
        self.SMALL_CONV_MAX_WGS = (int(os.environ.get("VF_SMALL_CONV_MAX_WGS1", 1024)),
                          int(os.environ.get("VF_SMALL_CONV_MAX_WGS3", 512)))
        self.SMALL_CONV_MAX_CIN3 = int(os.environ.get("VF_SMALL_CONV_MAX_CIN3", 256))
        self.SMALL_CONV_MAX_S3 = int(os.environ.get("VF_SMALL_CONV_MAX_S3", 1))
        self.SMALL_PACK = os.environ.get("VF_SMALL_PACK", "1") == "1"
        self.RES_FOLD = os.environ.get("VF_RES_FOLD", "1") == "1"
        self.WINO_GN_FUSION = os.environ.get("VF_WINO_GN", "1") == "1"
        self.ATTN_DSCORE = os.environ.get("VF_ATTN_DSCORE", "1") != "0"
        self.ATTN_DVDK = os.environ.get("VF_ATTN_DVDK", "1") != "0"
        self.BF16X3 = os.environ.get("VF_BF16X3") == "1"
        self.ROWSUM_FUSION = True
        self.COLSUM_DEFER = True
        self.WRED_DEFER = os.environ.get("VF_WRED_DEFER", "1") != "0"
        self.WRED_DEFER_GENERIC = os.environ.get("VF_WRED_DEFER_GENERIC", "1") != "0"
        self.col_sums = None
        self.slab_sums = None
        self._PENDING_TASK = None
        self._WRED_ARENA = {}
        self._ws = {}
        self._WINO_KIND_CACHE = {}
        self._TA_DESC = {}
        self._TA_GDST = {}
        self._SSIM_WINDOW = {}
        self._RNG_IDS = {}
        self._VC_CACHE = []


st = State()
```

### view_fusion_amd/unet.py

```python
import torch
from torch import nn


class _Named(nn.Module):

    def __init__(self, **children):
        super().__init__()
        for name, mod in children.items():
            self.add_module(name, mod)

    def __getitem__(self, name):
        return self._modules[name]


def _norm_act_conv(cin, cout, groups):
    return _Named(block=_Named(**{"0": nn.GroupNorm(groups, cin), "3": nn.Conv2d(cin, cout, 3, padding=1)}))


class _ResBlock(nn.Module):
    def __init__(self, cin, cout, emb_dim, groups, dropout=0):
        super().__init__()
        self.noise_func = _Named(noise_func=_Named(**{"0": nn.Linear(emb_dim, cout)}))
        self.block1 = _norm_act_conv(cin, cout, groups)
        self.block2 = _norm_act_conv(cout, cout, groups)
        self.res_conv = nn.Conv2d(cin, cout, 1) if cin != cout else nn.Identity()
        self.groups = groups
        self.dropout = float(dropout)

    def _drop(self, a, draws):
        if self.dropout == 0 or not self.training:
            return a
        from . import ops
        return ops.dropout(a, self.dropout, next(draws) if draws is not None else None)

    def _forward_inference(self, x, e, skip, a_in, next_gn):
        from . import ops
        b1, b2 = self.block1["block"], self.block2["block"]
        conv1, conv2 = b1["3"], b2["3"]
        S, _, H, W = x.shape
        Cout = conv2.weight.shape[0]
        if skip is not None:
            C1, C = x.shape[1], x.shape[1] + skip.shape[1]
            if not (isinstance(self.res_conv, nn.Conv2d) and ops.cat_fusable(C1, C, x.shape[2] * x.shape[3], self.groups)):
                x, skip = ops.concat_channels(x, skip), None
        fold = (self.res_conv, x, skip) if ops.can_fold_residual(S, Cout, H, W, self.res_conv) else None
        res = None
        if skip is not None:
            if fold is None:
                res = ops.conv1x1_cat(x, skip, self.res_conv)
            a, _, _ = ops.group_norm_cat_skip(x, skip, b1["0"].weight, b1["0"].bias, self.groups, silu=True)
        else:
            if isinstance(self.res_conv, nn.Identity):
                res = x
            elif fold is None:
                res = ops.conv2d(x, self.res_conv)
            a = a_in if a_in is not None else ops.group_norm(x, b1["0"].weight, b1["0"].bias, self.groups, silu=True)
        _, a2 = ops.conv2d_gn(a, conv1, b2["0"], self.groups, True, view_bias=e)
        if next_gn is None:
            return ops.conv2d(a2, conv2, residual=res, res_fold=fold), None
        return ops.conv2d_gn(a2, conv2, next_gn[0], self.groups, next_gn[1], residual=res, want_y=True, res_fold=fold)

    def forward(self, x, e, skip=None, tap=False, draws=None):
        from . import ops
        b1, b2 = self.block1["block"], self.block2["block"]
        if skip is not None:
            C1, C = x.shape[1], x.shape[1] + skip.shape[1]
            if not (isinstance(self.res_conv, nn.Conv2d) and ops.cat_fusable(C1, C, x.shape[2] * x.shape[3], self.groups)):
                x, skip = ops.concat_channels(x, skip), None
        if skip is not None:
            a, x1, x2 = ops.group_norm_cat_skip(x, skip, b1["0"].weight, b1["0"].bias, self.groups, silu=True)
            h = ops.conv2d(a, b1["3"], view_bias=e)
            a = self._drop(ops.group_norm(h, b2["0"].weight, b2["0"].bias, self.groups, silu=True), draws)
            return ops.conv2d(a, b2["3"], residual=ops.conv1x1_cat(x1, x2, self.res_conv), twin=self.res_conv)
        a, xs, xt = ops.group_norm_skip(x, b1["0"].weight, b1["0"].bias, self.groups, silu=True, tap=True)
        h = ops.conv2d(a, b1["3"], view_bias=e)
        a = self._drop(ops.group_norm(h, b2["0"].weight, b2["0"].bias, self.groups, silu=True), draws)
        twin = None if isinstance(self.res_conv, nn.Identity) else self.res_conv
        skip = xs if twin is None else ops.conv2d(xs, twin)
        y = ops.conv2d(a, b2["3"], residual=skip, twin=twin)
        return (y, xt) if tap else y


class _SelfAttention(nn.Module):
    def __init__(self, ch, groups):
        super().__init__()
        self.norm = nn.GroupNorm(groups, ch)
        self.qkv = nn.Conv2d(ch, ch * 3, 1, bias=False)
        self.out = nn.Conv2d(ch, ch, 1)
        self.groups = groups

    def forward(self, x, n=None):
        from . import ops
        if n is None:
            n, xs = ops.group_norm_skip(x, self.norm.weight, self.norm.bias, self.groups, silu=False)
        else:
            xs = x
        qkv = ops.conv2d(n, self.qkv)
        o = ops.attention(qkv)
        return ops.conv2d(o, self.out, residual=xs)


class _ResAttnBlock(nn.Module):
    def __init__(self, cin, cout, emb_dim, groups, with_attn, dropout=0):
        super().__init__()
        self.with_attn = with_attn
        self.res_block = _ResBlock(cin, cout, emb_dim, groups, dropout)
        if with_attn:
            self.attn = _SelfAttention(cout, groups)

    def forward_inference(self, x, e, skip=None, a_in=None, next_gn=None):
        if self.with_attn:
            y, n = self.res_block._forward_inference(x, e, skip, a_in, (self.attn.norm, False))
            return self.attn(y, n), None
        return self.res_block._forward_inference(x, e, skip, a_in, next_gn)

    def forward(self, x, e, skip=None, tap=False, draws=None):
        xt = None
        if tap:
            x, xt = self.res_block(x, e, skip, tap=True, draws=draws)
        else:
            x = self.res_block(x, e, skip, draws=draws)
        x = self.attn(x) if self.with_attn else x
        return (x, xt) if tap else x


class _Resample(nn.Module):
    def __init__(self, ch, up):
        super().__init__()
        self.up = up
        self.conv = nn.Conv2d(ch, ch, 3, padding=1) if up else nn.Conv2d(ch, ch, 3, 2, 1)

    def forward(self, x, tap=False):
        from . import ops
        return ops.conv2d(x, self.conv, mode="up2" if self.up else "down2", tap=tap)


class UNet(nn.Module):
    def __init__(self, in_channel=6, out_channel=3, inner_channel=32, norm_groups=32,
                 channel_mults=(1, 2, 4, 8, 8), attn_res=(8,), res_blocks=3, dropout=0,
                 with_noise_level_emb=True, image_size=128):
        super().__init__()
        if not with_noise_level_emb:
            raise TypeError("with_noise_level_emb=False: the reference UNet cannot be constructed without the "
                            "noise-level embedding (nn.Linear(None, C) in FeatureWiseAffine, model/unet.py:165)")
        if not 0 <= dropout < 1:
            raise ValueError(f"dropout probability has to be in [0, 1), got {dropout}")
        self.inner_channel = inner_channel
        self.noise_level_mlp = _Named(**{"0": nn.Linear(inner_channel, inner_channel * 4),
                                         "2": nn.Linear(inner_channel * 4, inner_channel)})
        emb = inner_channel
        ch = inner_channel
        skips = [ch]
        res = image_size
        downs = [nn.Conv2d(in_channel, inner_channel, 3, padding=1)]
        last = len(channel_mults) - 1
        for lvl, mult in enumerate(channel_mults):
            width = inner_channel * mult
            for _ in range(res_blocks):
                downs.append(_ResAttnBlock(ch, width, emb, norm_groups, res in attn_res, dropout))
                ch = width
                skips.append(ch)
            if lvl != last:
                downs.append(_Resample(ch, up=False))
                skips.append(ch)
                res //= 2
        self.downs = nn.ModuleList(downs)
        self.mid = nn.ModuleList([_ResAttnBlock(ch, ch, emb, norm_groups, True, dropout),
                                  _ResAttnBlock(ch, ch, emb, norm_groups, False, dropout)])
        ups = []
        for lvl in reversed(range(len(channel_mults))):
            width = inner_channel * channel_mults[lvl]
            for _ in range(res_blocks + 1):
                ups.append(_ResAttnBlock(ch + skips.pop(), width, emb, norm_groups, res in attn_res, dropout))
                ch = width
            if lvl > 0:
                ups.append(_Resample(ch, up=True))
                res *= 2
        self.ups = nn.ModuleList(ups)
        self.final_conv = _norm_act_conv(ch, out_channel if out_channel is not None else in_channel,
                                         norm_groups)
        self.norm_groups = norm_groups
        self._annotate_geometry(image_size)

    def _annotate_geometry(self, image_size):
        attn_levels = set()

        def mark(conv, lvl, mode="same"):
            object.__setattr__(conv, "_vf_geom", (lvl, mode))

        def mark_block(blk, lvl):
            rb = blk.res_block
            mark(rb.block1["block"]["3"], lvl)
            mark(rb.block2["block"]["3"], lvl)
            if isinstance(rb.res_conv, nn.Conv2d):
                mark(rb.res_conv, lvl)
            if blk.with_attn:
                attn_levels.add(lvl)
                mark(blk.attn.qkv, lvl)
                mark(blk.attn.out, lvl)

        lvl = 0
        for layer in self.downs:
            if isinstance(layer, _ResAttnBlock):
                mark_block(layer, lvl)
            elif isinstance(layer, _Resample):
                lvl += 1
                mark(layer.conv, lvl, "down2")
            else:
                mark(layer, lvl)
        for layer in self.mid:
            mark_block(layer, lvl)
        for layer in self.ups:
            if isinstance(layer, _ResAttnBlock):
                mark_block(layer, lvl)
            else:
                lvl -= 1
                mark(layer.conv, lvl, "up2")
        mark(self.final_conv["block"]["3"], lvl)
        object.__setattr__(self, "_vf_image_size", image_size)
        object.__setattr__(self, "_vf_depth", sum(isinstance(m, _Resample) and not m.up for m in self.downs))
        object.__setattr__(self, "_vf_attn_levels", tuple(sorted(attn_levels)))

    def check_input_size(self, H, W):
        f = 1 << self._vf_depth
        if H <= 0 or W <= 0 or H % f or W % f:
            raise ValueError(f"input size {H}x{W}: both sides must be positive multiples of {f} "
                             f"(2**(len(channel_mults) - 1)) for the encoder / decoder maps to match")
        if (H * W) % 4:
            raise ValueError(f"input size {H}x{W}: H*W must be a multiple of 4")

    def _affine_layers(self):
        lst = getattr(self, "_vf_affine", None)
        if lst is None:
            lst = [m.res_block.noise_func["noise_func"]["0"] for m in list(self.downs) + list(self.mid) + list(self.ups)
                   if isinstance(m, _ResAttnBlock)]
            object.__setattr__(self, "_vf_affine", lst)
        return lst

    def _has_dropout(self):
        return any(isinstance(m, _ResBlock) and m.dropout > 0 for m in self.modules())

    def _forward_inference(self, x, es):
        from . import ops

        def gn1_of(layer):
            if not isinstance(layer, _ResAttnBlock):
                return None
            return (layer.res_block.block1["block"]["0"], True)

        feats, a_next = [], None
        downs = list(self.downs)
        for i, layer in enumerate(downs):
            if isinstance(layer, _ResAttnBlock):
                nxt = downs[i + 1] if i + 1 < len(downs) else self.mid[0]
                x, a_next = layer.forward_inference(x, next(es), a_in=a_next, next_gn=gn1_of(nxt))
            elif isinstance(layer, _Resample):
                x, a_next = layer(x), None
            else:
                x, a_next = ops.conv2d(x, layer), None
            feats.append(x)
        x, a_next = self.mid[0].forward_inference(x, next(es), a_in=a_next, next_gn=gn1_of(self.mid[1]))
        x, a_next = self.mid[1].forward_inference(x, next(es), a_in=a_next, next_gn=None)
        ups = list(self.ups)
        fc = self.final_conv["block"]
        for i, layer in enumerate(ups):
            if isinstance(layer, _ResAttnBlock):
                last = i + 1 == len(ups)
                x, a_next = layer.forward_inference(x, next(es), skip=feats.pop(), next_gn=(fc["0"], True) if last else None)
            else:
                x, a_next = layer(x), None
        a = a_next if a_next is not None else ops.group_norm(x, fc["0"].weight, fc["0"].bias, self.norm_groups, silu=True)
        return ops.conv2d(a, fc["3"])

    def forward(self, x, angle, time, dropout_u=None):
        from . import ops
        draws = iter(dropout_u) if dropout_u is not None else None
        ops._check(x)
        self.check_input_size(x.shape[2], x.shape[3])
        if torch.is_grad_enabled() and self.final_conv["block"]["3"].weight.requires_grad:
            ops.pack_all(self, x.shape[0], tuple(x.shape[2:]))
        mlp = self.noise_level_mlp
        inference = not torch.is_grad_enabled() and not (self.training and self._has_dropout())

        def embed():
            pe = ops.sincos_embedding(time, angle, self.inner_channel)
            emb = ops.linear(pe, mlp["0"].weight, mlp["0"].bias)
            emb = ops.linear(ops.swish(emb), mlp["2"].weight, mlp["2"].bias)
            return ops.time_affine_all(emb, self._affine_layers())

        if inference:
            return self._forward_inference(x, iter(embed()))
        es = iter(embed())

        feats = []
        for layer in self.downs:
            if isinstance(layer, _ResAttnBlock):
                x, xin = layer(x, next(es), tap=True, draws=draws)
                if feats:
                    feats[-1] = xin
            elif isinstance(layer, _Resample):
                x, xin = layer(x, tap=True)
                if feats:
                    feats[-1] = xin
            else:
                x = ops.conv2d(x, layer)
            feats.append(x)
        first = True
        for layer in self.mid:
            if first:
                x, feats[-1] = layer(x, next(es), tap=True, draws=draws)
                first = False
            else:
                x = layer(x, next(es), draws=draws)
        for layer in self.ups:
            if isinstance(layer, _ResAttnBlock):
                x = layer(x, next(es), feats.pop(), draws=draws)
            else:
                x = layer(x)
        fc = self.final_conv["block"]
        a = ops.group_norm(x, fc["0"].weight, fc["0"].bias, self.norm_groups, silu=True)
        return ops.conv2d(a, fc["3"])
```

Baseline: 3230 view denoise-steps/s (UNet fwd+bwd per stacked view, incl. compose/MSE/Adam).

## Fold attention output projection into V weights and fuse bias/residual epilogue

```diff
diff --git a/include/vf_hip.h b/include/vf_hip.h
--- a/include/vf_hip.h
+++ b/include/vf_hip.h
@@ -116,6 +116,13 @@
              int K, long sAb, long sAm, long sAk, long sBb, long sBk, long sBn, long sCb, long sCm, long sCn,
              float alpha, float beta, void* stream);
 int vf_attention_fwd(const float* qkv, float* out, float* P , int S, int C, int L, void* stream);
+int vf_attention_fwd_epi(const float* qkv, float* out, float* P , const float* bias ,
+                         const float* residual , int S, int C, int L, void* stream);
+long vf_attn_fold_blocks(int C);
+int vf_attn_fold(const float* w_qkv, const float* w_out, float* w_fold, int C, void* stream);
+int vf_attn_fold_multi(const void* desc, int nlayers, long total_blocks, void* stream);
+int vf_attn_fold_bwd(const float* dw_fold, const float* w_qkv, const float* w_out, float* dw_qkv, float* dw_out, int C,
+                     void* stream);
 int vf_attention_fwd_kernel(int S, int C, int L);
 int vf_attention_dscore(const float* qkv, const float* dO, const float* P, float* dS, float* dqkv, int S, int C, int L,
                         void* stream);
diff --git a/view_fusion_amd/_lib.py b/view_fusion_amd/_lib.py
--- a/view_fusion_amd/_lib.py
+++ b/view_fusion_amd/_lib.py
@@ -68,7 +68,12 @@
     "vf_time_affine_bwd": [_P, _I, _P, _P, _P, _P, _P, _P, _P, _I, _I, _I, _P],
     "vf_bgemm": [_P, _P, _P, _P, _I, _I, _I, _I, _L, _L, _L, _L, _L, _L, _L, _L, _L, _F, _F, _P],
     "vf_attention_fwd": [_P, _P, _P, _I, _I, _I, _P],
+    "vf_attention_fwd_epi": [_P, _P, _P, _P, _P, _I, _I, _I, _P],
     "vf_attention_fwd_kernel": [_I, _I, _I],
+    "vf_attn_fold_blocks": [_I],
+    "vf_attn_fold": [_P, _P, _P, _I, _P],
+    "vf_attn_fold_multi": [_P, _I, _L, _P],
+    "vf_attn_fold_bwd": [_P, _P, _P, _P, _P, _I, _P],
     "vf_attention_dscore": [_P, _P, _P, _P, _P, _I, _I, _I, _P],
     "vf_attention_dvdk": [_P, _P, _P, _P, _P, _I, _I, _I, _P],
     "vf_attn_stream_fwd": [_P, _P, _P, _I, _I, _I, _P],
@@ -164,7 +169,7 @@
     "vf_batch_host_plan": [_U64, _P, _I, _I, _I, _I, _L, _P, _P, _P, _P, _P, _P, _P],
 }
 _RESTYPE = {"vf_conv1x1_bf16x3_pack_dwords": _L, "vf_conv_wgrad_ws_floats": _L, "vf_time_affine_ws_floats": _L, "vf_wino_conv_ws_floats": _L, "vf_wino44_conv_ws_floats": _L, "vf_wino_wgrad_ws_floats": _L, "vf_conv_fwd_ws_floats": _L,
-            "vf_conv_small_pack_floats": _L, "vf_ssim_workspace_floats": _L, "vf_lpips_workspace_floats": _L}
+            "vf_conv_small_pack_floats": _L, "vf_attn_fold_blocks": _L, "vf_ssim_workspace_floats": _L, "vf_lpips_workspace_floats": _L}
 
 _lib = None
 N_CALLS = 0
diff --git a/view_fusion_amd/csrc/attention.hip b/view_fusion_amd/csrc/attention.hip
--- a/view_fusion_amd/csrc/attention.hip
+++ b/view_fusion_amd/csrc/attention.hip
@@ -2,8 +2,16 @@
 
 namespace {
 
+__device__ __forceinline__ float attn_epi(const float* __restrict__ bias, const float* __restrict__ res, int c, size_t i) {
+    float v = 0.f;
+    if (bias) v = bias[c];
+    if (res) v += res[i];
+    return v;
+}
+
 __global__ __launch_bounds__(512) void attn_fwd_kh_kernel(const float* __restrict__ qkv, float* __restrict__ out,
-                                                          float* __restrict__ P, int C, float alpha) {
+                                                          float* __restrict__ P, int C, float alpha,
+                                                          const float* __restrict__ bias, const float* __restrict__ res) {
     constexpr int L = 256, NTH = 512, QW = 128, NKT = 4, CKA = 16, RSV = L + 4;
     constexpr int KS = L + 32;
     constexpr int KQ = CKA * KS + CKA * QW, VT = 32 * RSV;
@@ -134,10 +142,16 @@
     f32x16 oprev = {0};
     for (int c0 = 0, cur = 0; c0 < C; c0 += 32, cur ^= 1) {
         if (kh == 0 && c0 > 0) {
+            float ad[16];
 #pragma unroll
             for (int r = 0; r < 16; ++r) {
                 const int c = c0 - 32 + (r & 3) + 8 * (r >> 2) + 4 * lh;
-                out[((size_t)b * C + c) * L + qi] = oprev[r] + oex[cur ^ 1][qb][r][lane];
+                ad[r] = attn_epi(bias, res, c, ((size_t)b * C + c) * L + qi);
+            }
+#pragma unroll
+            for (int r = 0; r < 16; ++r) {
+                const int c = c0 - 32 + (r & 3) + 8 * (r >> 2) + 4 * lh;
+                out[((size_t)b * C + c) * L + qi] = (oprev[r] + oex[cur ^ 1][qb][r][lane]) + ad[r];
             }
         }
         VF_AK_STOREV(cur ^ 1);
@@ -170,10 +184,16 @@
     }
     if (kh == 0) {
         const int last = (C / 32 - 1) & 1;
+        float ad[16];
 #pragma unroll
         for (int r = 0; r < 16; ++r) {
             const int c = C - 32 + (r & 3) + 8 * (r >> 2) + 4 * lh;
-            out[((size_t)b * C + c) * L + qi] = oprev[r] + oex[last][qb][r][lane];
+            ad[r] = attn_epi(bias, res, c, ((size_t)b * C + c) * L + qi);
+        }
+#pragma unroll
+        for (int r = 0; r < 16; ++r) {
+            const int c = C - 32 + (r & 3) + 8 * (r >> 2) + 4 * lh;
+            out[((size_t)b * C + c) * L + qi] = (oprev[r] + oex[last][qb][r][lane]) + ad[r];
         }
     }
 #undef VF_AK_LOADV
@@ -192,7 +212,8 @@
 template <bool DSCORE>
 __global__ __launch_bounds__(256, 3) void attn_fwd_q32_kernel(const float* __restrict__ qkv, float* __restrict__ out,
                                                               float* __restrict__ P, int C, float alpha, int S,
-                                                              const float* __restrict__ dO, float* __restrict__ dS) {
+                                                              const float* __restrict__ dO, float* __restrict__ dS,
+                                                              const float* __restrict__ bias, const float* __restrict__ res) {
     constexpr int L = 256, NTH = 256, NKT = 2, CKA = 16;
     constexpr int KS = L + 32;
     constexpr int KQ = CKA * KS + CKA * 32;
@@ -294,6 +315,14 @@
     VF_A3_LOADV(vb, 1);
 
     const int qi = q0 + li;
+    float ad[4] = {0.f, 0.f, 0.f, 0.f}, adn[4] = {0.f, 0.f, 0.f, 0.f};
+    if constexpr (!DSCORE) {
+#pragma unroll
+        for (int r = 0; r < 4; ++r) {
+            const int c = 8 * w + 4 * lh + r;
+            ad[r] = attn_epi(bias, res, c, ((size_t)b * C + c) * L + qi);
+        }
+    }
     if constexpr (DSCORE) {
         const size_t prow = ((size_t)b * L + qi) * L + w * (NKT * 32) + 4 * lh;
         float4 pv[NKT][4];
@@ -391,6 +420,15 @@
         } }
     for (int ct = 0; ct < npiece / 2; ++ct) {
         f32x16 o = {0};
+        if constexpr (!DSCORE) {
+            if (ct + 1 < npiece / 2) {
+#pragma unroll
+                for (int r = 0; r < 4; ++r) {
+                    const int c = (ct + 1) * 32 + 8 * w + 4 * lh + r;
+                    adn[r] = attn_epi(bias, res, c, ((size_t)b * C + c) * L + qi);
+                }
+            }
+        }
         VF_A3_PV(0)
         VF_A3_STOREV(vb);
         VF_A3_LOADV(vb, min(2 * ct + 3, npiece - 1));
@@ -406,8 +444,10 @@
         for (int r = 0; r < 4; ++r) {
             const float* x_ = ox + (4 * w + r) * 64 + lane;
             const float v_ = (x_[0] + x_[16 * 64]) + (x_[32 * 64] + x_[48 * 64]);
-            ob[(size_t)r * L] = DSCORE ? alpha * v_ : v_;
-        }
+            ob[(size_t)r * L] = DSCORE ? alpha * v_ : v_ + ad[r];
+        }
+#pragma unroll
+        for (int r = 0; r < 4; ++r) ad[r] = adn[r];
     }
 #undef VF_A3_PV
 #undef VF_A3_LOADV
@@ -427,7 +467,8 @@
 template <int L>
 __global__ __launch_bounds__(L / 32 * 64) void attn_fwd_split_kernel(const float* __restrict__ qkv,
                                                                      float* __restrict__ out, float* __restrict__ P,
-                                                                     int C, float alpha) {
+                                                                     int C, float alpha, const float* __restrict__ bias,
+                                                                     const float* __restrict__ res) {
     constexpr int NW = L / 32, NTH = NW * 64, CKA = 32;
     constexpr int KS = L + 32;
     constexpr int PS = 40;
@@ -522,8 +563,22 @@
     }
     __syncthreads();
 
+    float ad[16], adn[16];
+#pragma unroll
+    for (int r = 0; r < 16; ++r) {
+        const int c = min(wid, ntile - 1) * 32 + 4 * lh + (r & 3) + 8 * (r >> 2);
+        ad[r] = attn_epi(bias, res, c, ((size_t)b * C + c) * L + q0 + li);
+        adn[r] = 0.f;
+    }
     for (int t = wid; t < ntile; t += NW) {
         f32x16 o = {0};
+        if (t + NW < ntile) {
+#pragma unroll
+            for (int r = 0; r < 16; ++r) {
+                const int c = (t + NW) * 32 + 4 * lh + (r & 3) + 8 * (r >> 2);
+                adn[r] = attn_epi(bias, res, c, ((size_t)b * C + c) * L + q0 + li);
+            }
+        }
 #pragma unroll 1
         for (int kbt = 0; kbt < NB; ++kbt) {
             const int nt = kbt + 1 < NB ? t : min(t + NW, ntile - 1), nk = kbt + 1 < NB ? kbt + 1 : 0;
@@ -540,7 +595,10 @@
         }
         float* ob = out + ((size_t)b * C + t * 32 + 4 * lh) * L + q0 + li;
 #pragma unroll
-        for (int r = 0; r < 16; ++r) ob[(size_t)((r & 3) + 8 * (r >> 2)) * L] = o[r];
+        for (int r = 0; r < 16; ++r) {
+            ob[(size_t)((r & 3) + 8 * (r >> 2)) * L] = o[r] + ad[r];
+            ad[r] = adn[r];
+        }
     }
 #undef load_v
 #undef VF_AS_LV1
@@ -548,7 +606,9 @@
 
 template <int L>
 __global__ __launch_bounds__(L / 32 * 64) void attn_fwd_q16_kernel(const float* __restrict__ qkv, float* __restrict__ out,
-                                                                   float* __restrict__ P, int C, float alpha) {
+                                                                   float* __restrict__ P, int C, float alpha,
+                                                                   const float* __restrict__ bias,
+                                                                   const float* __restrict__ res) {
     constexpr int NW = L / 32, QB = 16, PF = 16;
     constexpr int KPI = L < 128 ? L : 128;
     constexpr int NG = KPI / 16, NH = L / KPI;
@@ -642,6 +702,14 @@
 #pragma unroll
         for (int g = 0; g < NG; ++g) pb[g] = *reinterpret_cast<const f32x4*>(Pl + (((KPI / 4) * h + 4 * g + kk) * QB + j) * 4);
         f32x4 o = {0.f, 0.f, 0.f, 0.f};
+        float ad[4] = {0.f, 0.f, 0.f, 0.f};
+        if (NH == 1 || h == 0) {
+#pragma unroll
+            for (int r = 0; r < 4; ++r) {
+                const int c = t * 16 + 4 * kk + r;
+                ad[r] = attn_epi(bias, res, c, ((size_t)b * C + c) * L + q0 + j);
+            }
+        }
 #define VF_Q16_PV(G) if constexpr ((G) < NG) {                                                                \
         o = __builtin_amdgcn_mfma_f32_16x16x4f32(va##G.x, pb[(G) < NG ? (G) : 0][0], o, 0, 0, 0);                 \
         o = __builtin_amdgcn_mfma_f32_16x16x4f32(va##G.y, pb[(G) < NG ? (G) : 0][1], o, 0, 0, 0);                 \
@@ -659,12 +727,12 @@
             __syncthreads();
             if (h == 0) {
 #pragma unroll
-                for (int r = 0; r < 4; ++r) ob[(size_t)r * L] = o[r] + oxs[wid >> 1][r][lane];
+                for (int r = 0; r < 4; ++r) ob[(size_t)r * L] = (o[r] + oxs[wid >> 1][r][lane]) + ad[r];
             }
             if (base + NW < nitem) __syncthreads();
         } else {
 #pragma unroll
-            for (int r = 0; r < 4; ++r) ob[(size_t)r * L] = o[r];
+            for (int r = 0; r < 4; ++r) ob[(size_t)r * L] = o[r] + ad[r];
         }
     }
 #undef VF_Q16_LOADV
@@ -779,27 +847,33 @@
     return L == 64 ? 3 : 0;
 }
 
-int vf_attention_fwd(const float* qkv, float* out, float* P, int S, int C, int L, void* stream) {
+int vf_attention_fwd_epi(const float* qkv, float* out, float* P, const float* bias, const float* residual, int S, int C,
+                         int L, void* stream) {
     if (S <= 0) return 0;
     if (C % 32 != 0) return (int)hipErrorInvalidValue;
     const float alpha = 1.0f / sqrtf((float)C);
     hipStream_t st = (hipStream_t)stream;
     const int kernel = vf_attention_fwd_kernel(S, C, L);
     if (kernel == 1 && L == 256)
-        hipLaunchKernelGGL(attn_fwd_q16_kernel<256>, dim3(16, S), dim3(512), 0, st, qkv, out, P, C, alpha);
+        hipLaunchKernelGGL(attn_fwd_q16_kernel<256>, dim3(16, S), dim3(512), 0, st, qkv, out, P, C, alpha, bias, residual);
     else if (kernel == 1)
-        hipLaunchKernelGGL(attn_fwd_q16_kernel<64>, dim3(4, S), dim3(128), 0, st, qkv, out, P, C, alpha);
+        hipLaunchKernelGGL(attn_fwd_q16_kernel<64>, dim3(4, S), dim3(128), 0, st, qkv, out, P, C, alpha, bias, residual);
     else if (kernel == 2)
-        hipLaunchKernelGGL(attn_fwd_q32_kernel<false>, dim3(8 * S), dim3(256), 0, st, qkv, out, P, C, alpha, S, nullptr, nullptr);
+        hipLaunchKernelGGL(attn_fwd_q32_kernel<false>, dim3(8 * S), dim3(256), 0, st, qkv, out, P, C, alpha, S, nullptr, nullptr,
+                           bias, residual);
     else if (kernel == 3 && L == 256)
-        hipLaunchKernelGGL(attn_fwd_split_kernel<256>, dim3(8, S), dim3(512), 0, st, qkv, out, P, C, alpha);
+        hipLaunchKernelGGL(attn_fwd_split_kernel<256>, dim3(8, S), dim3(512), 0, st, qkv, out, P, C, alpha, bias, residual);
     else if (kernel == 4)
-        hipLaunchKernelGGL(attn_fwd_kh_kernel, dim3(2, S), dim3(512), 0, st, qkv, out, P, C, alpha);
+        hipLaunchKernelGGL(attn_fwd_kh_kernel, dim3(2, S), dim3(512), 0, st, qkv, out, P, C, alpha, bias, residual);
     else if (kernel == 3)
-        hipLaunchKernelGGL(attn_fwd_split_kernel<64>, dim3(2, S), dim3(128), 0, st, qkv, out, P, C, alpha);
+        hipLaunchKernelGGL(attn_fwd_split_kernel<64>, dim3(2, S), dim3(128), 0, st, qkv, out, P, C, alpha, bias, residual);
     else
         return (int)hipErrorInvalidValue;
     VF_RETURN_LAST_ERROR();
+}
+
+int vf_attention_fwd(const float* qkv, float* out, float* P, int S, int C, int L, void* stream) {
+    return vf_attention_fwd_epi(qkv, out, P, nullptr, nullptr, S, C, L, stream);
 }
 
 int vf_attention_dscore(const float* qkv, const float* dO, const float* P, float* dS, float* dqkv, int S, int C, int L,
@@ -807,7 +881,7 @@
     if (S <= 0) return 0;
     if (L != 256 || C % 32 != 0 || C < 32) return (int)hipErrorInvalidValue;
     hipLaunchKernelGGL(attn_fwd_q32_kernel<true>, dim3(8 * S), dim3(256), 0, (hipStream_t)stream, qkv, dqkv,
-                       const_cast<float*>(P), C, 1.0f / sqrtf((float)C), S, dO, dS);
+                       const_cast<float*>(P), C, 1.0f / sqrtf((float)C), S, dO, dS, nullptr, nullptr);
     VF_RETURN_LAST_ERROR();
 }
 
diff --git a/view_fusion_amd/csrc/gemm.hip b/view_fusion_amd/csrc/gemm.hip
--- a/view_fusion_amd/csrc/gemm.hip
+++ b/view_fusion_amd/csrc/gemm.hip
@@ -354,7 +354,145 @@
 
 }
 
+namespace {
+
+struct FoldRow {
+    const float* A;
+    const float* B;
+    float* C;
+    const float* cp_src;
+    float* cp_dst;
+    long long M, N, K, sAm, sAk, sBk, sBn, ldc, cp_n, first;
+};
+
+struct FoldRows2 { FoldRow r[2]; };
+
+constexpr int FT = 32, FK = 64;
+
+__global__ __launch_bounds__(256) void fold_gemm_kernel(const FoldRow* __restrict__ tab, FoldRows2 inl, int nrows) {
+    __shared__ float As[FT][FK + 1];
+    __shared__ float Bs[FK][FT + 1];
+    const int tid = threadIdx.x;
+    int ri = 0;
+    FoldRow d;
+    if (tab) {
+        while (ri + 1 < nrows && tab[ri + 1].first <= (long long)blockIdx.x) ++ri;
+        d = tab[ri];
+    } else {
+        ri = (nrows > 1 && inl.r[1].first <= (long long)blockIdx.x) ? 1 : 0;
+        d = ri ? inl.r[1] : inl.r[0];
+    }
+    const int M = (int)d.M, N = (int)d.N, K = (int)d.K;
+    const int tn = (N + FT - 1) / FT, tm = (M + FT - 1) / FT;
+    const int bl = blockIdx.x - (int)d.first;
+    const int m0 = (bl / tn) * FT, n0 = (bl % tn) * FT;
+    const int tx = tid & 31, ty = tid >> 5;
+    const bool a_kfast = d.sAk == 1, b_nfast = d.sBn == 1;
+    const int sAm = (int)d.sAm, sAk = (int)d.sAk, sBk = (int)d.sBk, sBn = (int)d.sBn;
+    int am[8], ak[8], bk[8], bn[8];
+#pragma unroll
+    for (int i = 0; i < 8; ++i) {
+        const int e = tid + 256 * i;
+        if (a_kfast) { ak[i] = e & 63; am[i] = e >> 6; } else { am[i] = e & 31; ak[i] = e >> 5; }
+        if (b_nfast) { bn[i] = e & 31; bk[i] = e >> 5; } else { bk[i] = e & 63; bn[i] = e >> 6; }
+    }
+    float ra[8], rb[8];
+#define VF_FOLD_LOAD(K0)                                                                                        \
+    _Pragma("unroll") for (int i = 0; i < 8; ++i) {                                                             \
+        const int m = m0 + am[i], ka = (K0) + ak[i], kb = (K0) + bk[i], n = n0 + bn[i];                         \
+        const float va = d.A[min(m, M - 1) * sAm + min(ka, K - 1) * sAk];                                       \
+        const float vb = d.B[min(kb, K - 1) * sBk + min(n, N - 1) * sBn];                                       \
+        ra[i] = (m < M && ka < K) ? va : 0.f;                                                                   \
+        rb[i] = (kb < K && n < N) ? vb : 0.f;                                                                   \
+    }
+    float acc[4] = {0.f, 0.f, 0.f, 0.f};
+    VF_FOLD_LOAD(0)
+    const long long cstep = (long long)tm * tn * 256, c0i = (long long)bl * 256 + tid;
+    const bool cp4 = d.cp_src && (d.cp_n & 3) == 0 &&
+                     ((reinterpret_cast<size_t>(d.cp_src) | reinterpret_cast<size_t>(d.cp_dst)) & 15) == 0;
+    const long long n4 = cp4 ? d.cp_n >> 2 : 0;
+    float4 cv0 = make_float4(0.f, 0.f, 0.f, 0.f), cv1 = cv0;
+    if (c0i < n4) cv0 = reinterpret_cast<const float4*>(d.cp_src)[c0i];
+    if (c0i + cstep < n4) cv1 = reinterpret_cast<const float4*>(d.cp_src)[c0i + cstep];
+    for (int k0 = 0; k0 < K; k0 += FK) {
+        __syncthreads();
+#pragma unroll
+        for (int i = 0; i < 8; ++i) {
+            As[am[i]][ak[i]] = ra[i];
+            Bs[bk[i]][bn[i]] = rb[i];
+        }
+        __syncthreads();
+        if (k0 + FK < K) { VF_FOLD_LOAD(k0 + FK) }
+#pragma unroll
+        for (int k = 0; k < FK; ++k) {
+            const float bv = Bs[k][tx];
+#pragma unroll
+            for (int i = 0; i < 4; ++i) acc[i] = fmaf(As[ty + 8 * i][k], bv, acc[i]);
+        }
+    }
+#undef VF_FOLD_LOAD
+    if (n0 + tx < N) {
+#pragma unroll
+        for (int i = 0; i < 4; ++i)
+            if (m0 + ty + 8 * i < M) d.C[(long long)(m0 + ty + 8 * i) * d.ldc + n0 + tx] = acc[i];
+    }
+    if (cp4) {
+        if (c0i < n4) reinterpret_cast<float4*>(d.cp_dst)[c0i] = cv0;
+        if (c0i + cstep < n4) reinterpret_cast<float4*>(d.cp_dst)[c0i + cstep] = cv1;
+        for (long long i = c0i + 2 * cstep; i < n4; i += cstep)
+            reinterpret_cast<float4*>(d.cp_dst)[i] = reinterpret_cast<const float4*>(d.cp_src)[i];
+    } else if (d.cp_src) {
+        for (long long i = c0i; i < d.cp_n; i += cstep) d.cp_dst[i] = d.cp_src[i];
+    }
+}
+
+inline FoldRow fold_row(const float* A, const float* B, float* C, int n, long sAm, long sAk, long sBk, long sBn,
+                        const float* cp_src, float* cp_dst, long cp_n, long first) {
+    FoldRow r;
+    r.A = A; r.B = B; r.C = C; r.cp_src = cp_src; r.cp_dst = cp_dst;
+    r.M = r.N = r.K = n; r.sAm = sAm; r.sAk = sAk; r.sBk = sBk; r.sBn = sBn; r.ldc = n; r.cp_n = cp_n; r.first = first;
+    return r;
+}
+
+}
+
 extern "C" {
+
+long vf_attn_fold_blocks(int C) { return C > 0 ? (long)((C + FT - 1) / FT) * ((C + FT - 1) / FT) : 0; }
+
+int vf_attn_fold(const float* w_qkv, const float* w_out, float* w_fold, int C, void* stream) {
+    if (C <= 0) return (int)hipErrorInvalidValue;
+    const size_t cc = (size_t)C * C;
+    FoldRows2 t;
+    t.r[0] = fold_row(w_out, w_qkv + 2 * cc, w_fold + 2 * cc, C, C, 1, C, 1, w_qkv, w_fold, (long)(2 * cc), 0);
+    t.r[1] = t.r[0];
+    hipLaunchKernelGGL(fold_gemm_kernel, dim3((unsigned)vf_attn_fold_blocks(C)), dim3(256), 0, (hipStream_t)stream,
+                       (const FoldRow*)nullptr, t, 1);
+    VF_RETURN_LAST_ERROR();
+}
+
+int vf_attn_fold_multi(const void* desc, int nlayers, long total_blocks, void* stream) {
+    if (nlayers <= 0 || total_blocks <= 0) return 0;
+    if (!desc) return (int)hipErrorInvalidValue;
+    FoldRows2 t = {};
+    hipLaunchKernelGGL(fold_gemm_kernel, dim3((unsigned)total_blocks), dim3(256), 0, (hipStream_t)stream,
+                       (const FoldRow*)desc, t, nlayers);
+    VF_RETURN_LAST_ERROR();
+}
+
+int vf_attn_fold_bwd(const float* dw_fold, const float* w_qkv, const float* w_out, float* dw_qkv, float* dw_out, int C,
+                     void* stream) {
+    if (C <= 0) return (int)hipErrorInvalidValue;
+    const size_t cc = (size_t)C * C;
+    const long nb = vf_attn_fold_blocks(C);
+    const float* dB = dw_fold + 2 * cc;
+    FoldRows2 t;
+    t.r[0] = fold_row(dB, w_qkv + 2 * cc, dw_out, C, C, 1, 1, C, dw_fold, dw_qkv, (long)(2 * cc), 0);
+    t.r[1] = fold_row(w_out, dB, dw_qkv + 2 * cc, C, 1, C, C, 1, nullptr, nullptr, 0, nb);
+    hipLaunchKernelGGL(fold_gemm_kernel, dim3((unsigned)(2 * nb)), dim3(256), 0, (hipStream_t)stream,
+                       (const FoldRow*)nullptr, t, 2);
+    VF_RETURN_LAST_ERROR();
+}
 
 int vf_bgemm(const float* A, const float* B, float* C, const float* bias, int batch, int M, int N, int K,
              long sAb, long sAm, long sAk, long sBb, long sBk, long sBn, long sCb, long sCm, long sCn,
diff --git a/view_fusion_amd/ops/__init__.py b/view_fusion_amd/ops/__init__.py
--- a/view_fusion_amd/ops/__init__.py
+++ b/view_fusion_amd/ops/__init__.py
@@ -33,7 +33,8 @@
     time_affine_all
 )
 from .attention import (
-    _AttentionFn, _AttentionStreamFn, _ConcatFn, attention, attention_route, attention_streaming, concat_channels
+    FoldedQKV, _AttentionFn, _AttentionFoldFn, _AttentionStreamFn, _ConcatFn, _FoldFn, attention, attention_fold,
+    attention_route, attention_streaming, concat_channels, folded_qkv
 )
 from .diffusion import (
     _ComposeLossFn, _ComposeLossOptFn, compose, compose_loss, compose_mse_loss, draw_train, gather_level, p_sample_tail, philox_ids, psnr, randn_ids,
diff --git a/view_fusion_amd/ops/attention.py b/view_fusion_amd/ops/attention.py
--- a/view_fusion_amd/ops/attention.py
+++ b/view_fusion_amd/ops/attention.py
@@ -4,6 +4,7 @@
 
 from .state import st
 from .core import _c, _call, _check, _launch, _ptr, _stream
+from .deferred import _fold_late, _gout, _rowsum_get
 from .dense import _bgemm
 
 
@@ -34,34 +35,37 @@
     @staticmethod
     def backward(ctx, dO):
         qkv, P = ctx.saved_tensors
-        dO = _c(dO)
-        S, C3, H, W = qkv.shape
-        C, L = C3 // 3, H * W
-        alpha = 1.0 / math.sqrt(C)
-        dqkv = torch.empty_like(qkv)
-        dS = torch.empty_like(P)
-        st._KIND_OVERRIDE = "attn_bwd" if st.KERNEL_LOG is not None else None
-        fused_dq = False
-        if L == 256 and C % 32 == 0 and st.ATTN_DSCORE:
-            _call("vf_attention_dscore", _ptr(qkv), _ptr(dO), _ptr(P), _ptr(dS), _ptr(dqkv), S, C, L, _stream(),
-                  flops=4.0 * S * L * L * C)
-            fused_dq = True
-        else:
-            _bgemm(dO, qkv, dS, None, S, L, L, C, (C * L, 1, L), (C3 * L, L, 1), (L * L, L, 1), offB=2 * C * L)
-            _call("vf_softmax_bwd", _ptr(P), _ptr(dS), _ptr(dS), S * L, L, _stream())
-        if fused_dq and C % 64 == 0 and st.ATTN_DVDK:
-            _call("vf_attention_dvdk", _ptr(qkv), _ptr(dO), _ptr(P), _ptr(dS), _ptr(dqkv), S, C, L, _stream(),
-                  flops=4.0 * S * L * L * C)
-            st._KIND_OVERRIDE = None
-            return dqkv, None
-        _bgemm(dO, P, dqkv, None, S, C, L, L, (C * L, L, 1), (L * L, L, 1), (C3 * L, L, 1), offC=2 * C * L)
-        if not fused_dq:
-            _bgemm(qkv, dS, dqkv, None, S, C, L, L, (C3 * L, L, 1), (L * L, 1, L), (C3 * L, L, 1), alpha,
-                   offA=C * L, offC=0)
-        _bgemm(qkv, dS, dqkv, None, S, C, L, L, (C3 * L, L, 1), (L * L, L, 1), (C3 * L, L, 1), alpha,
-               offA=0, offC=C * L)
+        return _attention_backward(qkv, P, _c(dO)), None
+
+
+def _attention_backward(qkv, P, dO):
+    S, C3, H, W = qkv.shape
+    C, L = C3 // 3, H * W
+    alpha = 1.0 / math.sqrt(C)
+    dqkv = torch.empty_like(qkv)
+    dS = torch.empty_like(P)
+    st._KIND_OVERRIDE = "attn_bwd" if st.KERNEL_LOG is not None else None
+    fused_dq = False
+    if L == 256 and C % 32 == 0 and st.ATTN_DSCORE:
+        _call("vf_attention_dscore", _ptr(qkv), _ptr(dO), _ptr(P), _ptr(dS), _ptr(dqkv), S, C, L, _stream(),
+              flops=4.0 * S * L * L * C)
+        fused_dq = True
+    else:
+        _bgemm(dO, qkv, dS, None, S, L, L, C, (C * L, 1, L), (C3 * L, L, 1), (L * L, L, 1), offB=2 * C * L)
+        _call("vf_softmax_bwd", _ptr(P), _ptr(dS), _ptr(dS), S * L, L, _stream())
+    if fused_dq and C % 64 == 0 and st.ATTN_DVDK:
+        _call("vf_attention_dvdk", _ptr(qkv), _ptr(dO), _ptr(P), _ptr(dS), _ptr(dqkv), S, C, L, _stream(),
+              flops=4.0 * S * L * L * C)
         st._KIND_OVERRIDE = None
-        return dqkv, None
+        return dqkv
+    _bgemm(dO, P, dqkv, None, S, C, L, L, (C * L, L, 1), (L * L, L, 1), (C3 * L, L, 1), offC=2 * C * L)
+    if not fused_dq:
+        _bgemm(qkv, dS, dqkv, None, S, C, L, L, (C3 * L, L, 1), (L * L, 1, L), (C3 * L, L, 1), alpha,
+               offA=C * L, offC=0)
+    _bgemm(qkv, dS, dqkv, None, S, C, L, L, (C3 * L, L, 1), (L * L, L, 1), (C3 * L, L, 1), alpha,
+           offA=0, offC=C * L)
+    st._KIND_OVERRIDE = None
+    return dqkv
 
 
 STREAM_MIN_L = 4097
@@ -111,6 +115,129 @@
     if attention_route(qkv.shape[1] // 3, qkv.shape[2] * qkv.shape[3]) == "stream":
         return attention_streaming(qkv)
     return _AttentionFn.apply(qkv, torch.is_grad_enabled() and qkv.requires_grad)
+
+
+
+
+_PACK_ATTRS = ("_vf_pack", "_vf_wpack", "_vf_w4pack", "_vf_pack3")
+
+
+class FoldedQKV:
+    bias = None
+
+    def __init__(self, ch):
+        self.ch = ch
+        self.weight = None
+        self.key = None
+        self.fresh = False
+
+    def buffer(self, like):
+        if self.weight is None or self.weight.device != like.device:
+            self.weight = torch.empty(3 * self.ch, self.ch, 1, 1, device=like.device, dtype=torch.float32)
+            self.key, self.fresh = None, False
+            for attr in _PACK_ATTRS:
+                if getattr(self, attr, None) is not None:
+                    setattr(self, attr, None)
+        return self.weight
+
+    def stale_packs(self):
+        for attr in _PACK_ATTRS:
+            c = getattr(self, attr, None)
+            if c is not None and c[0] is not None:
+                setattr(self, attr, (None, c[1], c[2]))
+            if getattr(self, attr + "_fresh", False):
+                setattr(self, attr + "_fresh", False)
+
+
+class _FoldFn(torch.autograd.Function):
+
+    @staticmethod
+    def forward(ctx, wqkv, wout, holder):
+        ctx.save_for_backward(wqkv, wout)
+        return holder.weight.detach()
+
+    @staticmethod
+    def backward(ctx, dwf):
+        wqkv, wout = ctx.saved_tensors
+        dwf = _c(dwf)
+        C = wout.shape[0]
+        dwq = _gout(wqkv, 3 * C, C, 1, 1, like=dwf)
+        dwo = _gout(wout, C, C, 1, 1, like=dwf)
+        if _fold_late(dwf):
+            st.fold_pending.append((dwf, wqkv.detach(), wout.detach(), dwq, dwo, C))
+            dwq, dwo = dwq.view_as(dwq), dwo.view_as(dwo)
+        else:
+            _call("vf_attn_fold_bwd", _ptr(dwf), _ptr(wqkv.detach()), _ptr(wout.detach()), _ptr(dwq), _ptr(dwo), C,
+                  _stream(), flops=4.0 * C * C * C)
+        return (dwq if ctx.needs_input_grad[0] else None), (dwo if ctx.needs_input_grad[1] else None), None
+
+
+def folded_qkv(attn):
+    h = attn._vf_fold
+    wq, wo = attn.qkv.weight, attn.out.weight
+    _check(wq.detach(), wo.detach())
+    buf = h.buffer(wq)
+    training = torch.is_grad_enabled() and (wq.requires_grad or wo.requires_grad)
+    key = None if training else (wq._version, wq.data_ptr(), wo._version, wo.data_ptr())
+    if h.fresh and training:
+        h.fresh = False
+    elif training or h.key != key:
+        _call("vf_attn_fold", _ptr(wq.detach()), _ptr(wo.detach()), _ptr(buf), h.ch, _stream(), flops=2.0 * h.ch ** 3)
+        h.stale_packs()
+        h.fresh = False
+    h.key = key
+    if not training:
+        return h, buf
+    w = _FoldFn.apply(wq, wo, h)
+    w._vf_owners = (wq, wo)
+    return h, w
+
+
+class _AttentionFoldFn(torch.autograd.Function):
+
+    @staticmethod
+    def forward(ctx, qkv, bias, residual, need_p):
+        _check(qkv, bias, residual)
+        S, C3, H, W = qkv.shape
+        C, L = C3 // 3, H * W
+        y = torch.empty(S, C, H, W, device=qkv.device, dtype=torch.float32)
+        P = torch.empty(S, L, L, device=qkv.device, dtype=torch.float32) if need_p else None
+        _launch("attn_fwd", 4.0 * S * L * L * C, "vf_attention_fwd_epi", _ptr(qkv), _ptr(y), _ptr(P), _ptr(bias),
+                _ptr(residual), S, C, L, _stream(),
+                nbytes=4.0 * (qkv.numel() + (2 if residual is not None else 1) * y.numel() + (S * L * L if need_p else 0)))
+        ctx.save_for_backward(qkv, P)
+        ctx.pb = bias
+        return y
+
+    @staticmethod
+    def backward(ctx, dy):
+        qkv, P = ctx.saved_tensors
+        dy = _c(dy)
+        S, C, H, W = dy.shape
+        dqkv = _attention_backward(qkv, P, dy) if ctx.needs_input_grad[0] else None
+        db = None
+        if ctx.pb is not None and ctx.needs_input_grad[1]:
+            hit = _rowsum_get(dy)
+            db = hit[2].view_as(hit[2]) if (hit is not None and hit[2] is not None) else None
+            if db is None:
+                dvb = hit[1] if hit is not None else None
+                if dvb is None and C >= 192:
+                    db = _gout(ctx.pb, C, like=dy)
+                    _call("vf_bias_grad", _ptr(dy), _ptr(db), None, S, C, H * W, _stream())
+                else:
+                    if dvb is None:
+                        dvb = torch.empty(S, C, device=dy.device, dtype=torch.float32)
+                        _call("vf_rowsum", _ptr(dy), _ptr(dvb), S * C, H * W, _stream())
+                    db = _gout(ctx.pb, C, like=dy)
+                    _call("vf_colsum", _ptr(dvb), _ptr(db), 1, S, C, _stream())
+        return dqkv, db, (dy if ctx.needs_input_grad[2] else None), None
+
+
+def attention_fold(qkv, bias, residual):
+    S, C3, H, W = qkv.shape
+    if attention_route(C3 // 3, H * W) != "fused":
+        raise ValueError(f"attention_fold: C = {C3 // 3}, L = {H * W} is not on the fused route")
+    return _AttentionFoldFn.apply(qkv, bias, residual, torch.is_grad_enabled() and qkv.requires_grad)
 
 
 class _ConcatFn(torch.autograd.Function):
diff --git a/view_fusion_amd/ops/conv.py b/view_fusion_amd/ops/conv.py
--- a/view_fusion_amd/ops/conv.py
+++ b/view_fusion_amd/ops/conv.py
@@ -174,9 +174,13 @@
                     db = db_here.view_as(db_here)
         elif ctx.needs_input_grad[1]:
             need = _lib.load().vf_conv_wgrad_ws_floats(S, Cin, Cout, H, W, KS)
-            dw = _gout(ctx.pw, Cout, Cin, KS, KS, like=x)
-            if _wgrad("vf_conv_wgrad", (_ptr(x), _ptr(dy), _ptr(dw)), (S, Cin, Cout, H, W, KS, m), need, [ctx.pw],
+            leaf = ctx.pw.is_leaf
+            owners = [ctx.pw] if leaf else list(getattr(ctx.pw, "_vf_owners", None) or [None])
+            dw = _gout(ctx.pw if leaf else None, Cout, Cin, KS, KS, like=x)
+            if _wgrad("vf_conv_wgrad", (_ptr(x), _ptr(dy), _ptr(dw)), (S, Cin, Cout, H, W, KS, m), need, owners,
                       (dw, None, None), True, ctx.flops, ctx.tag, strm):
+                if not leaf:
+                    st._LATE_DW.add(dw.data_ptr())
                 dw = dw.view_as(dw)
         if want_b or want_v:
             if (want_v and dvb is None) or (want_b and db is None and dvb is None):
@@ -275,7 +279,8 @@
     return _Conv1x1CatFn.apply(x1, x2, layer.weight, layer.bias, layer, training)
 
 
-def conv2d(x, layer, view_bias=None, residual=None, mode="same", twin=None, tap=False, res_fold=None):
+def conv2d(x, layer, view_bias=None, residual=None, mode="same", twin=None, tap=False, res_fold=None, weight=None):
+    w = layer.weight if weight is None else weight
     if not torch.is_grad_enabled():
         S, Cin, Hi, Wi = x.shape
         Cout, _, KS, _ = layer.weight.shape
@@ -289,10 +294,10 @@
             y = _conv_small(x, None, layer.weight, layer.bias, view_bias, residual, S, Cin, Cout, H, W, KS, m)
             return (y, x) if tap else y
     assert res_fold is None
-    training = torch.is_grad_enabled() and layer.weight.requires_grad
+    training = torch.is_grad_enabled() and w.requires_grad
     if tap and torch.is_grad_enabled():
-        return _Conv2dFn.apply(x, layer.weight, layer.bias, view_bias, residual, layer, mode, training, twin, True)
-    y = _Conv2dFn.apply(x, layer.weight, layer.bias, view_bias, residual, layer, mode, training, twin)
+        return _Conv2dFn.apply(x, w, layer.bias, view_bias, residual, layer, mode, training, twin, True)
+    y = _Conv2dFn.apply(x, w, layer.bias, view_bias, residual, layer, mode, training, twin)
     return (y, x) if tap else y
 
 
diff --git a/view_fusion_amd/ops/core.py b/view_fusion_amd/ops/core.py
--- a/view_fusion_amd/ops/core.py
+++ b/view_fusion_amd/ops/core.py
@@ -55,6 +55,7 @@
               "vf_colsum": "reduce", "vf_colsum_multi": "reduce", "vf_rowsum": "reduce", "vf_bias_grad": "reduce",
               "vf_sumpool2": "reduce", "vf_conv_pack_weights": "pack", "vf_wino_pack_weights": "pack",
               "vf_conv_pack_weights_multi": "pack", "vf_wino_pack_weights_multi": "pack",
+              "vf_attn_fold": "pack", "vf_attn_fold_multi": "pack", "vf_attn_fold_bwd": "pack",
               "vf_time_affine_fwd": "embed", "vf_time_affine_bwd": "embed", "vf_sincos_embed": "embed",
               "vf_swish_fwd": "embed", "vf_swish_bwd": "embed",
               "vf_stack_views": "diffusion", "vf_compose_fwd": "diffusion", "vf_compose_mse_bwd": "diffusion",
diff --git a/view_fusion_amd/ops/deferred.py b/view_fusion_amd/ops/deferred.py
--- a/view_fusion_amd/ops/deferred.py
+++ b/view_fusion_amd/ops/deferred.py
@@ -182,8 +182,20 @@
     return st.col_sums.end_capture(), st.slab_sums.end_capture()
 
 
+def _fold_late(dwf):
+    return dwf.data_ptr() in st._LATE_DW
+
+
+def _fold_flush():
+    pend, st.fold_pending = st.fold_pending, []
+    st._LATE_DW.clear()
+    for dwf, wq, wo, dwq, dwo, C in pend:
+        _call("vf_attn_fold_bwd", _ptr(dwf), _ptr(wq), _ptr(wo), _ptr(dwq), _ptr(dwo), C, _stream(), flops=4.0 * C * C * C)
+
+
 def _flush():
     st.slab_sums.flush()
+    _fold_flush()
     for a in st._WRED_ARENA.values():
         a.used = 0
     st._PENDING_TASK = None
@@ -219,6 +231,8 @@
         if torch.cuda.is_current_stream_capturing():
             st.col_sums.pending.clear()
             st.slab_sums.pending.clear()
+            st.fold_pending.clear()
+            st._LATE_DW.clear()
         else:
             _flush()
     if not st.col_sums.pending and not st.slab_sums.pending:
@@ -228,13 +242,15 @@
 
 
 def flush_deferred():
-    if st.col_sums.pending or st.slab_sums.pending:
+    if st.col_sums.pending or st.slab_sums.pending or st.fold_pending:
         _flush()
 
 
 def drop_deferred():
     st.col_sums.pending.clear()
     st.slab_sums.pending.clear()
+    st.fold_pending.clear()
+    st._LATE_DW.clear()
     st._PENDING_TASK = None
     for a in st._WRED_ARENA.values():
         a.used = 0
diff --git a/view_fusion_amd/ops/packing.py b/view_fusion_amd/ops/packing.py
--- a/view_fusion_amd/ops/packing.py
+++ b/view_fusion_amd/ops/packing.py
@@ -77,10 +77,17 @@
 
 def pack_all(root, S=None, hw=None):
     plan = getattr(root, "_vf_pack_plan", None)
-    layers = plan[0] if plan is not None else [m for m in root.modules() if isinstance(m, torch.nn.Conv2d)]
+    if plan is not None:
+        layers, folds = plan[0], plan[3]
+    else:
+        layers = [m for m in root.modules() if isinstance(m, torch.nn.Conv2d)]
+        folds = [m for m in root.modules() if getattr(m, "_vf_fold", None) is not None]
+        layers += [m._vf_fold for m in folds]
     if not layers:
         return
     _check(layers[0].weight.detach())
+    for m in folds:
+        m._vf_fold.buffer(m.qkv.weight)
 
     if hw is None:
         size = getattr(root, "_vf_image_size", None)
@@ -118,8 +125,22 @@
             first[kind] += nblk
         descs = tuple((torch.tensor(rows[k], dtype=torch.int64).to(dev) if rows[k] else None, len(rows[k]), first[k])
                       for k in (0, 1, 2))
-        plan = (layers, key, descs)
+        frows, ffirst = [], 0
+        for m in folds:
+            wq, wo, wf, C = m.qkv.weight, m.out.weight, m._vf_fold.weight, m._vf_fold.ch
+            v = 8 * C * C
+            frows.append([wo.data_ptr(), wq.data_ptr() + v, wf.data_ptr() + v, wq.data_ptr(), wf.data_ptr(), C, C, C,
+                          C, 1, C, 1, C, 2 * C * C, ffirst])
+            ffirst += _lib.load().vf_attn_fold_blocks(C)
+        fdesc = (torch.tensor(frows, dtype=torch.int64).to(dev) if frows else None, len(frows), ffirst)
+        plan = (layers, key, descs, folds, fdesc)
         object.__setattr__(root, "_vf_pack_plan", plan)
+    if folds and st.ATTN_FOLD:
+        fdesc = plan[4]
+        _call("vf_attn_fold_multi", ctypes.c_void_p(fdesc[0].data_ptr()), fdesc[1], fdesc[2], _stream())
+    for m in folds:
+        h = m._vf_fold
+        h.key, h.fresh = None, bool(st.ATTN_FOLD)
     for k, fn in ((0, "vf_conv_pack_weights_multi"), (1, "vf_wino_pack_weights_multi"), (2, "vf_wino44_pack_weights_multi")):
         desc, n, blk = plan[2][k]
         if n:
diff --git a/view_fusion_amd/ops/state.py b/view_fusion_amd/ops/state.py
--- a/view_fusion_amd/ops/state.py
+++ b/view_fusion_amd/ops/state.py
@@ -23,6 +23,7 @@
         self.WINO_GN_FUSION = os.environ.get("VF_WINO_GN", "1") == "1"
         self.ATTN_DSCORE = os.environ.get("VF_ATTN_DSCORE", "1") != "0"
         self.ATTN_DVDK = os.environ.get("VF_ATTN_DVDK", "1") != "0"
+        self.ATTN_FOLD = int(os.environ.get("VF_ATTN_FOLD", "1"))
         self.BF16X3 = os.environ.get("VF_BF16X3") == "1"
         self.ROWSUM_FUSION = True
         self.COLSUM_DEFER = True
@@ -31,6 +32,8 @@
         self.col_sums = None
         self.slab_sums = None
         self._PENDING_TASK = None
+        self.fold_pending = []
+        self._LATE_DW = set()
         self._WRED_ARENA = {}
         self._ws = {}
         self._WINO_KIND_CACHE = {}
diff --git a/view_fusion_amd/unet.py b/view_fusion_amd/unet.py
--- a/view_fusion_amd/unet.py
+++ b/view_fusion_amd/unet.py
@@ -88,6 +88,8 @@
         self.qkv = nn.Conv2d(ch, ch * 3, 1, bias=False)
         self.out = nn.Conv2d(ch, ch, 1)
         self.groups = groups
+        from .ops.attention import FoldedQKV
+        object.__setattr__(self, "_vf_fold", FoldedQKV(ch))
 
     def forward(self, x, n=None):
         from . import ops
@@ -95,6 +97,10 @@
             n, xs = ops.group_norm_skip(x, self.norm.weight, self.norm.bias, self.groups, silu=False)
         else:
             xs = x
+        if ops.st.ATTN_FOLD and ops.attention_route(x.shape[1], x.shape[2] * x.shape[3]) == "fused":
+            holder, w = ops.folded_qkv(self)
+            qkv = ops.conv2d(n, holder, weight=w)
+            return ops.attention_fold(qkv, self.out.bias, xs)
         qkv = ops.conv2d(n, self.qkv)
         o = ops.attention(qkv)
         return ops.conv2d(o, self.out, residual=xs)
@@ -198,6 +204,7 @@
                 attn_levels.add(lvl)
                 mark(blk.attn.qkv, lvl)
                 mark(blk.attn.out, lvl)
+                mark(blk.attn._vf_fold, lvl)
 
         lvl = 0
         for layer in self.downs:
```

Result: no change. 3257 view denoise-steps/s (UNet fwd+bwd per stacked view, incl. compose/MSE/Adam) (median of 6 runs) (+0.8%).
